# acmater/prograph

Measured on AMD Instinct MI355X. Metric: sequence-pairs/s, higher is better.
Workload: dtype u8; 1 GPU; cfg3: N=200000 L=64 Hamming, kNN k=16; N=200000, L=64, rows_per_gpu=200000, alphabet=5-bit tokens 1..20, parallelism=rowblock1, engine=mfma

## Files before the change

include/prograph_hip.h:

```cpp
#ifndef PROGRAPH_HIP_H
#define PROGRAPH_HIP_H

#include <stdint.h>

#ifdef __cplusplus
extern "C" {
#endif

#define PG_ABI_VERSION 3

#define PG_E_BADARG   (-1)
#define PG_E_TOOLONG  (-2)
#define PG_E_TOOMANY  (-3)
#define PG_E_NODEV    (-4)
#define PG_E_COMM     (-5)

#define PG_MAX_L      128
#define PG_MAX_L_5BIT 255
#define PG_MAX_N_KNN  16777216
#define PG_MAX_K      63
#define PG_LEV_MAX_BAND 8

#define PG_BITS_5 5
#define PG_BITS_8 8

#define PG_CMP_LE 0
#define PG_CMP_LT 1
#define PG_CMP_EQ 2
#define PG_CMP_GE 3
#define PG_CMP_GT 4
#define PG_CMP_KEEP_ZERO 0x10

int         pg_version(void);
const char *pg_last_error(void);
int         pg_device_info(int *cu_count, int *wave_size, char *arch, int arch_len);

int64_t     pg_npad(int64_t n);
int         pg_ngroups(int l);
int         pg_nchunks(int l, int bits);
int64_t     pg_planes_bytes(int64_t n, int l, int bits);
int64_t     pg_workspace_bytes(int64_t nrows);

int pg_pack_planes(const void *src, int elem_bytes, int64_t n, int l, int64_t ld,
                   const int64_t *rows, int bits, void *planes, int64_t npad, uint32_t *flags,
                   void *stream);

int pg_pack_bytes(const uint8_t *src, int64_t n, int width, int64_t ld, const int64_t *rows, const uint8_t *lut256,
                  int bits, void *planes, int64_t npad, uint8_t *tokens_out, uint32_t *flags, void *stream);

int pg_hamming_dense(const void *x_planes, int64_t n, int64_t x_npad,
                     const void *y_planes, int64_t m, int64_t y_npad,
                     int l, int bits, void *out, int out_elem_bytes, int64_t ldo,
                     int accumulate, void *stream);

int pg_eps_slots(const void *row_planes, int64_t row_npad, int64_t row0, int64_t nrows,
                 const void *col_planes, int64_t col_npad, int64_t ncols,
                 int l, int bits, int cmp, double eps, int cap,
                 int32_t *slot_idx, uint8_t *slot_w, uint32_t *counts, void *workspace, void *stream);

int pg_eps_slots_sym(const void *planes, int64_t npad, int64_t n, int l, int bits, int cmp, double eps, int cap,
                     int32_t *slot_idx, uint8_t *slot_w, uint32_t *counts_up, uint32_t *counts_lo, void *workspace,
                     void *stream);
int pg_eps_compact_sym(const void *planes, int64_t npad, int64_t n, int l, int bits, int cmp, double eps, int cap,
                       const int32_t *slot_idx, const uint8_t *slot_w, const uint32_t *counts_up,
                       const uint32_t *counts_lo, const int64_t *indptr, int32_t *indices, uint8_t *weights,
                       int leave_overflow, void *stream);

int64_t pg_scan_scratch_bytes(int64_t n);
int pg_exclusive_scan(const uint32_t *counts, int64_t n, int64_t *indptr, void *scratch,
                      void *stream);

int pg_eps_compact(const void *row_planes, int64_t row_npad, int64_t row0, int64_t nrows,
                   const void *col_planes, int64_t col_npad, int64_t ncols,
                   int l, int bits, int cmp, double eps, int cap,
                   const int32_t *slot_idx, const uint8_t *slot_w, const uint32_t *counts,
                   const int64_t *indptr, int32_t *indices, uint8_t *weights, int leave_overflow, void *stream);

int pg_eps_fill_rows(const void *row_planes, int64_t row_npad, int64_t row0, const int64_t *row_list, int64_t n_list,
                     const void *col_planes, int64_t col_npad, int64_t ncols, int l, int bits, int cmp, double eps,
                     const int64_t *indptr, int32_t *indices, uint8_t *weights, uint32_t *scratch_counts, void *workspace,
                     void *stream);

int pg_knn_hamming(const void *row_planes, int64_t row_npad, int64_t row0, int64_t nrows,
                   const void *col_planes, int64_t col_npad, int64_t ncols,
                   int l, int bits, int k, int32_t *idx_out, uint8_t *dist_out,
                   void *workspace, void *stream);

int64_t pg_knn_sym_plan(int64_t n, int64_t slots, int piece, int piece_min, int32_t *out, int64_t max_passes);

int pg_knn_hamming_round(const void *row_planes, int64_t row_npad, int64_t row0, int64_t nrows,
                         const void *col_planes, int64_t col_npad, int64_t ncols, int l, int bits,
                         int k, int first_round, const uint32_t *floor_keys, uint32_t *last_keys,
                         int32_t *idx_out, uint8_t *dist_out, void *workspace, void *stream);

int64_t pg_query_workspace_bytes(int64_t nq, int64_t ndb, int k);
int pg_query_knn_hamming(const void *q_planes, int64_t nq, int64_t q_npad, const void *db_planes, int64_t ndb,
                         int64_t db_npad, int l, int bits, int k, const uint32_t *floor_keys, uint32_t *last_keys,
                         int32_t *idx_out, uint8_t *dist_out, void *workspace, int64_t workspace_bytes, void *stream);

int64_t pg_query_eps_segments(int64_t nq, int64_t ndb);
int pg_query_eps_count(const void *q_planes, int64_t nq, int64_t q_npad, const void *db_planes, int64_t ndb,
                       int64_t db_npad, int l, int bits, int cmp, double eps, int64_t nseg, uint32_t *seg_counts,
                       void *stream);
int pg_query_eps_fill(const void *q_planes, int64_t nq, int64_t q_npad, const void *db_planes, int64_t ndb,
                      int64_t db_npad, int l, int bits, int cmp, double eps, int64_t nseg, const int64_t *seg_indptr,
                      int32_t *indices, uint8_t *weights, void *stream);

int pg_index_flags(const void *planes, int64_t n, int64_t npad, int l, int bits,
                   int64_t ref, const uint32_t *want_dist, int pos_mode,
                   const uint32_t *pos_mask, const uint32_t *not_mask,
                   uint8_t *dist_out, uint64_t *hist, uint8_t *flags, void *stream);

int pg_lev_profile(const uint8_t *tokens, int64_t n, int l, int64_t ld, void *profiles,
                   int64_t npad, int32_t *lens, uint32_t *flags, void *stream);
int pg_lev_candidates(const void *profiles, int64_t npad, int64_t n, int64_t row0, int64_t nrows,
                      int band, int cap, int32_t *slot_idx, uint8_t *slot_w, uint32_t *counts,
                      void *stream);
int pg_lev_candidates_sym(const void *profiles, int64_t npad, int64_t n, int band, int cap,
                          int32_t *slot_idx, uint8_t *slot_w, int32_t *slot_aux, uint32_t *counts_up,
                          uint32_t *counts_lo, void *stream);
int pg_lev_knn(const uint8_t *tokens, int64_t n, int l, int64_t ld, const void *planes128,
               int64_t npad, const int32_t *lens, int64_t row0, int64_t nrows, int band, int k,
               int cap, const int32_t *slot_idx, uint8_t *slot_w, const int32_t *slot_aux,
               const uint32_t *counts, const uint32_t *counts_lo, int32_t *idx_out, uint8_t *dist_out,
               void *stream);

int pg_levenshtein_dense(const void *x_planes128, int64_t n, int64_t x_npad, const int32_t *x_lens,
                         const void *y_planes128, int64_t m, int64_t y_npad, const int32_t *y_lens, int l,
                         void *out, int out_elem_bytes, int64_t ldo, void *stream);
int pg_lev_eps_pairs(const uint8_t *tokens, int64_t n, int l, int64_t ld, const void *planes128,
                     int64_t npad, const int32_t *lens, int band, int cap, const int32_t *slot_idx,
                     uint8_t *slot_w, const int32_t *slot_aux, const uint32_t *counts_up,
                     const uint32_t *counts_lo, void *stream);
int pg_lev_eps_count(int64_t n, int cap, int cmp, int thr, const uint8_t *slot_w,
                     const uint32_t *counts_up, const uint32_t *counts_lo, uint32_t *counts_out,
                     void *stream);
int pg_lev_eps_fill(int64_t n, int cap, int cmp, int thr, const int32_t *slot_idx, const uint8_t *slot_w,
                    const uint32_t *counts_up, const uint32_t *counts_lo, const int64_t *indptr,
                    int32_t *indices, uint8_t *weights, void *stream);

#define PG_LEV_LONG_MAX_L 2048
int pg_lev_long_pack(const uint8_t *tokens, int64_t n, int l, int64_t ld, void *planes, int64_t npad, int32_t *lens,
                     uint32_t *flags, void *stream);
int pg_levenshtein_long_dense(const void *x_planes, int64_t n, int64_t x_npad, const int32_t *x_lens, int xl,
                              const void *y_planes, int64_t m, int64_t y_npad, const int32_t *y_lens, int yl, void *out,
                              int out_elem_bytes, int64_t ldo, void *stream);

int pg_sub_pack(const uint8_t *tokens, int64_t n, int l, int64_t ld, int a, void *packed, int64_t npad,
                uint32_t *flags, void *stream);
int pg_substitution_dense(const void *x_packed, int64_t n, int64_t x_npad, const void *y_packed, int64_t m,
                          int64_t y_npad, int l, const uint8_t *cost_u8, void *out, int64_t ldo,
                          int out_elem_bytes, int accumulate, void *stream);

int pg_alignment_dense(const void *x_packed, int64_t n, int64_t x_npad, int xl, const void *y_packed, int64_t m,
                       int64_t y_npad, int yl, const uint8_t *cost_u8, int gap, void *out, int64_t ldo,
                       int out_elem_bytes, void *stream);

int pg_alignment_affine_dense(const void *x_packed, int64_t n, int64_t x_npad, int xl, const void *y_packed, int64_t m,
                              int64_t y_npad, int yl, const uint8_t *cost_u8, int gap, int gap_open, void *out,
                              int64_t ldo, int out_elem_bytes, void *stream);

int pg_alignment_local_dense(const void *x_packed, int64_t n, int64_t x_npad, int xl, const void *y_packed, int64_t m,
                             int64_t y_npad, int yl, const int8_t *score_i8, int gap, int gap_open, void *out,
                             int64_t ldo, int out_elem_bytes, void *stream);

#define PG_ALN_LONG_MAX_L 2048
int pg_alignment_long_workspace(int xl, int64_t *one_workgroup_bytes, int64_t *full_bytes);
int pg_alignment_long_dense(const void *x_packed, int64_t n, int64_t x_npad, int xl, const void *y_packed, int64_t m,
                            int64_t y_npad, int yl, const uint8_t *cost_u8, int gap, int gap_open, void *out,
                            int64_t ldo, int out_elem_bytes, void *workspace, int64_t workspace_bytes, void *stream);
int pg_alignment_local_long_dense(const void *x_packed, int64_t n, int64_t x_npad, int xl, const void *y_packed, int64_t m,
                                  int64_t y_npad, int yl, const int8_t *score_i8, int gap, int gap_open, void *out,
                                  int64_t ldo, int out_elem_bytes, void *workspace, int64_t workspace_bytes,
                                  void *stream);

int pg_alignment_semiglobal_dense(const void *x_packed, int64_t n, int64_t x_npad, int xl, const void *y_packed, int64_t m,
                                  int64_t y_npad, int yl, const int8_t *score_i8, int gap, int gap_open, void *out,
                                  int64_t ldo, int out_elem_bytes, void *stream);
int pg_alignment_semiglobal_long_dense(const void *x_packed, int64_t n, int64_t x_npad, int xl, const void *y_packed, int64_t m,
                                       int64_t y_npad, int yl, const int8_t *score_i8, int gap, int gap_open, void *out,
                                       int64_t ldo, int out_elem_bytes, void *workspace, int64_t workspace_bytes,
                                       void *stream);

int pg_alignment_fit_dense(const void *x_packed, int64_t n, int64_t x_npad, int xl, const void *y_packed, int64_t m,
                           int64_t y_npad, int yl, const int8_t *score_i8, int gap, int gap_open, int bias, void *out,
                           int64_t ldo, int out_elem_bytes, void *stream);
int pg_alignment_fit_long_dense(const void *x_packed, int64_t n, int64_t x_npad, int xl, const void *y_packed, int64_t m,
                                int64_t y_npad, int yl, const int8_t *score_i8, int gap, int gap_open, int bias, void *out,
                                int64_t ldo, int out_elem_bytes, void *workspace, int64_t workspace_bytes, void *stream);

int pg_alignment_profile_dense(int mode, const void *x_packed, int64_t n, int64_t x_npad, int xl, const void *profiles,
                               const int32_t *lengths, int64_t m, int lpad, int yl, int bias, int top, int gap, int gap_open,
                               int out_bias, void *out, int64_t ldo, int out_elem_bytes, void *stream);
int pg_alignment_profile_long_dense(int mode, const void *x_packed, int64_t n, int64_t x_npad, int xl, const void *profiles,
                                    const int32_t *lengths, int64_t m, int lpad, int yl, int bias, int top, int gap,
                                    int gap_open, int out_bias, void *out, int64_t ldo, int out_elem_bytes, void *workspace,
                                    int64_t workspace_bytes, void *stream);

#define PG_ALN_TRACE_GLOBAL 0
#define PG_ALN_TRACE_LOCAL 1
#define PG_ALN_TRACE_SEMIGLOBAL 2
int pg_alignment_trace_workspace(int xl, int yl, int64_t *bytes_per_wave);
int pg_alignment_trace(int mode, const void *x_packed, int64_t n, int64_t x_npad, int xl, const void *y_packed, int64_t m,
                       int64_t y_npad, int yl, const int32_t *xi, const int32_t *yi, int64_t npairs, const void *table, int gap,
                       int gap_open, int32_t *head, uint8_t *ops, int64_t ldo, void *workspace, int64_t workspace_bytes,
                       void *stream);
int pg_alignment_trace_long_workspace(int xl, int yl, int64_t *bytes_per_wave);
int pg_alignment_trace_long(int mode, const void *x_packed, int64_t n, int64_t x_npad, int xl, const void *y_packed, int64_t m,
                            int64_t y_npad, int yl, const int32_t *xi, const int32_t *yi, int64_t npairs, const void *table,
                            int gap, int gap_open, int32_t *head, uint8_t *ops, int64_t ldo, void *workspace,
                            int64_t workspace_bytes, void *stream);
int pg_alignment_fit_trace(const void *x_packed, int64_t n, int64_t x_npad, int xl, const void *y_packed, int64_t m,
                           int64_t y_npad, int yl, const int32_t *xi, const int32_t *yi, int64_t npairs, const void *table,
                           int gap, int gap_open, int32_t *head, uint8_t *ops, int64_t ldo, void *workspace,
                           int64_t workspace_bytes, void *stream);
int pg_alignment_fit_trace_long(const void *x_packed, int64_t n, int64_t x_npad, int xl, const void *y_packed, int64_t m,
                                int64_t y_npad, int yl, const int32_t *xi, const int32_t *yi, int64_t npairs,
                                const void *table, int gap, int gap_open, int32_t *head, uint8_t *ops, int64_t ldo,
                                void *workspace, int64_t workspace_bytes, void *stream);

int pg_alignment_stats(int mode, const void *x_packed, int64_t n, int64_t x_npad, int xl, const void *y_packed, int64_t m,
                       int64_t y_npad, int yl, const int32_t *xi, const int32_t *yi, int64_t npairs, const void *table, int gap,
                       int gap_open, int32_t *head, void *stream);

int pg_alignment_list_scores(int mode, const void *x_packed, int64_t n, int64_t x_npad, int xl, const void *y_packed, int64_t m,
                             int64_t y_npad, int yl, const int64_t *indptr, const int32_t *indices, const void *table, int gap,
                             int gap_open, int32_t *scores, void *stream);

int pg_alignment_list_long_scores(int mode, const void *x_packed, int64_t n, int64_t x_npad, int xl, const void *y_packed,
                                  int64_t m, int64_t y_npad, int yl, const int64_t *indptr, const int32_t *indices,
                                  const void *table, int gap, int gap_open, int32_t *scores, void *workspace,
                                  int64_t workspace_bytes, void *stream);

int pg_spectrum_dims(int k, int symbols, int dims);
int pg_spectrum_profile(const uint8_t *tokens, int64_t n, int l, int64_t ld, const int64_t *rows, int k, int symbols, int dims,
                        void *out_f16, int64_t ldo, int32_t *flags, void *stream);

int pg_csr_row_stats(const int64_t *indptr, const int32_t *indices, const uint8_t *weights_u8,
                     const float *weights_f32, int64_t nrows, int64_t row0, const double *f, double *deg,
                     double *sum_f, double *sum_wf, double *self_w, double *col_sum, void *stream);

#define PG_W_UNSIGNED 0
#define PG_W_SIGNED 1
#define PG_W_FLOAT 2
#define PG_SYM_UNION 0
#define PG_SYM_MUTUAL 1
#define PG_COMBINE_MIN 0
#define PG_COMBINE_MAX 1
int64_t pg_csr_sort_workspace(int64_t nnz);
int pg_csr_sort_rows_count(const int64_t *indptr, const int32_t *indices, int64_t nrows, int64_t nnz, int64_t ncols,
                           uint32_t *counts, void *workspace, int64_t workspace_bytes, void *stream);
int pg_csr_sort_rows_fill(const int64_t *indptr, const void *weights, int elem_bytes, int64_t nrows, int64_t nnz,
                          const uint32_t *counts, const int64_t *out_indptr, int32_t *out_indices, void *out_weights,
                          const void *workspace, int64_t workspace_bytes, void *stream);
int pg_csr_histogram(const int32_t *indices, int64_t nnz, int64_t ncols, uint32_t *counts, void *stream);
int64_t pg_csr_transpose_workspace(int64_t nnz, int64_t ncols);
int pg_csr_transpose(const int64_t *indptr, const int32_t *indices, const void *weights, int elem_bytes, int64_t nrows,
                     int64_t nnz, int64_t ncols, int64_t row0, const int64_t *t_indptr, int32_t *t_indices, void *t_weights,
                     void *workspace, int64_t workspace_bytes, void *stream);
int64_t pg_csr_symmetrize_workspace(int64_t nnz_a, int64_t nnz_t);
int pg_csr_symmetrize_count(const int64_t *a_indptr, const int32_t *a_indices, const void *a_weights, int64_t nnz_a,
                            const int64_t *t_indptr, const int32_t *t_indices, const void *t_weights, int64_t nnz_t,
                            int elem_bytes, int kind, int mode, int combine, int64_t nrows, uint32_t *counts, void *workspace,
                            int64_t workspace_bytes, void *stream);
int pg_csr_symmetrize_fill(const int64_t *a_indptr, int64_t nnz_a, const int64_t *t_indptr, int64_t nnz_t, int elem_bytes,
                           int64_t nrows, const int64_t *out_indptr, int32_t *out_indices, void *out_weights,
                           const void *workspace, int64_t workspace_bytes, void *stream);

int pg_compact_flags(const uint8_t *flags, int64_t n, int64_t *out_idx, int64_t *out_count,
                     void *scratch, void *stream);

int pg_f16_nchunks(int d);
int pg_pack_f16(const void *src_f16, int64_t n, int d, int64_t ld, const int64_t *rows, void *packed, int64_t npad,
                void *stream);
int pg_minkowski_dense(const void *x_packed, int64_t n, int64_t x_npad, const void *y_packed, int64_t m,
                       int64_t y_npad, int d, int similarity, void *out_f16, int64_t ldo, void *stream);
int pg_f16_knn(const void *dist_f16, int64_t m, int64_t n, int64_t ld, int k, int first, int descending,
               int32_t *idx_out, void *w_out_f16, void *stream);
int pg_f16_knn_round(const void *dist_f16, int64_t m, int64_t n, int64_t ld, int k, int descending,
                     const int32_t *floor_idx, const void *floor_w_f16, int64_t floor_ld, int32_t *idx_out,
                     void *w_out_f16, int64_t ldo, void *stream);
int pg_f16_eps_count(const void *dist_f16, int64_t m, int64_t n, int64_t ld, int cmp, float eps_f16, int similarity,
                     uint32_t *counts, void *stream);
int pg_f16_eps_fill(const void *dist_f16, int64_t m, int64_t n, int64_t ld, int cmp, float eps_f16, int similarity,
                    const int64_t *indptr, int32_t *indices, void *weights_f16, void *stream);

int pg_i32_knn(const int32_t *vals, int64_t m, int64_t n, int64_t ld, int k, int first, int descending, int32_t *idx_out,
               int32_t *w_out, void *stream);
int pg_i32_knn_round(const int32_t *vals, int64_t m, int64_t n, int64_t ld, int k, int descending,
                     const int32_t *floor_idx, const int32_t *floor_w, int64_t floor_ld, int32_t *idx_out, int32_t *w_out,
                     int64_t ldo, void *stream);
int pg_i32_eps_count(const int32_t *vals, int64_t m, int64_t n, int64_t ld, int cmp, int64_t thr, uint32_t *counts,
                     void *stream);
int pg_i32_eps_fill(const int32_t *vals, int64_t m, int64_t n, int64_t ld, int cmp, int64_t thr, const int64_t *indptr,
                    int32_t *indices, int32_t *weights, void *stream);

int pg_minkowski_knn(const void *x_packed, int64_t n, int64_t x_npad, const void *y_packed, int64_t m, int64_t y_npad,
                     int d, int similarity, int k, int first, int32_t *idx_out, void *w_out_f16, void *stream);
int pg_minkowski_knn_round(const void *x_packed, int64_t n, int64_t x_npad, const void *y_packed, int64_t m,
                           int64_t y_npad, int d, int similarity, int k, const int32_t *floor_idx,
                           const void *floor_w_f16, int64_t floor_ld, int32_t *idx_out, void *w_out_f16, int64_t ldo,
                           void *stream);
int pg_minkowski_eps_slots(const void *x_packed, int64_t n, int64_t x_npad, const void *y_packed, int64_t m,
                           int64_t y_npad, int d, int similarity, int cmp, float eps_f16, int cap, int32_t *slot_idx,
                           void *slot_w_f16, uint32_t *counts, void *stream);
int pg_minkowski_eps_compact(int64_t m, int cap, const int32_t *slot_idx, const void *slot_w_f16, const uint32_t *counts,
                             const int64_t *indptr, int32_t *indices, void *weights_f16, void *stream);
int pg_minkowski_eps_fill_rows(const void *x_packed, int64_t n, int64_t x_npad, const void *y_packed, int64_t m,
                               int64_t y_npad, int d, int similarity, int cmp, float eps_f16, const int64_t *row_list,
                               int64_t n_list, const int64_t *indptr, int32_t *indices, void *weights_f16, void *stream);

int pg_cosine_prep(const void *packed, int64_t n, int64_t npad, int d, float *norms, float *rnorms, uint32_t *flags,
                   void *stream);
int pg_cosine_dense(const void *x_packed, const float *x_norms, const float *x_rnorms, int64_t n, int64_t x_npad,
                    const void *y_packed, const float *y_norms, const float *y_rnorms, int64_t m, int64_t y_npad, int d,
                    int similarity, float *out, int64_t ldo, void *stream);
int pg_cosine_knn(const void *x_packed, const float *x_norms, const float *x_rnorms, int64_t n, int64_t x_npad,
                  const void *y_packed, const float *y_norms, const float *y_rnorms, int64_t m, int64_t y_npad, int d,
                  int similarity, int k, int first, int32_t *idx_out, float *w_out, void *stream);
int pg_cosine_knn_round(const void *x_packed, const float *x_norms, const float *x_rnorms, int64_t n, int64_t x_npad,
                        const void *y_packed, const float *y_norms, const float *y_rnorms, int64_t m, int64_t y_npad, int d,
                        int similarity, int k, const int32_t *floor_idx, const float *floor_w, int64_t floor_ld,
                        int32_t *idx_out, float *w_out, int64_t ldo, void *stream);
int pg_cosine_eps_slots(const void *x_packed, const float *x_norms, const float *x_rnorms, int64_t n, int64_t x_npad,
                        const void *y_packed, const float *y_norms, const float *y_rnorms, int64_t m, int64_t y_npad, int d,
                        int similarity, int cmp, float eps, int cap, int32_t *slot_idx, float *slot_w, uint32_t *counts,
                        void *stream);
int pg_cosine_eps_compact(int64_t m, int cap, const int32_t *slot_idx, const float *slot_w, const uint32_t *counts,
                          const int64_t *indptr, int32_t *indices, float *weights, void *stream);
int pg_cosine_eps_fill_rows(const void *x_packed, const float *x_norms, const float *x_rnorms, int64_t n, int64_t x_npad,
                            const void *y_packed, const float *y_norms, const float *y_rnorms, int64_t m, int64_t y_npad,
                            int d, int similarity, int cmp, float eps, const int64_t *row_list, int64_t n_list,
                            const int64_t *indptr, int32_t *indices, float *weights, void *stream);

int pg_euclidean_dense(const void *x_packed, const float *x_norms, const float *x_rnorms, int64_t n, int64_t x_npad,
                       const void *y_packed, const float *y_norms, const float *y_rnorms, int64_t m, int64_t y_npad, int d,
                       int similarity, float *out, int64_t ldo, void *stream);
int pg_euclidean_knn(const void *x_packed, const float *x_norms, const float *x_rnorms, int64_t n, int64_t x_npad,
                     const void *y_packed, const float *y_norms, const float *y_rnorms, int64_t m, int64_t y_npad, int d,
                     int similarity, int k, int first, int32_t *idx_out, float *w_out, void *stream);
int pg_euclidean_knn_round(const void *x_packed, const float *x_norms, const float *x_rnorms, int64_t n, int64_t x_npad,
                           const void *y_packed, const float *y_norms, const float *y_rnorms, int64_t m, int64_t y_npad,
                           int d, int similarity, int k, const int32_t *floor_idx, const float *floor_w, int64_t floor_ld,
                           int32_t *idx_out, float *w_out, int64_t ldo, void *stream);
int pg_euclidean_eps_slots(const void *x_packed, const float *x_norms, const float *x_rnorms, int64_t n, int64_t x_npad,
                           const void *y_packed, const float *y_norms, const float *y_rnorms, int64_t m, int64_t y_npad,
                           int d, int similarity, int cmp, float eps, int cap, int32_t *slot_idx, float *slot_w,
                           uint32_t *counts, void *stream);
int pg_euclidean_eps_fill_rows(const void *x_packed, const float *x_norms, const float *x_rnorms, int64_t n, int64_t x_npad,
                               const void *y_packed, const float *y_norms, const float *y_rnorms, int64_t m, int64_t y_npad,
                               int d, int similarity, int cmp, float eps, const int64_t *row_list, int64_t n_list,
                               const int64_t *indptr, int32_t *indices, float *weights, void *stream);

#define PG_COMM_ID_BYTES 128
int pg_comm_available(void);
int pg_comm_unique_id(void *id128);
int pg_comm_init(void **comm, int nranks, int rank, const void *id128);
int pg_comm_destroy(void *comm);
int pg_allgather_tokens(void *comm, const void *shard, int64_t rows_per_rank, int l, void *full, void *stream);

#ifdef __cplusplus
}
#endif
#endif
```

prograph_amd/_native.py:

```python
import ctypes
import os
import threading

import numpy as np
import torch

_HERE = os.path.dirname(os.path.abspath(__file__))
LIB_PATH = os.environ.get("PROGRAPH_HIP_LIB") or os.path.join(_HERE, "libprograph_hip.so")
ABI_VERSION = 3

BITS_5, BITS_8 = 5, 8
CMP_LE, CMP_LT, CMP_EQ, CMP_GE, CMP_GT = 0, 1, 2, 3, 4
CMP_KEEP_ZERO = 0x10
MAX_L, MAX_L_5BIT, MAX_K, MAX_K_ROUNDS, MAX_N_KNN, LEV_MAX_BAND = 128, 255, 63, 1023, 1 << 24, 8
SUB_MAX_L, SUB_MAX_A = 2048, 32
ALN_MAX_L, ALN_MAX_GAP = 128, 255
ALN_MAX_OPEN = 255
ALN_LOCAL_MIN, ALN_LOCAL_MAX = -128, 127
ALN_LONG_MAX_L = 2048
ALN_TRACE_GLOBAL, ALN_TRACE_LOCAL, ALN_TRACE_SEMIGLOBAL = 0, 1, 2
ALN_TRACE_FIT = 3
ALN_PROFILE_MODES = ("local", "semiglobal", "fit")
ALN_TRACE_LONG_WORKSPACE = 2 << 30
LEV_LONG_MAX_L = 2048
SPECTRUM_MAX_L, SPECTRUM_MAX_K, SPECTRUM_MAX_D = 2048, 6, 32768
ALN_LONG_CELL_MAX = 65535

SYMBOLS = [
    "pg_version", "pg_last_error", "pg_device_info", "pg_npad", "pg_ngroups", "pg_nchunks", "pg_planes_bytes", "pg_workspace_bytes",
    "pg_pack_planes", "pg_pack_bytes",
    "pg_hamming_dense", "pg_eps_slots", "pg_scan_scratch_bytes", "pg_exclusive_scan",
    "pg_eps_compact", "pg_eps_fill_rows", "pg_eps_slots_sym", "pg_eps_compact_sym", "pg_knn_hamming", "pg_knn_sym_plan", "pg_knn_hamming_round", "pg_index_flags", "pg_compact_flags",
    "pg_lev_profile", "pg_lev_candidates", "pg_lev_candidates_sym", "pg_lev_knn", "pg_csr_row_stats",
    "pg_levenshtein_dense", "pg_lev_eps_pairs", "pg_lev_eps_count", "pg_lev_eps_fill",
    "pg_lev_long_pack", "pg_levenshtein_long_dense",
    "pg_sub_pack", "pg_substitution_dense", "pg_alignment_dense", "pg_alignment_affine_dense",
    "pg_alignment_local_dense", "pg_alignment_long_workspace", "pg_alignment_long_dense", "pg_alignment_local_long_dense",
    "pg_alignment_semiglobal_dense", "pg_alignment_semiglobal_long_dense",
    "pg_alignment_fit_dense", "pg_alignment_fit_long_dense", "pg_alignment_fit_trace", "pg_alignment_fit_trace_long",
    "pg_alignment_profile_dense", "pg_alignment_profile_long_dense",
    "pg_alignment_trace_workspace", "pg_alignment_trace", "pg_alignment_trace_long_workspace", "pg_alignment_trace_long",
    "pg_alignment_stats", "pg_alignment_list_scores", "pg_alignment_list_long_scores",
    "pg_spectrum_dims", "pg_spectrum_profile",
    "pg_i32_knn", "pg_i32_knn_round", "pg_i32_eps_count", "pg_i32_eps_fill",
    "pg_comm_available", "pg_comm_unique_id", "pg_comm_init", "pg_comm_destroy", "pg_allgather_tokens",
    "pg_f16_nchunks", "pg_pack_f16", "pg_minkowski_dense", "pg_f16_knn", "pg_f16_knn_round", "pg_f16_eps_count",
    "pg_f16_eps_fill", "pg_minkowski_knn", "pg_minkowski_knn_round", "pg_minkowski_eps_slots", "pg_minkowski_eps_compact",
    "pg_minkowski_eps_fill_rows", "pg_cosine_prep", "pg_cosine_dense", "pg_cosine_knn", "pg_cosine_knn_round",
    "pg_cosine_eps_slots", "pg_cosine_eps_compact", "pg_cosine_eps_fill_rows",
    "pg_euclidean_dense", "pg_euclidean_knn", "pg_euclidean_knn_round", "pg_euclidean_eps_slots", "pg_euclidean_eps_fill_rows",
    "pg_query_workspace_bytes", "pg_query_knn_hamming",
    "pg_query_eps_segments", "pg_query_eps_count", "pg_query_eps_fill",
    "pg_csr_sort_workspace", "pg_csr_sort_rows_count", "pg_csr_sort_rows_fill", "pg_csr_histogram", "pg_csr_transpose_workspace",
    "pg_csr_transpose", "pg_csr_symmetrize_workspace", "pg_csr_symmetrize_count", "pg_csr_symmetrize_fill",
]


class NativeUnavailable(RuntimeError):
    pass


_lib = None
_lock = threading.Lock()

_i64, _i32, _vp, _dbl = ctypes.c_int64, ctypes.c_int, ctypes.c_void_p, ctypes.c_double
_COS_METRICS = ("cosine", "euclidean")


def _load():
    global _lib
    with _lock:
        if _lib is not None:
            return _lib
        if not os.path.exists(LIB_PATH):
            raise NativeUnavailable(
                f"{LIB_PATH} is missing: build it with `python -c 'import __graft_entry__ as g; g.build()'` "
                "or `make -C prograph_amd/csrc` (hipcc, --offload-arch=gfx950)")
        try:
            lib = ctypes.CDLL(LIB_PATH, mode=ctypes.RTLD_GLOBAL)
        except OSError as e:
            raise NativeUnavailable(f"cannot load {LIB_PATH}: {e}") from e
        missing = [s for s in SYMBOLS if not hasattr(lib, s)]
        if missing:
            raise NativeUnavailable(f"{LIB_PATH} does not export {missing}")
        lib.pg_version.restype = _i32
        if lib.pg_version() != ABI_VERSION:
            raise NativeUnavailable(f"ABI mismatch: library {lib.pg_version()}, binding {ABI_VERSION}")
        lib.pg_last_error.restype = ctypes.c_char_p
        lib.pg_npad.restype = _i64
        lib.pg_npad.argtypes = [_i64]
        lib.pg_ngroups.restype = _i32
        lib.pg_ngroups.argtypes = [_i32]
        lib.pg_nchunks.restype = _i32
        lib.pg_nchunks.argtypes = [_i32, _i32]
        lib.pg_planes_bytes.restype = _i64
        lib.pg_planes_bytes.argtypes = [_i64, _i32, _i32]
        lib.pg_scan_scratch_bytes.restype = _i64
        lib.pg_scan_scratch_bytes.argtypes = [_i64]
        lib.pg_workspace_bytes.restype = _i64
        lib.pg_workspace_bytes.argtypes = [_i64]
        lib.pg_device_info.argtypes = [ctypes.POINTER(_i32), ctypes.POINTER(_i32), ctypes.c_char_p, _i32]
        lib.pg_pack_planes.argtypes = [_vp, _i32, _i64, _i32, _i64, _vp, _i32, _vp, _i64, _vp, _vp]
        lib.pg_pack_bytes.argtypes = [_vp, _i64, _i32, _i64, _vp, _vp, _i32, _vp, _i64, _vp, _vp, _vp]
        lib.pg_hamming_dense.argtypes = [_vp, _i64, _i64, _vp, _i64, _i64, _i32, _i32, _vp, _i32, _i64, _i32, _vp]
        lib.pg_eps_slots.argtypes = [_vp, _i64, _i64, _i64, _vp, _i64, _i64, _i32, _i32, _i32, _dbl, _i32,
                                     _vp, _vp, _vp, _vp, _vp]
        lib.pg_exclusive_scan.argtypes = [_vp, _i64, _vp, _vp, _vp]
        lib.pg_eps_slots_sym.argtypes = [_vp, _i64, _i64, _i32, _i32, _i32, _dbl, _i32, _vp, _vp, _vp, _vp, _vp, _vp]
        lib.pg_eps_compact_sym.argtypes = [_vp, _i64, _i64, _i32, _i32, _i32, _dbl, _i32, _vp, _vp, _vp, _vp, _vp, _vp,
                                           _vp, _i32, _vp]
        lib.pg_eps_compact.argtypes = [_vp, _i64, _i64, _i64, _vp, _i64, _i64, _i32, _i32, _i32, _dbl, _i32,
                                       _vp, _vp, _vp, _vp, _vp, _vp, _i32, _vp]
        lib.pg_eps_fill_rows.argtypes = [_vp, _i64, _i64, _vp, _i64, _vp, _i64, _i64, _i32, _i32, _i32, _dbl,
                                         _vp, _vp, _vp, _vp, _vp, _vp]
        lib.pg_knn_hamming.argtypes = [_vp, _i64, _i64, _i64, _vp, _i64, _i64, _i32, _i32, _i32, _vp, _vp, _vp, _vp]
        lib.pg_knn_sym_plan.restype = _i64
        lib.pg_knn_sym_plan.argtypes = [_i64, _i64, _i32, _i32, _vp, _i64]
        lib.pg_knn_hamming_round.argtypes = [_vp, _i64, _i64, _i64, _vp, _i64, _i64, _i32, _i32, _i32, _i32, _vp, _vp, _vp,
                                             _vp, _vp, _vp]
        lib.pg_query_workspace_bytes.restype = _i64
        lib.pg_query_workspace_bytes.argtypes = [_i64, _i64, _i32]
        lib.pg_query_knn_hamming.argtypes = [_vp, _i64, _i64, _vp, _i64, _i64, _i32, _i32, _i32, _vp, _vp, _vp, _vp, _vp,
                                             _i64, _vp]
        lib.pg_query_eps_segments.restype = _i64
        lib.pg_query_eps_segments.argtypes = [_i64, _i64]
        lib.pg_query_eps_count.argtypes = [_vp, _i64, _i64, _vp, _i64, _i64, _i32, _i32, _i32, _dbl, _i64, _vp, _vp]
        lib.pg_query_eps_fill.argtypes = [_vp, _i64, _i64, _vp, _i64, _i64, _i32, _i32, _i32, _dbl, _i64, _vp, _vp, _vp, _vp]
        lib.pg_index_flags.argtypes = [_vp, _i64, _i64, _i32, _i32, _i64, _vp, _i32, _vp, _vp, _vp, _vp, _vp, _vp]
        lib.pg_compact_flags.argtypes = [_vp, _i64, _vp, _vp, _vp, _vp]
        lib.pg_csr_row_stats.argtypes = [_vp, _vp, _vp, _vp, _i64, _i64, _vp, _vp, _vp, _vp, _vp, _vp, _vp]
        lib.pg_csr_sort_workspace.restype = lib.pg_csr_transpose_workspace.restype = lib.pg_csr_symmetrize_workspace.restype = _i64
        lib.pg_csr_sort_workspace.argtypes = [_i64]
        lib.pg_csr_transpose_workspace.argtypes = lib.pg_csr_symmetrize_workspace.argtypes = [_i64, _i64]
        lib.pg_csr_sort_rows_count.argtypes = [_vp, _vp, _i64, _i64, _i64, _vp, _vp, _i64, _vp]
        lib.pg_csr_sort_rows_fill.argtypes = [_vp, _vp, _i32, _i64, _i64, _vp, _vp, _vp, _vp, _vp, _i64, _vp]
        lib.pg_csr_histogram.argtypes = [_vp, _i64, _i64, _vp, _vp]
        lib.pg_csr_transpose.argtypes = [_vp, _vp, _vp, _i32, _i64, _i64, _i64, _i64, _vp, _vp, _vp, _vp, _i64, _vp]
        lib.pg_csr_symmetrize_count.argtypes = [_vp, _vp, _vp, _i64, _vp, _vp, _vp, _i64, _i32, _i32, _i32, _i32, _i64, _vp, _vp,
                                                _i64, _vp]
        lib.pg_csr_symmetrize_fill.argtypes = [_vp, _i64, _vp, _i64, _i32, _i64, _vp, _vp, _vp, _vp, _i64, _vp]
        lib.pg_lev_profile.argtypes = [_vp, _i64, _i32, _i64, _vp, _i64, _vp, _vp, _vp]
        lib.pg_lev_candidates.argtypes = [_vp, _i64, _i64, _i64, _i64, _i32, _i32, _vp, _vp, _vp, _vp]
        lib.pg_lev_candidates_sym.argtypes = [_vp, _i64, _i64, _i32, _i32, _vp, _vp, _vp, _vp, _vp, _vp]
        lib.pg_lev_knn.argtypes = [_vp, _i64, _i32, _i64, _vp, _i64, _vp, _i64, _i64, _i32, _i32, _i32, _vp, _vp, _vp, _vp,
                                   _vp, _vp, _vp, _vp]
        lib.pg_levenshtein_dense.argtypes = [_vp, _i64, _i64, _vp, _vp, _i64, _i64, _vp, _i32, _vp, _i32, _i64, _vp]
        lib.pg_lev_eps_pairs.argtypes = [_vp, _i64, _i32, _i64, _vp, _i64, _vp, _i32, _i32, _vp, _vp, _vp, _vp, _vp, _vp]
        lib.pg_lev_eps_count.argtypes = [_i64, _i32, _i32, _i32, _vp, _vp, _vp, _vp, _vp]
        lib.pg_lev_eps_fill.argtypes = [_i64, _i32, _i32, _i32, _vp, _vp, _vp, _vp, _vp, _vp, _vp, _vp]
        lib.pg_lev_long_pack.argtypes = [_vp, _i64, _i32, _i64, _vp, _i64, _vp, _vp, _vp]
        lib.pg_levenshtein_long_dense.argtypes = [_vp, _i64, _i64, _vp, _i32, _vp, _i64, _i64, _vp, _i32, _vp, _i32, _i64, _vp]
        lib.pg_sub_pack.argtypes = [_vp, _i64, _i32, _i64, _i32, _vp, _i64, _vp, _vp]
        lib.pg_substitution_dense.argtypes = [_vp, _i64, _i64, _vp, _i64, _i64, _i32, _vp, _vp, _i64, _i32, _i32, _vp]
        lib.pg_alignment_dense.argtypes = [_vp, _i64, _i64, _i32, _vp, _i64, _i64, _i32, _vp, _i32, _vp, _i64, _i32, _vp]
        lib.pg_alignment_affine_dense.argtypes = [_vp, _i64, _i64, _i32, _vp, _i64, _i64, _i32, _vp, _i32, _i32, _vp, _i64, _i32,
                                                  _vp]
        lib.pg_alignment_local_dense.argtypes = lib.pg_alignment_affine_dense.argtypes
        lib.pg_alignment_long_workspace.argtypes = [_i32, ctypes.POINTER(_i64), ctypes.POINTER(_i64)]
        lib.pg_alignment_long_dense.argtypes = [_vp, _i64, _i64, _i32, _vp, _i64, _i64, _i32, _vp, _i32, _i32, _vp, _i64, _i32,
                                                _vp, _i64, _vp]
        lib.pg_alignment_local_long_dense.argtypes = lib.pg_alignment_long_dense.argtypes
        lib.pg_alignment_semiglobal_dense.argtypes = lib.pg_alignment_affine_dense.argtypes
        lib.pg_alignment_semiglobal_long_dense.argtypes = lib.pg_alignment_long_dense.argtypes
        lib.pg_alignment_fit_dense.argtypes = [_vp, _i64, _i64, _i32, _vp, _i64, _i64, _i32, _vp, _i32, _i32, _i32, _vp, _i64,
                                               _i32, _vp]
        lib.pg_alignment_fit_long_dense.argtypes = [_vp, _i64, _i64, _i32, _vp, _i64, _i64, _i32, _vp, _i32, _i32, _i32, _vp,
                                                    _i64, _i32, _vp, _i64, _vp]
        lib.pg_alignment_profile_dense.argtypes = [_i32, _vp, _i64, _i64, _i32, _vp, _vp, _i64, _i32, _i32, _i32, _i32, _i32, _i32,
                                                   _i32, _vp, _i64, _i32, _vp]
        lib.pg_alignment_profile_long_dense.argtypes = lib.pg_alignment_profile_dense.argtypes[:-1] + [_vp, _i64, _vp]
        lib.pg_alignment_trace_workspace.argtypes = [_i32, _i32, ctypes.POINTER(_i64)]
        lib.pg_alignment_trace.argtypes = [_i32, _vp, _i64, _i64, _i32, _vp, _i64, _i64, _i32, _vp, _vp, _i64, _vp, _i32, _i32,
                                           _vp, _vp, _i64, _vp, _i64, _vp]
        lib.pg_alignment_trace_long_workspace.argtypes = lib.pg_alignment_trace_workspace.argtypes
        lib.pg_alignment_trace_long.argtypes = lib.pg_alignment_trace.argtypes
        lib.pg_alignment_fit_trace.argtypes = lib.pg_alignment_trace.argtypes[1:]
        lib.pg_alignment_fit_trace_long.argtypes = lib.pg_alignment_trace.argtypes[1:]
        lib.pg_alignment_stats.argtypes = lib.pg_alignment_trace.argtypes[:16] + [_vp]
        lib.pg_alignment_list_scores.argtypes = [_i32, _vp, _i64, _i64, _i32, _vp, _i64, _i64, _i32, _vp, _vp, _vp, _i32, _i32, _vp, _vp]
        lib.pg_alignment_list_long_scores.argtypes = [_i32, _vp, _i64, _i64, _i32, _vp, _i64, _i64, _i32, _vp, _vp, _vp, _i32, _i32, _vp,
                                                      _vp, _i64, _vp]
        lib.pg_spectrum_dims.argtypes = [_i32, _i32, _i32]
        lib.pg_spectrum_profile.argtypes = [_vp, _i64, _i32, _i64, _vp, _i32, _i32, _i32, _vp, _i64, _vp, _vp]
        lib.pg_i32_knn.argtypes = [_vp, _i64, _i64, _i64, _i32, _i32, _i32, _vp, _vp, _vp]
        lib.pg_i32_knn_round.argtypes = [_vp, _i64, _i64, _i64, _i32, _i32, _vp, _vp, _i64, _vp, _vp, _i64, _vp]
        lib.pg_i32_eps_count.argtypes = [_vp, _i64, _i64, _i64, _i32, _i64, _vp, _vp]
        lib.pg_i32_eps_fill.argtypes = [_vp, _i64, _i64, _i64, _i32, _i64, _vp, _vp, _vp, _vp]
        lib.pg_f16_nchunks.argtypes = [_i32]
        lib.pg_pack_f16.argtypes = [_vp, _i64, _i32, _i64, _vp, _vp, _i64, _vp]
        lib.pg_minkowski_dense.argtypes = [_vp, _i64, _i64, _vp, _i64, _i64, _i32, _i32, _vp, _i64, _vp]
        lib.pg_f16_knn.argtypes = [_vp, _i64, _i64, _i64, _i32, _i32, _i32, _vp, _vp, _vp]
        lib.pg_f16_knn_round.argtypes = [_vp, _i64, _i64, _i64, _i32, _i32, _vp, _vp, _i64, _vp, _vp, _i64, _vp]
        lib.pg_f16_eps_count.argtypes = [_vp, _i64, _i64, _i64, _i32, ctypes.c_float, _i32, _vp, _vp]
        lib.pg_f16_eps_fill.argtypes = [_vp, _i64, _i64, _i64, _i32, ctypes.c_float, _i32, _vp, _vp, _vp, _vp]
        lib.pg_minkowski_knn.argtypes = [_vp, _i64, _i64, _vp, _i64, _i64, _i32, _i32, _i32, _i32, _vp, _vp, _vp]
        lib.pg_minkowski_knn_round.argtypes = [_vp, _i64, _i64, _vp, _i64, _i64, _i32, _i32, _i32, _vp, _vp, _i64, _vp, _vp,
                                               _i64, _vp]
        lib.pg_minkowski_eps_slots.argtypes = [_vp, _i64, _i64, _vp, _i64, _i64, _i32, _i32, _i32, ctypes.c_float, _i32,
                                               _vp, _vp, _vp, _vp]
        lib.pg_minkowski_eps_compact.argtypes = [_i64, _i32, _vp, _vp, _vp, _vp, _vp, _vp, _vp]
        lib.pg_minkowski_eps_fill_rows.argtypes = [_vp, _i64, _i64, _vp, _i64, _i64, _i32, _i32, _i32, ctypes.c_float, _vp,
                                                   _i64, _vp, _vp, _vp, _vp]
        _ops = [_vp, _vp, _vp, _i64, _i64, _vp, _vp, _vp, _i64, _i64, _i32, _i32]
        lib.pg_cosine_prep.argtypes = [_vp, _i64, _i64, _i32, _vp, _vp, _vp, _vp]
        lib.pg_cosine_eps_compact.argtypes = [_i64, _i32, _vp, _vp, _vp, _vp, _vp, _vp, _vp]
        for metric in _COS_METRICS:
            getattr(lib, f"pg_{metric}_dense").argtypes = _ops + [_vp, _i64, _vp]
            getattr(lib, f"pg_{metric}_knn").argtypes = _ops + [_i32, _i32, _vp, _vp, _vp]
            getattr(lib, f"pg_{metric}_knn_round").argtypes = _ops + [_i32, _vp, _vp, _i64, _vp, _vp, _i64, _vp]
            getattr(lib, f"pg_{metric}_eps_slots").argtypes = _ops + [_i32, ctypes.c_float, _i32, _vp, _vp, _vp, _vp]
            getattr(lib, f"pg_{metric}_eps_fill_rows").argtypes = _ops + [_i32, ctypes.c_float, _vp, _i64, _vp, _vp, _vp, _vp]
        lib.pg_comm_unique_id.argtypes = [_vp]
        lib.pg_comm_init.argtypes = [ctypes.POINTER(_vp), _i32, _i32, _vp]
        lib.pg_comm_destroy.argtypes = [_vp]
        lib.pg_allgather_tokens.argtypes = [_vp, _vp, _i64, _i32, _vp, _vp]
        for name in SYMBOLS:
            fn = getattr(lib, name)
            if fn.restype is ctypes.c_int and name not in ("pg_version",):
                fn.restype = _i32
        _lib = lib
        return lib


def lib():
    return _load()


def device():
    if not torch.cuda.is_available():
        raise NativeUnavailable("no HIP device visible to torch; the Hamming/graph path has no CPU fallback")
    return torch.device("cuda", torch.cuda.current_device())


def _check(rc, what):
    if rc != 0:
        msg = lib().pg_last_error().decode("utf-8", "replace")
        raise RuntimeError(f"{what} failed (rc={rc}): {msg}")


def _stream():
    return ctypes.c_void_p(torch.cuda.current_stream().cuda_stream)


def _ptr(t):
    return ctypes.c_void_p(0) if t is None else ctypes.c_void_p(t.data_ptr())


def workspace(nrows, dev):
    return torch.empty(int(lib().pg_workspace_bytes(int(nrows))), dtype=torch.uint8, device=dev)


def npad(n):
    return ((max(int(n), 1) + 255) // 256) * 256


def ngroups(l):
    return (max(int(l), 1) + 31) // 32


def nchunks(l, bits):
    return (ngroups(l) * int(bits) + 3) // 4


def planes_bytes(n, l, bits):
    return (nchunks(l, bits) * 16 + 64) * npad(n)


class Planes:
    __slots__ = ("buf", "n", "l", "npad", "g", "q", "bits", "flags")

    def __init__(self, buf, n, l, bits, flags=None):
        self.buf, self.n, self.l, self.bits, self.flags = buf, int(n), int(l), int(bits), flags
        self.npad, self.g, self.q = npad(n), ngroups(l), nchunks(l, bits)

    def ensure_valid(self):
        if self.flags is not None and int(self.flags.item()):
            raise ValueError(f"tokens outside 0..{(1 << self.bits) - 1} cannot be packed with {self.bits} bit planes")
        self.flags = None

    @property
    def nbytes(self):
        return self.buf.numel()


def pack(tokens, rows=None, bits=None, width=None, check=True):
    L = lib()
    dev = device()
    if not isinstance(tokens, torch.Tensor):
        tokens = torch.from_numpy(np.ascontiguousarray(np.asarray(tokens)))
    if tokens.dim() != 2:
        raise ValueError("token matrix must be 2-D")
    if tokens.dtype not in (torch.uint8, torch.int8, torch.int16, torch.int32, torch.int64):
        raise TypeError(f"integer tokens expected, got {tokens.dtype}")
    if tokens.dtype == torch.int8:
        tokens = tokens.to(torch.int16)
    tokens = tokens.to(dev).contiguous()
    n_src, l = tokens.shape
    lw = l if width is None else int(width)
    if lw < l:
        raise ValueError("width smaller than the token matrix")
    if lw > MAX_L_5BIT:
        raise ValueError(f"L={lw} exceeds the native limit of {MAX_L_5BIT}")
    ridx = None
    n = n_src
    if rows is not None:
        ridx = torch.as_tensor(np.asarray(rows), dtype=torch.int64).reshape(-1)
        if ridx.numel() and (int(ridx.min()) < -n_src or int(ridx.max()) >= n_src):
            raise IndexError("row index out of range")
        ridx = torch.where(ridx < 0, ridx + n_src, ridx).to(dev)
        n = int(ridx.numel())
    if n == 0 or l == 0:
        raise ValueError("empty token matrix")
    if bits is None:
        lo, hi = int(tokens.min()), int(tokens.max())
        if lo < 0 or hi > 255:
            raise ValueError("tokens outside 0..255 cannot use the byte-token Hamming path")
        bits = BITS_5 if hi <= 31 else BITS_8
    if lw > (MAX_L_5BIT if bits == BITS_5 else MAX_L):
        raise ValueError(f"L={lw} exceeds the native limit for {bits} bit planes")
    np_ = npad(n)
    if lw != l:
        wide = torch.zeros((n_src, lw), dtype=tokens.dtype, device=dev)
        wide[:, :l] = tokens
        tokens = wide
    buf = torch.empty(planes_bytes(n, lw, bits), dtype=torch.uint8, device=dev)
    flags = torch.empty(1, dtype=torch.int32, device=dev)
    _check(L.pg_pack_planes(_ptr(tokens), tokens.element_size(), n, lw, tokens.stride(0), _ptr(ridx), int(bits),
                            _ptr(buf), np_, _ptr(flags), _stream()), "pg_pack_planes")
    planes = Planes(buf, n, lw, bits, flags)
    if check:
        planes.ensure_valid()
    return planes


def pack_bytes(raw, lut, bits=BITS_5, want_tokens=True, check=True):
    L = lib()
    dev = device()
    if not isinstance(raw, torch.Tensor):
        raw = torch.from_numpy(np.ascontiguousarray(np.asarray(raw, dtype=np.uint8)))
    if raw.dim() != 2 or raw.dtype != torch.uint8:
        raise TypeError("pack_bytes expects a 2-D uint8 byte matrix")
    raw = raw.to(dev).contiguous()
    n, width = raw.shape
    if n == 0 or width == 0:
        raise ValueError("empty byte matrix")
    if width > (MAX_L_5BIT if bits == BITS_5 else MAX_L):
        raise ValueError(f"L={width} exceeds the native limit for {bits} bit planes")
    lut_t = torch.as_tensor(np.asarray(lut, dtype=np.uint8).reshape(256)).to(dev)
    np_ = npad(n)
    buf = torch.empty(planes_bytes(n, width, bits), dtype=torch.uint8, device=dev)
    flags = torch.empty(1, dtype=torch.int32, device=dev)
    tokens = torch.empty((n, width), dtype=torch.uint8, device=dev) if want_tokens else None
    _check(L.pg_pack_bytes(_ptr(raw), n, width, raw.stride(0), None, _ptr(lut_t), int(bits), _ptr(buf), np_, _ptr(tokens),
                           _ptr(flags), _stream()), "pg_pack_bytes")
    planes = Planes(buf, n, width, bits, flags)
    if check:
        planes.ensure_valid()
    return planes, tokens


_TORCH_OUT = {1: torch.uint8, 2: torch.float16, 4: torch.int32, 8: torch.int64}


def hamming_dense(xp, yp, out_bytes=8, out=None):
    if xp.g != yp.g or xp.bits != yp.bits:
        raise ValueError("operands must be packed with the same width and bit planes")
    accumulate = out is not None
    if out is None:
        out = torch.empty((yp.n, xp.n), dtype=_TORCH_OUT[out_bytes], device=xp.buf.device)
    out_bytes = out.element_size()
    _check(lib().pg_hamming_dense(_ptr(xp.buf), xp.n, xp.npad, _ptr(yp.buf), yp.n, yp.npad, xp.g * 32, xp.bits,
                                  _ptr(out), out_bytes, out.stride(0), 1 if accumulate else 0, _stream()),
           "pg_hamming_dense")
    return out


def _bits2(rp, cp):
    if rp.bits != cp.bits or rp.g != cp.g:
        raise ValueError("row and column operands must be packed with the same width and bit planes")
    return rp.bits


def _csr_alloc(counts, wdtype, extra=None):
    L = lib()
    m, dev = counts.numel(), counts.device
    indptr = torch.empty(m + 1, dtype=torch.int64, device=dev)
    scratch = torch.empty(int(L.pg_scan_scratch_bytes(m)), dtype=torch.uint8, device=dev)
    _check(L.pg_exclusive_scan(_ptr(counts), m, _ptr(indptr), _ptr(scratch), _stream()), "pg_exclusive_scan")
    if extra is None:
        nnz, also = int(indptr[-1].item()), ()
    else:
        nnz, *also = (int(v) for v in torch.stack([indptr[-1], extra]).cpu())
    indices = torch.empty(max(nnz, 1), dtype=torch.int32, device=dev)[:nnz]
    weights = torch.empty(max(nnz, 1), dtype=wdtype, device=dev)[:nnz]
    return (indptr, indices, weights, *also)


def cat_csr(parts):
    if len(parts) == 1:
        return parts[0]
    base, ptrs = 0, [torch.zeros(1, dtype=torch.int64, device=parts[0][0].device)]
    for indptr, _, _ in parts:
        ptrs.append(indptr[1:] + base)
        base += int(indptr[-1].item())
    return torch.cat(ptrs), torch.cat([p_[1] for p_ in parts]), torch.cat([p_[2] for p_ in parts])


def eps_graph(rp, cp, cmp, eps, row0=0, nrows=None, cap=256):
    L = lib()
    nrows = rp.n - row0 if nrows is None else int(nrows)
    dev = rp.buf.device
    bits = _bits2(rp, cp)
    cap = int(cap)
    symenv = os.environ.get("PG_EPS_SYM", "auto")
    sym = (rp is cp and row0 == 0 and nrows == rp.n and rp.n < (1 << 27) and cap >= 2 and symenv != "0"
           and (symenv == "1" or rp.n >= 32768))
    counts = torch.empty(nrows, dtype=torch.int32, device=dev)
    counts_lo = torch.empty(nrows, dtype=torch.int32, device=dev) if sym else None
    slot_idx = torch.empty(nrows * cap, dtype=torch.int32, device=dev)
    slot_w = torch.empty(nrows * cap, dtype=torch.uint8, device=dev)
# ... 1266 lines not shown
```

prograph_amd/csrc/pg_api.hip:

```cpp
#include "pg_common.h"
#include "pg_mm.h"
#include "pg_plan.h"
#include "../../include/prograph_hip.h"

#include <dlfcn.h>
#include <math.h>
#include <rccl/rccl.h>
#include <stdio.h>
#include <stdlib.h>
#include <string.h>
#include <atomic>
#include <mutex>

static thread_local char g_err[256] = "";

void pg_set_error(const char *msg) { snprintf(g_err, sizeof(g_err), "%s", msg); }

extern char **environ;
static PgKnobs read_knobs() { return pg_knobs_read(environ); }

#define PG_MAX_DEVICES 64
static int cu_count() {
  static std::atomic<int> cus[PG_MAX_DEVICES];
  int dev = 0;
  if (hipGetDevice(&dev) != hipSuccess) return 0;
  const bool cached = dev >= 0 && dev < PG_MAX_DEVICES;
  if (cached && cus[dev].load(std::memory_order_relaxed) > 0) return cus[dev].load(std::memory_order_relaxed);
  hipDeviceProp_t prop;
  if (hipGetDeviceProperties(&prop, dev) != hipSuccess) return 0;
  if (cached) cus[dev].store(prop.multiProcessorCount, std::memory_order_relaxed);
  return prop.multiProcessorCount;
}

extern "C" {

int pg_version(void) { return PG_ABI_VERSION; }
const char *pg_last_error(void) { return g_err; }

int pg_device_info(int *cus, int *wave, char *arch, int arch_len) {
  int dev = 0;
  hipDeviceProp_t prop;
  hipError_t e = hipGetDevice(&dev);
  if (e != hipSuccess) return pg_launched((int)e, "hipGetDevice");
  e = hipGetDeviceProperties(&prop, dev);
  if (e != hipSuccess) return pg_launched((int)e, "hipGetDeviceProperties");
  if (cus) *cus = prop.multiProcessorCount;
  if (wave) *wave = prop.warpSize;
  if (arch && arch_len > 0) snprintf(arch, (size_t)arch_len, "%s", prop.gcnArchName);
  return 0;
}

int64_t pg_npad(int64_t n) { return n <= 0 ? 256 : ((n + 255) / 256) * 256; }
int pg_ngroups(int l) { return plan_ngroups(l); }
int pg_nchunks(int l, int bits) { return plan_nchunks(l, bits); }
int64_t pg_planes_bytes(int64_t n, int l, int bits) { return ((int64_t)pg_nchunks(l, bits) * 16 + PG_AUX_BYTES) * pg_npad(n); }
int64_t pg_workspace_bytes(int64_t nrows) { return workspace_bytes(nrows, cu_count(), read_knobs()); }

}

__global__ __launch_bounds__(1024) void pg_knn_sym_plan_kernel(long long nb, long long nst, long long slots, int piece, int pmin,
                                                                int4 *plan, u32 *pieceStart, uint4 *zero, long long zero4) {
  __shared__ u32 sums[1024];
  const int t = threadIdx.x;
  if (blockIdx.x > 0) {
    for (long long i = (long long)(blockIdx.x - 1) * 1024 + t; i < zero4; i += (long long)(gridDim.x - 1) * 1024) zero[i] = make_uint4(0u, 0u, 0u, 0u);
    return;
  }
  const long long per = (nb + 1023) / 1024, b0 = t * per, b1 = b0 + per < nb ? b0 + per : nb;
  u32 mine = 0;
  for (long long b = b0; b < b1; ++b) mine += (u32)sym_block_pieces(b, nst, slots, piece, pmin);
  sums[t] = mine;
  __syncthreads();
  for (int o = 1; o < 1024; o <<= 1) {
    const u32 x = t >= o ? sums[t - o] : 0u;
    __syncthreads();
    sums[t] += x;
    __syncthreads();
  }
  u32 at = sums[t] - mine;
  for (long long b = b0; b < b1; ++b) {
    const int np = sym_block_pieces(b, nst, slots, piece, pmin);
    pieceStart[b] = at;
    for (int q = 0; q < np; ++q, ++at) {
      int f, e;
      sym_piece_range(b, nst, np, q, &f, &e);
      plan[at] = make_int4((int)b, f, e, q);
    }
  }
  if (t == 1023) pieceStart[nb] = sums[1023];
}
extern "C" {
int64_t pg_knn_sym_plan(int64_t n, int64_t slots, int piece, int piece_min, int32_t *out, int64_t max_passes) {
  if (n <= 0 || slots <= 0) return pg_fail(PG_E_BADARG, "pg_knn_sym_plan: bad argument");
  return sym_plan_host(n, slots, piece, piece_min > 0 ? piece_min : (int)read_knobs().symPieceMin.v, out, max_passes);
}
}

#define PG_PACK_SEQS 64
#define PG_PACK_LD 68

__host__ __device__ __forceinline__ unsigned long long pg_transpose8(unsigned long long x) {
  unsigned long long t;
  t = (x ^ (x >> 7)) & 0x00AA00AA00AA00AAull;  x = x ^ t ^ (t << 7);
  t = (x ^ (x >> 14)) & 0x0000CCCC0000CCCCull; x = x ^ t ^ (t << 14);
  t = (x ^ (x >> 28)) & 0x00000000F0F0F0F0ull; x = x ^ t ^ (t << 28);
  return x;
}

template <typename T, int B>
__global__ __launch_bounds__(256) void pg_pack_kernel(const T *__restrict__ src, long long n, int l, long long ld,
                                                      const long long *__restrict__ rows, u32 *__restrict__ planes,
                                                      long long npad, int ng, int nq, u32 *flags,
                                                      const unsigned char *__restrict__ lut = nullptr,
                                                      unsigned char *__restrict__ tokOut = nullptr) {
  constexpr int E = (int)sizeof(T), PER = 16 / E;
  __shared__ __attribute__((aligned(16))) u32 words[PG_PACK_SEQS * PG_PACK_LD];
  const long long s0 = (long long)blockIdx.x * PG_PACK_SEQS;
  const int tid = threadIdx.x;
  const bool vec = !lut && ((unsigned long long)src & 15ull) == 0 && ((ld * E) & 15ll) == 0;
  for (int item = tid; item < PG_PACK_SEQS * ng; item += 256) {
    const int sl = item / ng, g = item - sl * ng;
    const long long s = s0 + sl;
    unsigned long long x[4] = {0, 0, 0, 0}, high = 0;
    if (s < n) {
      const T *row = src + (rows ? rows[s] : s) * ld;
      if (vec && g * 32 + 32 <= l) {
        const uint4 *r16 = reinterpret_cast<const uint4 *>(row + g * 32);
#pragma unroll
        for (int c = 0; c < 32 / PER; ++c) {
          const uint4 v = r16[c];
          T e[PER];
          __builtin_memcpy(e, &v, 16);
#pragma unroll
          for (int i = 0; i < PER; ++i) {
            const int j = c * PER + i;
            const unsigned long long t = (unsigned long long)(long long)e[i];
            high |= t;
            x[j >> 3] |= (t & 0xFFull) << (8 * (j & 7));
          }
        }
      } else {
#pragma unroll
        for (int j = 0; j < 32; ++j) {
          const int pos = g * 32 + j;
          if (pos < l) {
            long long v = (long long)row[pos];
            if (lut) {
              v = lut[(unsigned char)v];
              if (tokOut) tokOut[s * (long long)l + pos] = (unsigned char)v;
            }
            high |= (unsigned long long)v;
            x[j >> 3] |= ((unsigned long long)v & 0xFFull) << (8 * (j & 7));
          }
        }
      }
    }
    if (high >> B) atomicOr(flags, 1u);
#pragma unroll
    for (int i = 0; i < 4; ++i) x[i] = pg_transpose8(x[i]);
#pragma unroll
    for (int p = 0; p < B; ++p) {
      const u32 w = (u32)((x[0] >> (8 * p)) & 0xFFull) | (u32)((x[1] >> (8 * p)) & 0xFFull) << 8 |
                    (u32)((x[2] >> (8 * p)) & 0xFFull) << 16 | (u32)((x[3] >> (8 * p)) & 0xFFull) << 24;
      words[sl * PG_PACK_LD + p * ng + g] = w;
    }
  }
  __syncthreads();
  const int nw = ng * B;
  for (int item = tid; item < PG_PACK_SEQS * nq; item += 256) {
    const int q = item / PG_PACK_SEQS, sl = item % PG_PACK_SEQS;
    uint4 v = *reinterpret_cast<const uint4 *>(&words[sl * PG_PACK_LD + 4 * q]);
    if (4 * q + 1 >= nw) v.y = 0;
    if (4 * q + 2 >= nw) v.z = 0;
    if (4 * q + 3 >= nw) v.w = 0;
    reinterpret_cast<uint4 *>(planes)[(long long)q * npad + s0 + sl] = v;
  }
  const int sl = tid & 63;
  const long long s = s0 + sl;
  if (tid < 64) {
    u32 sigw[2] = {0, 0};
    for (int g = 0; g < ng; ++g) sigw[g & 1] ^= words[sl * PG_PACK_LD + g];
    const unsigned long long sig = pg_sig54(sigw[0], sigw[1]);
    const u32 lo = (u32)sig, hi = (u32)(sig >> 32) | (s < n ? 0xFFC00000u : 0u);
    uint4 *e = reinterpret_cast<uint4 *>(planes + (long long)nq * npad * 4) + (s >> 5) * 64 + (s & 31);
    e[0] = make_uint4(pg_nib8(lo) << 1, pg_nib8(lo >> 8) << 1, pg_nib8(lo >> 16) << 1, pg_nib8(lo >> 24) << 1);
    e[32] = make_uint4(pg_nib8(hi) << 1, pg_nib8(hi >> 8) << 1, pg_nib8(hi >> 16) << 1, pg_nib8(hi >> 24) << 1);
  } else if (tid < 128) {
    u32 fold[8] = {0, 0, 0, 0, 0, 0, 0, 0};
#pragma unroll
    for (int p = 0; p < B; ++p)
      for (int g = 0; g < ng; ++g) fold[p] ^= words[sl * PG_PACK_LD + p * ng + g];
    uint4 *f = reinterpret_cast<uint4 *>(planes + (long long)nq * npad * 4) + npad * 2;
    f[s] = make_uint4(fold[0], fold[1], fold[2], fold[3]);
    f[npad + s] = make_uint4(fold[4], fold[5], fold[6], fold[7]);
  }
}

#define PG_SCAN_TILE 2048

template <typename T>
__device__ __forceinline__ long long scan_val(const T *in, long long i, long long n) {
  return i < n ? (long long)(in[i] != 0 ? (sizeof(T) == 1 ? 1 : in[i]) : 0) : 0;
}

__device__ __forceinline__ long long wave_incl_scan(long long v, int lane) {
#pragma unroll
  for (int o = 1; o < 64; o <<= 1) {
    long long t = __shfl_up(v, o);
    if (lane >= o) v += t;
  }
  return v;
}

__device__ __forceinline__ long long block_excl_scan(long long v, long long &total) {
  __shared__ long long wsum[4];
  const int lane = threadIdx.x & 63, wv = threadIdx.x >> 6;
  const long long inc = wave_incl_scan(v, lane);
  if (lane == 63) wsum[wv] = inc;
  __syncthreads();
  long long base = 0;
  for (int w = 0; w < wv; ++w) base += wsum[w];
  total = wsum[0] + wsum[1] + wsum[2] + wsum[3];
  __syncthreads();
  return base + inc - v;
}

template <typename T>
__global__ __launch_bounds__(256) void pg_scan_partials(const T *__restrict__ in, long long n, long long *partials) {
  const long long b0 = (long long)blockIdx.x * PG_SCAN_TILE;
  long long s = 0;
#pragma unroll
  for (int j = 0; j < 8; ++j) s += scan_val(in, b0 + threadIdx.x * 8 + j, n);
  long long total;
  block_excl_scan(s, total);
  if (threadIdx.x == 0) partials[blockIdx.x] = total;
}

__global__ __launch_bounds__(256) void pg_scan_single(long long *partials, long long nb) {
  long long carry = 0;
  for (long long c0 = 0; c0 < nb; c0 += 256) {
    const long long i = c0 + threadIdx.x;
    const long long v = i < nb ? partials[i] : 0;
    long long total;
    const long long ex = block_excl_scan(v, total);
    if (i < nb) partials[i] = carry + ex;
    carry += total;
  }
  if (threadIdx.x == 0) partials[nb] = carry;
}

template <typename T, int MODE>
__global__ __launch_bounds__(256) void pg_scan_apply(const T *__restrict__ in, long long n, const long long *partials,
                                                     long long nb, long long *out, long long *count) {
  const long long b0 = (long long)blockIdx.x * PG_SCAN_TILE;
  long long v[8], s = 0;
#pragma unroll
  for (int j = 0; j < 8; ++j) { v[j] = scan_val(in, b0 + threadIdx.x * 8 + j, n); s += v[j]; }
  long long total;
  long long ex = block_excl_scan(s, total) + partials[blockIdx.x];
#pragma unroll
  for (int j = 0; j < 8; ++j) {
    const long long i = b0 + threadIdx.x * 8 + j;
    if (i < n) {
      if (MODE == 0) out[i] = ex;
      else if (v[j]) out[ex] = i;
    }
    ex += v[j];
  }
  if (blockIdx.x == 0 && threadIdx.x == 0) {
    if (MODE == 0) out[n] = partials[nb];
    if (count) *count = partials[nb];
  }
}

template <int B>
__global__ __launch_bounds__(256) void pg_index_kernel(const u32 *__restrict__ planes, long long n, long long npad, int ng,
                                                       long long ref, const u32 *__restrict__ want, int posMode,
                                                       const u32 *__restrict__ posMask, const u32 *__restrict__ notMask,
                                                       unsigned char *distOut, u64 *hist, unsigned char *flags) {
  __shared__ u32 lh[256];
  lh[threadIdx.x] = 0;
  __syncthreads();
  const long long s = (long long)blockIdx.x * 256 + threadIdx.x;
  if (s < n) {
    u32 d = 0, anyP = 0, anyNot = 0;
    bool allP = true;
    for (int g = 0; g < ng; ++g) {
      u32 t = 0;
#pragma unroll
      for (int p = 0; p < B; ++p) {
        const int w = p * ng + g;
        const long long base = (long long)(w >> 2) * npad;
        t |= planes[(base + s) * 4 + (w & 3)] ^ planes[(base + ref) * 4 + (w & 3)];
      }
      d += __builtin_popcount(t);
      if (posMode) {
        const u32 pm = posMask[g], nm = notMask[g];
        anyP |= t & pm;
        allP = allP && ((t & pm) == pm);
        anyNot |= t & nm;
      }
    }
    if (distOut) distOut[s] = (unsigned char)d;
    if (hist) atomicAdd(&lh[d & 255u], 1u);
    if (flags) {
      bool ok = want ? ((want[(d >> 5) & 7u] >> (d & 31u)) & 1u) != 0 : true;
      if (posMode == 1) ok = ok && (anyP != 0) && (anyNot == 0);
      if (posMode == 2) ok = ok && allP && (anyNot == 0);
      flags[s] = ok ? 1 : 0;
    }
  }
  __syncthreads();
  if (hist && lh[threadIdx.x]) atomicAdd((unsigned long long *)&hist[threadIdx.x], (unsigned long long)lh[threadIdx.x]);
}

__device__ __forceinline__ double wave_sum(double v) {
#pragma unroll
  for (int o = 32; o > 0; o >>= 1) v += __shfl_down(v, o);
  return v;
}

__global__ __launch_bounds__(256) void pg_csr_row_stats_kernel(const long long *__restrict__ indptr,
                                                               const int *__restrict__ indices,
                                                               const unsigned char *__restrict__ w8,
                                                               const float *__restrict__ wf, long long nrows,
                                                               long long row0, const double *__restrict__ f, double *deg,
                                                               double *sf, double *swf, double *selfw, double *colsum) {
  const int lane = threadIdx.x & 63;
  const long long row = (long long)blockIdx.x * 4 + (threadIdx.x >> 6);
  if (row >= nrows) return;
  const long long a = indptr[row], b = indptr[row + 1];
  double d = 0, s1 = 0, s2 = 0, sw = 0;
  for (long long e = a + lane; e < b; e += 64) {
    const double w = w8 ? (double)w8[e] : (wf ? (double)wf[e] : 1.0);
    const int col = indices[e];
    if (col < 0) continue;
    const double fj = f ? f[col] : 0.0;
    d += w; s1 += fj; s2 += w * fj;
    if (col == row0 + row) sw += w;
    if (colsum) atomicAdd(&colsum[col], w);
  }
  d = wave_sum(d); s1 = wave_sum(s1); s2 = wave_sum(s2); sw = wave_sum(sw);
  if (lane == 0) {
    if (deg) deg[row] = d;
    if (sf) sf[row] = s1;
    if (swf) swf[row] = s2;
    if (selfw) selfw[row] = sw;
  }
}

static int check_l(int l, int bits = 8, bool exact = false) {
  if (l <= 0) return pg_fail(PG_E_BADARG, "sequence length must be positive");
  const int maxg = bits == 5 ? PG_MAX_L_5BIT / 32 + 1 : PG_MAX_L / 32;
  if ((l + 31) / 32 > maxg || (exact && l > (bits == 5 ? PG_MAX_L_5BIT : PG_MAX_L)))
    return pg_fail(PG_E_TOOLONG, "sequence length exceeds the native limit (128 tokens, 255 with 5 bit planes)");
  return 0;
}
static int check_bits(int b) {
  if (b != PG_BITS_5 && b != PG_BITS_8) return pg_fail(PG_E_BADARG, "bits must be 5 or 8");
  return 0;
}

static void eps_interval(int cmp, double eps, u32 *lo, u32 *span, long long dmin = 1) {
  const long long INF = 1000000;
  long long l = dmin, h = INF;
  switch (cmp) {
    case PG_CMP_LE: h = (long long)floor(eps); break;
    case PG_CMP_LT: h = (long long)ceil(eps) - 1; break;
    case PG_CMP_EQ:
      if (floor(eps) == eps) { l = (long long)eps; h = (long long)eps; } else { l = 1; h = 0; }
      break;
    case PG_CMP_GE: l = (long long)ceil(eps); break;
    case PG_CMP_GT: l = (long long)floor(eps) + 1; break;
  }
  if (l < dmin) l = dmin;
  if (h > INF) h = INF;
  if (h < l) { *lo = 0xFFFFFF00u; *span = 0; return; }
  *lo = (u32)l;
  *span = (u32)(h - l);
}

__global__ __launch_bounds__(1024) void pg_decide_kernel(const u32 *counts, int nsample, int wavesPerRow, u32 need, long long ncols,
                                                          int force, u32 *gate, u32 *line, int lineWords) {
  __shared__ u32 sClustered[16];
  __shared__ unsigned long long sEps[16], sNear[16];
  const int tid = threadIdx.x, s = tid >> 4, sub = tid & 15;
  if (tid < lineWords) line[tid] = 0u;
  u32 nearS = 0, epsS = 0;
  if (s < nsample)
    for (int w = sub; w < wavesPerRow; w += 16) {
      nearS += counts[2 * (s * wavesPerRow + w)];
      epsS += counts[2 * (s * wavesPerRow + w) + 1];
    }
  for (int o = 8; o > 0; o >>= 1) {
    nearS += (u32)__shfl_xor((int)nearS, o);
    epsS += (u32)__shfl_xor((int)epsS, o);
  }
  u32 clustered = (sub == 0 && s < nsample && nearS * PG_PROBE_STRIDE >= need) ? 1u : 0u;
  unsigned long long eps = (sub == 0 && s < nsample) ? (unsigned long long)epsS * PG_PROBE_STRIDE : 0ull;
  unsigned long long nearAll = (sub == 0 && s < nsample) ? (unsigned long long)nearS * PG_PROBE_STRIDE : 0ull;
  for (int o = 32; o > 0; o >>= 1) {
    clustered += (u32)__shfl_xor((int)clustered, o);
    eps += (unsigned long long)__shfl_xor((long long)eps, o);
    nearAll += (unsigned long long)__shfl_xor((long long)nearAll, o);
  }
  if ((tid & 63) == 0) { sClustered[tid >> 6] = clustered; sEps[tid >> 6] = eps; sNear[tid >> 6] = nearAll; }
  __syncthreads();
  if (tid == 0) {
    clustered = 0; eps = 0; nearAll = 0;
    for (int i = 0; i < 16; ++i) { clustered += sClustered[i]; eps += sEps[i]; nearAll += sNear[i]; }
    const bool oneCluster = 2ull * nearAll > (unsigned long long)nsample * (unsigned long long)ncols;
    gate[0] = force >= 0 ? (u32)(force & 1) + ((force & 4) ? 2u : 0u) : (2u * clustered >= (u32)nsample ? (oneCluster ? 2u : 0u) : 1u);
    gate[1] = force >= 0 ? (u32)((force >> 1) & 1) : (eps * 25ull > (unsigned long long)nsample * (unsigned long long)ncols ? 1u : 0u);
  }
}
__global__ __launch_bounds__(PG_WG_THREADS) void pg_knn_merge_kernel(const u32 *partial, long long nrows, int pieces, int k, int *idx,
                                                                     unsigned char *dist, u32 cap, u32 *evictCount, u32 *evictRows,
                                                                     long long rowAbs0, const u32 *gate, u32 gateMask) {
  __shared__ u32 keys[PG_WG_WAVES][4][16 * PG_MM_KL];
  if (gate && !((gateMask >> __builtin_nontemporal_load(gate)) & 1u)) return;
  const int lane = threadIdx.x & 63, wv = threadIdx.x >> 6, g = lane >> 4, b = lane & 15;
  const long long row0 = ((long long)blockIdx.x * PG_WG_WAVES + wv) * 4;
  if (row0 >= nrows) return;
  const int k1 = k + 1, n = pieces * k1;
  for (int r = 0; r < 4; ++r)
    if (row0 + r < nrows)
      for (int e = lane; e < n; e += 64) keys[wv][r][e] = partial[(row0 + r) * n + e];
  __builtin_amdgcn_fence(__ATOMIC_RELEASE, "wavefront");
  __builtin_amdgcn_wave_barrier();
  __builtin_amdgcn_fence(__ATOMIC_ACQUIRE, "wavefront");
  const long long row = row0 + g;
  const bool mine = row < nrows && b < pieces;
  int pos = 0;
  u32 head = mine ? keys[wv][g][b * k1] : 0xFFFFFFFFu;
  for (int r = 0; r <= k; ++r) {
    u32 m = head;
    for (int o = 8; o > 0; o >>= 1) {
      const u32 x = (u32)__shfl_xor((int)m, o, 16);
      m = x < m ? x : m;
    }
    if (b == 0 && row < nrows) {
      if (r >= 1) {
        idx[row * k + r - 1] = m == 0xFFFFFFFFu ? -1 : (int)(m & 0x00FFFFFFu);
        dist[row * k + r - 1] = (unsigned char)(m >> 24);
      }
      if (r == k && (m >> 24) >= cap) evictRows[atomicAdd(evictCount, 1u)] = (u32)(rowAbs0 + row);
    }
    if (mine && head == m && m != 0xFFFFFFFFu) {
      ++pos;
      head = pos < k1 ? keys[wv][g][b * k1 + pos] : 0xFFFFFFFFu;
    }
  }
}

#define PG_SYM_ROR(x, N) ((u32)__builtin_amdgcn_update_dpp(0, (int)(x), 0x120 + (N), 0xF, 0xF, false))
#define PG_SYM_CE(a, b) { const u32 x_ = a, y_ = b; a = x_ < y_ ? x_ : y_; b = x_ < y_ ? y_ : x_; }
__global__ __launch_bounds__(PG_WG_THREADS) __attribute__((amdgpu_waves_per_eu(7, 8))) void pg_knn_sym_merge_kernel(const u32 *partial, const u32 *pieceStart, const u32 *lowCount,
                                                                         const u32 *lowKeys, u32 capL, int rowBits, long long nrows, int k, int *idx,
                                                                         unsigned char *dist, u32 cap, u32 *evictCount, u32 *evictRows,
                                                                         const u32 *gate, u32 gateMask, u32 *gate2, u32 *ticket, u32 limit) {
  constexpr int kRec = PG_MM_KL, kOwn = PG_SYM_MAX_PIECES * kRec, kLane = PG_SYM_MAX_CAPL / 16;
  static_assert(kRec == 20 && kLane == 16, "records of whole uint4; sixteen delivered keys a lane");
  __shared__ __attribute__((aligned(16))) u32 keys[PG_WG_WAVES][4][kOwn];
  static_assert(4 * PG_WG_WAVES * PG_SYM_MAX_CAPL <= PG_WG_WAVES * 4 * kOwn, "the bins fit the records' block");
  u32 (*bins)[PG_SYM_MAX_CAPL] = reinterpret_cast<u32 (*)[PG_SYM_MAX_CAPL]>(&keys[0][0][0]);
  __shared__ u32 binCount[2][4 * PG_WG_WAVES];
  const u32 gv = gate ? __builtin_nontemporal_load(gate) : 0u;
  const int lane = threadIdx.x & 63, wv = threadIdx.x >> 6, g = lane >> 4, b = lane & 15;
  const bool open = !gate || ((gateMask >> gv) & 1u);
  if (threadIdx.x < 4 * PG_WG_WAVES) binCount[0][threadIdx.x] = 0u;
  int trip = 0;
  for (long long first = (long long)blockIdx.x * (4 * PG_WG_WAVES); open && first < nrows; first += (long long)gridDim.x * (4 * PG_WG_WAVES), trip ^= 1) {
    const int k1 = k + 1, off = kRec - k1;
    const long long blk = first >> 6;
    const long long row = first + 4 * wv + g;
    const bool mine = row < nrows;
    const long long rowIn = mine ? row : first;
    const u32 s0 = pieceStart[blk], s1 = pieceStart[blk + 1];
    const u32 logged = lowCount[first];
    u32 np = s1 - s0;
    np = np > PG_SYM_MAX_PIECES ? PG_SYM_MAX_PIECES : np;
    u32 *own = &keys[wv][g][0];
    const bool has = mine && b < (int)np;
    const uint4 *rec = reinterpret_cast<const uint4 *>(partial) + (((long long)s0 + (b < (int)np ? b : 0)) * 64 + (rowIn & 63)) * (kRec / 4);
    const uint4 r0 = rec[0], r1 = rec[1], r2 = rec[2], r3 = rec[3], r4 = rec[4];
    const u32 capG = sym_group_cap((u32)nrows, (u32)first, capL);
    const u32 nlog = logged < capG ? logged : capG;
    const u32 *log = lowKeys + first * (long long)capL;
    __syncthreads();
    for (u32 e0 = threadIdx.x; e0 < nlog; e0 += 4 * PG_WG_THREADS) {
      u32 en[4];
#pragma unroll
      for (int j = 0; j < 4; ++j) en[j] = e0 + j * PG_WG_THREADS < nlog ? log[e0 + j * PG_WG_THREADS] : 0u;
#pragma unroll
      for (int j = 0; j < 4; ++j) {
        if (e0 + j * PG_WG_THREADS < nlog) {
          const u32 place = sym_entry_place(en[j]);
          const u32 at = atomicAdd(&binCount[trip][place], 1u);
          if (at < capL) bins[place][at] = sym_entry_key(en[j], rowBits);
        }
      }
    }
    if (threadIdx.x < 4 * PG_WG_WAVES) binCount[trip ^ 1][threadIdx.x] = 0u;
    __syncthreads();
    const u32 cnt = mine ? binCount[trip][4 * wv + g] : 0u;
    const int nl = (int)(cnt < capL ? cnt : capL);
    const u32 *low = &bins[4 * wv + g][b];
    u32 d0, d1, d2, d3, d4, d5, d6, d7, d8, d9, d10, d11, d12, d13, d14, d15;
#define PG_SYM_BIN(j, d) d = 16 * j + b < nl ? low[16 * j] : 0xFFFFFFFFu;
    PG_SYM_BIN(0, d0) PG_SYM_BIN(1, d1) PG_SYM_BIN(2, d2) PG_SYM_BIN(3, d3) PG_SYM_BIN(4, d4) PG_SYM_BIN(5, d5) PG_SYM_BIN(6, d6) PG_SYM_BIN(7, d7)
    PG_SYM_BIN(8, d8) PG_SYM_BIN(9, d9) PG_SYM_BIN(10, d10) PG_SYM_BIN(11, d11) PG_SYM_BIN(12, d12) PG_SYM_BIN(13, d13) PG_SYM_BIN(14, d14) PG_SYM_BIN(15, d15)
#undef PG_SYM_BIN
    __syncthreads();
    {
      uint4 *st = reinterpret_cast<uint4 *>(own + b * kRec);
      st[0] = r0; st[1] = r1; st[2] = r2; st[3] = r3; st[4] = r4;
    }
    if (__builtin_amdgcn_ballot_w64(nl > 16) != 0) {
      PG_SYM_CE(d0, d1) PG_SYM_CE(d2, d3) PG_SYM_CE(d4, d5) PG_SYM_CE(d6, d7) PG_SYM_CE(d8, d9) PG_SYM_CE(d10, d11) PG_SYM_CE(d12, d13) PG_SYM_CE(d14, d15)
      PG_SYM_CE(d0, d2) PG_SYM_CE(d1, d3) PG_SYM_CE(d4, d6) PG_SYM_CE(d5, d7) PG_SYM_CE(d8, d10) PG_SYM_CE(d9, d11) PG_SYM_CE(d12, d14) PG_SYM_CE(d13, d15)
      PG_SYM_CE(d1, d2) PG_SYM_CE(d5, d6) PG_SYM_CE(d9, d10) PG_SYM_CE(d13, d14) PG_SYM_CE(d0, d4) PG_SYM_CE(d1, d5) PG_SYM_CE(d2, d6) PG_SYM_CE(d3, d7)
      PG_SYM_CE(d8, d12) PG_SYM_CE(d9, d13) PG_SYM_CE(d10, d14) PG_SYM_CE(d11, d15) PG_SYM_CE(d2, d4) PG_SYM_CE(d3, d5) PG_SYM_CE(d10, d12) PG_SYM_CE(d11, d13)
      PG_SYM_CE(d1, d2) PG_SYM_CE(d3, d4) PG_SYM_CE(d5, d6) PG_SYM_CE(d9, d10) PG_SYM_CE(d11, d12) PG_SYM_CE(d13, d14) PG_SYM_CE(d0, d8) PG_SYM_CE(d1, d9)
      PG_SYM_CE(d2, d10) PG_SYM_CE(d3, d11) PG_SYM_CE(d4, d12) PG_SYM_CE(d5, d13) PG_SYM_CE(d6, d14) PG_SYM_CE(d7, d15) PG_SYM_CE(d4, d8) PG_SYM_CE(d5, d9)
      PG_SYM_CE(d6, d10) PG_SYM_CE(d7, d11) PG_SYM_CE(d2, d4) PG_SYM_CE(d3, d5) PG_SYM_CE(d6, d8) PG_SYM_CE(d7, d9) PG_SYM_CE(d10, d12) PG_SYM_CE(d11, d13)
      PG_SYM_CE(d1, d2) PG_SYM_CE(d3, d4) PG_SYM_CE(d5, d6) PG_SYM_CE(d7, d8) PG_SYM_CE(d9, d10) PG_SYM_CE(d11, d12) PG_SYM_CE(d13, d14)
    }
    int pos = 0;
    u32 head = has ? own[b * kRec + off] : 0xFFFFFFFFu, res = 0xFFFFFFFFu;
    for (int r = 0; r <= k; ++r) {
      u32 m = head < d0 ? head : d0, x;
      x = PG_SYM_ROR(m, 8); m = x < m ? x : m;
      x = PG_SYM_ROR(m, 4); m = x < m ? x : m;
      x = PG_SYM_ROR(m, 2); m = x < m ? x : m;
      x = PG_SYM_ROR(m, 1); m = x < m ? x : m;
      const bool any = m != 0xFFFFFFFFu;
      if (any && head == m) {
        ++pos;
        head = pos < k1 ? own[b * kRec + off + pos] : 0xFFFFFFFFu;
      }
      const bool dwin = any && d0 == m;
      d0 = dwin ? d1 : d0; d1 = dwin ? d2 : d1; d2 = dwin ? d3 : d2; d3 = dwin ? d4 : d3;
      d4 = dwin ? d5 : d4; d5 = dwin ? d6 : d5; d6 = dwin ? d7 : d6; d7 = dwin ? d8 : d7;
      d8 = dwin ? d9 : d8; d9 = dwin ? d10 : d9; d10 = dwin ? d11 : d10; d11 = dwin ? d12 : d11;
      d12 = dwin ? d13 : d12; d13 = dwin ? d14 : d13; d14 = dwin ? d15 : d14; d15 = dwin ? 0xFFFFFFFFu : d15;
      if (b == r - 1) res = m;
      if (b == 0 && mine) {
        if (r > 16) {
          idx[row * k + r - 1] = m == 0xFFFFFFFFu ? -1 : (int)(m & 0x00FFFFFFu);
          dist[row * k + r - 1] = (unsigned char)(m >> 24);
        }
        if (r == k && ((m >> 24) >= cap || cnt > capL || logged > capG)) evictRows[atomicAdd(evictCount, 1u)] = (u32)row;
      }
    }
    if (mine && b < k) {
      idx[row * k + b] = res == 0xFFFFFFFFu ? -1 : (int)(res & 0x00FFFFFFu);
      dist[row * k + b] = (unsigned char)(res >> 24);
    }
  }
  __syncthreads();
  if (threadIdx.x == 0) {
    if (__hip_atomic_fetch_add(ticket, 1u, __ATOMIC_RELAXED, __HIP_MEMORY_SCOPE_AGENT) == gridDim.x - 1u) {
      u32 zero = 0u;
      asm volatile("" : "+v"(zero));
      const u32 evictedRows = __hip_atomic_fetch_add(evictCount, zero, __ATOMIC_RELAXED, __HIP_MEMORY_SCOPE_AGENT);
      *ticket = 0u;
      if (gv != 0u) *gate2 = gv;
      else if (evictedRows > limit) { *evictCount = 0u; *gate2 = 0u; }
      else *gate2 = 3u;
    }
  }
}

typedef int (*probe_fn)(int, const ProbeParams &, hipStream_t);
typedef int (*knn_rows_fn)(int, const KnnRowsParams &, int, hipStream_t);
static const knn_rows_fn kKnnRows[8] = {pg_launch_knn_rows_g1, pg_launch_knn_rows_g2, pg_launch_knn_rows_g3, pg_launch_knn_rows_g4,
                                        pg_launch_knn_rows_g5, pg_launch_knn_rows_g6, pg_launch_knn_rows_g7, pg_launch_knn_rows_g8};
static const probe_fn kProbe[8] = {pg_launch_probe_g1, pg_launch_probe_g2, pg_launch_probe_g3, pg_launch_probe_g4,
                                   pg_launch_probe_g5, pg_launch_probe_g6, pg_launch_probe_g7, pg_launch_probe_g8};
static int run_probe(const NsqParams &e, int l, int bits, u32 near, u32 lo, u32 span, u32 need, void *workspace, hipStream_t s,
                     const PgKnobs &kn, const u32 **gate) {
  if (!workspace) return pg_fail(PG_E_BADARG, "workspace required (pg_workspace_bytes)");
  u32 *gates = (u32 *)((char *)workspace + PG_WS_GATES), *counts = (u32 *)((char *)workspace + PG_WS_COUNTS);
  ProbeParams pp;
  pp.rowPlanes = e.rowPlanes; pp.colPlanes = e.colPlanes; pp.rowNpad = e.rowNpad; pp.colNpad = e.colNpad;
  pp.row0 = e.row0; pp.nrows = e.nrows; pp.ncols = e.ncols;
  pp.nsample = e.nrows < PG_PROBE_ROWS ? (int)e.nrows : PG_PROBE_ROWS;
  pp.wavesPerRow = PG_PROBE_WAVES;
  if (kn.probeS.v > 0) pp.nsample = (int)kn.probeS.v;
  if (kn.probeW.v > 0) pp.wavesPerRow = (int)kn.probeW.v;
  pp.near = near; pp.lo = lo; pp.span = span; pp.counts = counts;
  if (int rc = pg_launched(kProbe[pg_ngroups(l) - 1](bits, pp, s), "pg_probe_kernel")) return rc;
  const int force = (int)kn.gateForce.v;
  static_assert(PG_WS_GATES / 4 <= 1024, "pg_decide_kernel zeroes one word per thread");
  pg_decide_kernel<<<dim3(1), dim3(1024), 0, s>>>(counts, pp.nsample, pp.wavesPerRow, need, e.ncols, force, gates, (u32 *)workspace,
                                                  PG_WS_GATES / 4);
  if (int rc = pg_launched("pg_decide_kernel")) return rc;
  *gate = gates;
  return 0;
}

typedef int (*nsq_fn)(int, int, const NsqParams &, int, hipStream_t);
typedef int (*dense_fn)(int, const DenseParams &, hipStream_t);
typedef int (*compact_fn)(int, const CompactParams &, hipStream_t);
typedef int (*occ_fn)(int, int);
static const occ_fn kNsqOcc[8] = {pg_occ_nsq_g1, pg_occ_nsq_g2, pg_occ_nsq_g3, pg_occ_nsq_g4,
                                  pg_occ_nsq_g5, pg_occ_nsq_g6, pg_occ_nsq_g7, pg_occ_nsq_g8};
static int nsq_occupancy(int groups, int mode, int bits) {
  static std::atomic<int> cache[8][3][2];
  std::atomic<int> &c = cache[groups - 1][mode][bits == 8];
  int v = c.load(std::memory_order_relaxed);
  if (v == 0) {
    const int n = kNsqOcc[groups - 1](mode, bits);
    v = n < 1 ? 4 : (n > 8 ? 8 : n);
    c.store(v, std::memory_order_relaxed);
  }
  return v;
}
static const nsq_fn kNsq[8] = {pg_launch_nsq_g1, pg_launch_nsq_g2, pg_launch_nsq_g3, pg_launch_nsq_g4,
                               pg_launch_nsq_g5, pg_launch_nsq_g6, pg_launch_nsq_g7, pg_launch_nsq_g8};
static const dense_fn kDense[8] = {pg_launch_dense_g1, pg_launch_dense_g2, pg_launch_dense_g3, pg_launch_dense_g4,
                                   pg_launch_dense_g5, pg_launch_dense_g6, pg_launch_dense_g7, pg_launch_dense_g8};
static const compact_fn kCompact[8] = {pg_launch_compact_g1, pg_launch_compact_g2, pg_launch_compact_g3,
                                       pg_launch_compact_g4, pg_launch_compact_g5, pg_launch_compact_g6,
                                       pg_launch_compact_g7, pg_launch_compact_g8};

static void set_rows_plan(NsqParams *p, int *grid, const PassPlan &pl, const PgKnobs &kn) {
  if (kn.debugPlan.set) fprintf(stderr, "[pg plan] rows=%lld occ=%d rows_per_wave=%lld waves=%lld\n", (long long)p->nrows, pl.occ, (long long)pl.rowsPerWave, pl.passes);
  p->rowsPerWave = pl.rowsPerWave; p->rowsPerPass = pl.rowsPerPass;
  *grid = pl.grid;
}
static int plan_rows_here(NsqParams *p, int *grid, int occ, double recBytes, const PgKnobs &kn, int maxRows = PG_RB) {
  const int cus = cu_count();
  if (cus <= 0) return pg_fail(PG_E_NODEV, "no HIP device");
  set_rows_plan(p, grid, plan_rows(p->nrows, p->ncols, cus, occ, recBytes, kn, maxRows), kn);
  return 0;
}

extern "C" {

int pg_pack_planes(const void *src, int elem_bytes, int64_t n, int l, int64_t ld, const int64_t *rows, int bits,
                   void *planes, int64_t npad, uint32_t *flags, void *stream) {
  if (!src || !planes || !flags || n < 0 || ld < l) return pg_fail(PG_E_BADARG, "pg_pack_planes: bad argument");
  if (int rc = check_bits(bits)) return rc;
  if (int rc = check_l(l, bits, true)) return rc;
  if (npad < n || npad % 256) return pg_fail(PG_E_BADARG, "pg_pack_planes: npad must be pg_npad(n)");
  const int ng = pg_ngroups(l), nq = pg_nchunks(l, bits);
  hipStream_t s = (hipStream_t)stream;
  hipError_t e = hipMemsetAsync(flags, 0, sizeof(uint32_t), s);
  if (e != hipSuccess) return pg_launched((int)e, "hipMemsetAsync");
  const dim3 grid((unsigned)(npad / PG_PACK_SEQS)), block(256);
  const long long *r = (const long long *)rows;
  u32 *pl = (u32 *)planes;
#define PG_PACK(T)                                                                                          \
  do {                                                                                                      \
    if (bits == 5) pg_pack_kernel<T, 5><<<grid, block, 0, s>>>((const T *)src, n, l, ld, r, pl, npad, ng, nq, flags); \
    else pg_pack_kernel<T, 8><<<grid, block, 0, s>>>((const T *)src, n, l, ld, r, pl, npad, ng, nq, flags); \
  } while (0)
  switch (elem_bytes) {
    case 1: PG_PACK(unsigned char); break;
    case 2: PG_PACK(short); break;
    case 4: PG_PACK(int); break;
    case 8: PG_PACK(long long); break;
    default: return pg_fail(PG_E_BADARG, "pg_pack_planes: elem_bytes must be 1, 2, 4 or 8");
  }
#undef PG_PACK
  return pg_launched("pg_pack_kernel");
}

int pg_pack_bytes(const uint8_t *src, int64_t n, int width, int64_t ld, const int64_t *rows, const uint8_t *lut256, int bits,
                  void *planes, int64_t npad, uint8_t *tokens_out, uint32_t *flags, void *stream) {
  if (!src || !lut256 || !planes || !flags || n < 0 || ld < width) return pg_fail(PG_E_BADARG, "pg_pack_bytes: bad argument");
  if (int rc = check_bits(bits)) return rc;
  if (int rc = check_l(width, bits, true)) return rc;
  if (npad < n || npad % 256) return pg_fail(PG_E_BADARG, "pg_pack_bytes: npad must be pg_npad(n)");
  const int ng = pg_ngroups(width), nq = pg_nchunks(width, bits);
  hipStream_t s = (hipStream_t)stream;
  hipError_t e = hipMemsetAsync(flags, 0, sizeof(uint32_t), s);
  if (e != hipSuccess) return pg_launched((int)e, "hipMemsetAsync");
  const dim3 grid((unsigned)(npad / PG_PACK_SEQS)), block(256);
  if (bits == 5)
    pg_pack_kernel<unsigned char, 5><<<grid, block, 0, s>>>(src, n, width, ld, (const long long *)rows, (u32 *)planes, npad, ng, nq,
                                                            flags, lut256, tokens_out);
  else
    pg_pack_kernel<unsigned char, 8><<<grid, block, 0, s>>>(src, n, width, ld, (const long long *)rows, (u32 *)planes, npad, ng, nq,
                                                            flags, lut256, tokens_out);
  return pg_launched("pg_pack_kernel(bytes)");
}

int pg_hamming_dense(const void *x_planes, int64_t n, int64_t x_npad, const void *y_planes, int64_t m, int64_t y_npad,
                     int l, int bits, void *out, int out_elem_bytes, int64_t ldo, int accumulate, void *stream) {
  if (!x_planes || !y_planes || !out || n <= 0 || m <= 0 || ldo < n)
    return pg_fail(PG_E_BADARG, "pg_hamming_dense: bad argument");
  if (int rc = check_bits(bits)) return rc;
  if (int rc = check_l(l, bits)) return rc;
  if (out_elem_bytes != 1 && out_elem_bytes != 2 && out_elem_bytes != 4 && out_elem_bytes != 8)
    return pg_fail(PG_E_BADARG, "pg_hamming_dense: out_elem_bytes must be 1, 2, 4 or 8");
  if (x_npad < n || x_npad % 256 || y_npad < m) return pg_fail(PG_E_BADARG, "pg_hamming_dense: bad npad");
  if ((m + PG_RBD - 1) / PG_RBD > 65535) return pg_fail(PG_E_BADARG, "pg_hamming_dense: m too large for one launch");
  DenseParams p;
  p.xPlanes = (const uint4 *)x_planes; p.xNpad = x_npad; p.n = n;
  p.yPlanes = (const uint4 *)y_planes; p.yNpad = y_npad; p.m = m;
  p.out = out; p.ldo = ldo; p.outBytes = out_elem_bytes; p.accumulate = accumulate ? 1 : 0;
  return pg_launched(kDense[pg_ngroups(l) - 1](bits, p, (hipStream_t)stream), "pg_dense_kernel");
}

static int fill_nsq(NsqParams *p, const void *row_planes, int64_t row_npad, int64_t row0, int64_t nrows,
                    const void *col_planes, int64_t col_npad, int64_t ncols, int l, int bits, const PgKnobs &kn) {
  if (!row_planes || !col_planes || row0 < 0 || nrows <= 0 || ncols <= 0) return pg_fail(PG_E_BADARG, "bad argument");
  if (int rc = check_bits(bits)) return rc;
  if (int rc = check_l(l, bits)) return rc;
  if (col_npad < ncols || col_npad % 256 || row_npad < row0 + nrows) return pg_fail(PG_E_BADARG, "bad npad");
  if (ncols > 0x7fffffffLL) return pg_fail(PG_E_TOOMANY, "ncols exceeds int32 indices");
  memset(p, 0, sizeof(*p));
  p->filter = (int)kn.lbFilter.v;
  p->rowPlanes = (const uint4 *)row_planes; p->rowNpad = row_npad; p->row0 = row0; p->nrows = nrows;
  p->colPlanes = (const uint4 *)col_planes; p->colNpad = col_npad; p->ncols = ncols;
  p->colSig = p->colPlanes + (long long)pg_nchunks(l, bits) * col_npad;
  p->colFold = p->colSig + 2 * col_npad;
  p->rowFold = p->rowPlanes + ((long long)pg_nchunks(l, bits) + 2) * row_npad;
  return 0;
}

#ifdef PG_MM_STATS
static unsigned long long *g_stats = nullptr;
extern "C" int pg_debug_stats(unsigned long long *out12, int reset) {
  const size_t nst = PG_NSTAT + 2 * 65536;
  if (!g_stats) { if (hipMalloc(&g_stats, nst * 8) != hipSuccess) return -1; hipMemset(g_stats, 0, nst * 8); }
  if (out12) { hipDeviceSynchronize(); hipMemcpy(out12, g_stats, (reset & 2 ? nst : PG_NSTAT) * 8, hipMemcpyDeviceToHost); }
  if (reset & 1) hipMemset(g_stats, 0, nst * 8);
  return 0;
}
#endif
typedef int (*mm_sym_fn)(const NsqParams &, int, hipStream_t);
static const mm_sym_fn kMmSym[8] = {pg_launch_mm_knn_sym_g1, pg_launch_mm_knn_sym_g2, pg_launch_mm_knn_sym_g3, pg_launch_mm_knn_sym_g4,
                                    pg_launch_mm_knn_sym_g5, pg_launch_mm_knn_sym_g6, pg_launch_mm_knn_sym_g7, pg_launch_mm_knn_sym_g8};
static const nsq_fn kMm[8] = {pg_launch_mm_g1, pg_launch_mm_g2, pg_launch_mm_g3, pg_launch_mm_g4,
                              pg_launch_mm_g5, pg_launch_mm_g6, pg_launch_mm_g7, pg_launch_mm_g8};
static int mm_occupancy(int groups, int mode, int bits) {
  static std::atomic<int> cache[8][5][2];
  std::atomic<int> &c = cache[groups - 1][mode][bits == 8];
  int v = c.load(std::memory_order_relaxed);
  if (v == 0) {
    const int n = kMm[groups - 1](mode, bits, NsqParams(), -1, nullptr);
    v = n < 1 ? 4 : (n > 4 ? 4 : n);
    c.store(v, std::memory_order_relaxed);
  }
  return v;
}
static void set_mm_plan(NsqParams *p, int *grid, int64_t nrows, const PassPlan &pl, const PgKnobs &kn) {
  p->rowsPerWave = pl.rowsPerWave; p->rowsPerPass = pl.rowsPerPass;
  p->mmTailFrom = pl.tailFrom; p->mmTailRows = pl.tailRows;
  if (kn.debugPlan.set) fprintf(stderr, "[pg plan mm] rows=%lld: %lld passes of %lld rows + %lld of %lld\n", (long long)nrows, pl.tailFrom, (long long)pl.rowsPerWave, pl.passes - pl.tailFrom, (long long)pl.tailRows);
  p->mmDenseL1 = (int)kn.mmL1.v;
  p->mmDenseL2 = (int)kn.mmL2.v;
  p->mmDirectRun = (int)kn.mmRun.v;
#ifdef PG_MM_STATS
  if (!g_stats) pg_debug_stats(nullptr, 1);
  p->stats = g_stats;
#endif
  p->mmPasses = pl.passes; p->mmGridWaves = pl.gridWaves;
  if (grid) *grid = pl.grid;
}
static int pass_counter(NsqParams *p, void *workspace, hipStream_t s, bool probed = false) {
  if (!workspace) return pg_fail(PG_E_BADARG, "workspace required (pg_workspace_bytes)");
  unsigned *c = (unsigned *)workspace;
  if (!probed) {
    const hipError_t e = hipMemsetAsync(c, 0, PG_WS_GATES, s);
    if (e != hipSuccess) return pg_launched((int)e, "workspace: hipMemsetAsync");
  }
  p->mmPassCounter = c;
  return 0;
}

int pg_eps_slots(const void *row_planes, int64_t row_npad, int64_t row0, int64_t nrows, const void *col_planes,
                 int64_t col_npad, int64_t ncols, int l, int bits, int cmp, double eps, int cap, int32_t *slot_idx,
                 uint8_t *slot_w, uint32_t *counts, void *workspace, void *stream) {
  NsqParams p;
  const PgKnobs kn = read_knobs();
  if (int rc = fill_nsq(&p, row_planes, row_npad, row0, nrows, col_planes, col_npad, ncols, l, bits, kn)) return rc;
  if (!slot_idx || !slot_w || !counts || cap < 0 || cmp < PG_CMP_LE || cmp > PG_CMP_GT)
    return pg_fail(PG_E_BADARG, "pg_eps_slots: bad argument");
  eps_interval(cmp, eps, &p.lo, &p.span);
  p.hi1 = (p.lo > 0xFFFFFF00u - 1u) ? 0u : p.lo + p.span + 1u;
  p.cap = (u32)cap; p.slotIdx = slot_idx; p.slotW = slot_w; p.counts = counts;
  int grid = 0;
  p.epsOrdered = kn.epsOrdered.v != 0;
  if (use_mm_engine(nrows, kn, l, false)) {
    set_mm_plan(&p, &grid, nrows, plan_mm(nrows, cu_count(), kn), kn);
    if (int rc = pass_counter(&p, workspace, (hipStream_t)stream)) return rc;
    return pg_launched(kMm[pg_ngroups(l) - 1](PG_MODE_EPS, bits, p, grid, (hipStream_t)stream), "pg_mm_kernel(eps)");
  }
  if (int rc = plan_rows_here(&p, &grid, nsq_occupancy(pg_ngroups(l), PG_MODE_EPS, bits), 16.0 * pg_nchunks(l, bits), kn)) return rc;
  return pg_launched(kNsq[pg_ngroups(l) - 1](PG_MODE_EPS, bits, p, grid, (hipStream_t)stream), "pg_nsq_kernel(eps)");
}

int pg_eps_slots_sym(const void *planes, int64_t npad, int64_t n, int l, int bits, int cmp, double eps, int cap,
                     int32_t *slot_idx, uint8_t *slot_w, uint32_t *counts_up, uint32_t *counts_lo, void *workspace,
                     void *stream) {
  NsqParams p;
  const PgKnobs kn = read_knobs();
  if (int rc = fill_nsq(&p, planes, npad, 0, n, planes, npad, n, l, bits, kn)) return rc;
  if (!slot_idx || !slot_w || !counts_up || !counts_lo || cap < 0 || cmp < PG_CMP_LE || cmp > PG_CMP_GT)
    return pg_fail(PG_E_BADARG, "pg_eps_slots_sym: bad argument");
  if (n >= (1ll << 27)) return pg_fail(PG_E_TOOMANY, "pg_eps_slots_sym: n must be below 2^27");
  eps_interval(cmp, eps, &p.lo, &p.span);
  p.hi1 = (p.lo > 0xFFFFFF00u - 1u) ? 0u : p.lo + p.span + 1u;
  p.cap = (u32)cap; p.slotIdx = slot_idx; p.slotW = slot_w; p.counts = counts_up; p.countsLo = counts_lo;
  hipError_t e = hipMemsetAsync(counts_lo, 0, (size_t)n * sizeof(uint32_t), (hipStream_t)stream);
  if (e != hipSuccess) return pg_launched((int)e, "hipMemsetAsync");
  int grid = 0;
  if (probe_enabled(kn) && n >= PG_PROBE_MIN_N) {
    const u32 *gate = nullptr;
    if (int rc = run_probe(p, l, bits, 0u, p.lo, p.span, 1u, workspace, (hipStream_t)stream, kn, &gate)) return rc;
    NsqParams r = p;
    r.countsLo = nullptr;
    r.gate = gate + 1; r.gateMask = 1u << 1;
    int rgrid = 0;
    if (int rc = plan_rows_here(&r, &rgrid, nsq_occupancy(pg_ngroups(l), PG_MODE_EPS, bits), 16.0 * pg_nchunks(l, bits), kn)) return rc;
    if (int rc = pg_launched(kNsq[pg_ngroups(l) - 1](PG_MODE_EPS, bits, r, rgrid, (hipStream_t)stream), "pg_nsq_kernel(eps, gated)")) return rc;
    p.gate = gate + 1; p.gateMask = 1u << 0;
  }
  p.epsOrdered = kn.epsOrdered.v != 0;
  if (use_mm_engine(n, kn, l, false)) {
    long long rs = (n + 6399) / 6400;
    rs = (rs + 1) / 2 * 2;
    rs = rs < 8 ? 8 : (rs > PG_MM_RB ? PG_MM_RB : rs);
    const bool fine = pg_nchunks(l, bits) <= 3 && kn.mmPlan.v != 2;
    set_mm_plan(&p, &grid, n, plan_mm(n, cu_count(), kn, PG_MM_RB, 4, false, fine ? (int)rs : 0), kn);
    if (int rc = pass_counter(&p, workspace, (hipStream_t)stream, p.gate != nullptr)) return rc;
    return pg_launched(kMm[pg_ngroups(l) - 1](PG_MODE_EPS_SYM, bits, p, grid, (hipStream_t)stream), "pg_mm_kernel(eps sym)");
  }
  if (!kn.rowsPerWave.set && !kn.wavesPerCu.set) {
    const long long r = n >= 80000 ? 16 : 8;
    p.rowsPerWave = (int)r; p.rowsPerPass = (int)r;
    grid = (int)(((n + r - 1) / r + PG_WG_WAVES - 1) / PG_WG_WAVES);
  } else if (int rc = plan_rows_here(&p, &grid, nsq_occupancy(pg_ngroups(l), PG_MODE_EPS_SYM, bits), 16.0 * pg_nchunks(l, bits), kn, 16)) {
    return rc;
  }
  return pg_launched(kNsq[pg_ngroups(l) - 1](PG_MODE_EPS_SYM, bits, p, grid, (hipStream_t)stream), "pg_nsq_kernel(eps sym)");
}

int pg_eps_compact_sym(const void *planes, int64_t npad, int64_t n, int l, int bits, int cmp, double eps, int cap,
                       const int32_t *slot_idx, const uint8_t *slot_w, const uint32_t *counts_up,
                       const uint32_t *counts_lo, const int64_t *indptr, int32_t *indices, uint8_t *weights,
                       int leave_overflow, void *stream) {
  CompactParams c;
  c.skipOverflow = leave_overflow ? 1 : 0;
  if (int rc = fill_nsq(&c.e, planes, npad, 0, n, planes, npad, n, l, bits, read_knobs())) return rc;
  if (!slot_idx || !slot_w || !counts_up || !counts_lo || !indptr || cap < 0 || cmp < PG_CMP_LE || cmp > PG_CMP_GT)
    return pg_fail(PG_E_BADARG, "pg_eps_compact_sym: bad argument");
  eps_interval(cmp, eps, &c.e.lo, &c.e.span);
  c.e.hi1 = c.e.lo + c.e.span + 1u;
  c.e.cap = (u32)cap;
  c.e.slotIdx = const_cast<int *>(slot_idx);
  c.e.slotW = const_cast<unsigned char *>(slot_w);
  c.e.counts = const_cast<u32 *>(counts_up);
  c.e.countsLo = const_cast<u32 *>(counts_lo);
  c.indptr = (const long long *)indptr; c.indices = indices; c.weights = weights;
  return pg_launched(kCompact[pg_ngroups(l) - 1](bits, c, (hipStream_t)stream), "pg_compact_kernel(sym)");
}

int64_t pg_scan_scratch_bytes(int64_t n) {
  const int64_t nb = (n + PG_SCAN_TILE - 1) / PG_SCAN_TILE;
  return (nb + 2) * (int64_t)sizeof(long long);
}

int pg_exclusive_scan(const uint32_t *counts, int64_t n, int64_t *indptr, void *scratch, void *stream) {
  if (!counts || !indptr || !scratch || n <= 0) return pg_fail(PG_E_BADARG, "pg_exclusive_scan: bad argument");
  hipStream_t s = (hipStream_t)stream;
  const long long nb = (n + PG_SCAN_TILE - 1) / PG_SCAN_TILE;
  long long *part = (long long *)scratch;
  pg_scan_partials<u32><<<dim3((unsigned)nb), dim3(256), 0, s>>>(counts, n, part);
  pg_scan_single<<<dim3(1), dim3(256), 0, s>>>(part, nb);
  pg_scan_apply<u32, 0><<<dim3((unsigned)nb), dim3(256), 0, s>>>(counts, n, part, nb, (long long *)indptr, nullptr);
  return pg_launched("pg_scan");
}

int pg_eps_compact(const void *row_planes, int64_t row_npad, int64_t row0, int64_t nrows, const void *col_planes,
                   int64_t col_npad, int64_t ncols, int l, int bits, int cmp, double eps, int cap,
                   const int32_t *slot_idx, const uint8_t *slot_w, const uint32_t *counts, const int64_t *indptr,
                   int32_t *indices, uint8_t *weights, int leave_overflow, void *stream) {
  CompactParams c;
  c.skipOverflow = leave_overflow ? 1 : 0;
  if (int rc = fill_nsq(&c.e, row_planes, row_npad, row0, nrows, col_planes, col_npad, ncols, l, bits, read_knobs())) return rc;
  if (!slot_idx || !slot_w || !counts || !indptr || cap < 0 || cmp < PG_CMP_LE || cmp > PG_CMP_GT)
    return pg_fail(PG_E_BADARG, "pg_eps_compact: bad argument");
  eps_interval(cmp, eps, &c.e.lo, &c.e.span);
  c.e.hi1 = c.e.lo + c.e.span + 1u;
  c.e.cap = (u32)cap;
  c.e.slotIdx = const_cast<int *>(slot_idx);
  c.e.slotW = const_cast<unsigned char *>(slot_w);
  c.e.counts = const_cast<u32 *>(counts);
  c.indptr = (const long long *)indptr; c.indices = indices; c.weights = weights;
  return pg_launched(kCompact[pg_ngroups(l) - 1](bits, c, (hipStream_t)stream), "pg_compact_kernel");
}

int pg_eps_fill_rows(const void *row_planes, int64_t row_npad, int64_t row0, const int64_t *row_list, int64_t n_list,
                     const void *col_planes, int64_t col_npad, int64_t ncols, int l, int bits, int cmp, double eps,
                     const int64_t *indptr, int32_t *indices, uint8_t *weights, uint32_t *scratch_counts, void *workspace,
                     void *stream) {
  NsqParams p;
  if (!row_list || n_list <= 0) return pg_fail(PG_E_BADARG, "pg_eps_fill_rows: bad argument");
  const PgKnobs kn = read_knobs();
  if (int rc = fill_nsq(&p, row_planes, row_npad, row0, n_list, col_planes, col_npad, ncols, l, bits, kn)) return rc;
  if (!indptr || !indices || !weights || !scratch_counts || cmp < PG_CMP_LE || cmp > PG_CMP_GT)
    return pg_fail(PG_E_BADARG, "pg_eps_fill_rows: bad argument");
  eps_interval(cmp, eps, &p.lo, &p.span);
  p.hi1 = (p.lo > 0xFFFFFF00u - 1u) ? 0u : p.lo + p.span + 1u;
  p.cap = 0xFFFFFFFFu;
  p.rowList = (const long long *)row_list; p.fillIndptr = (const long long *)indptr;
  p.slotIdx = indices; p.slotW = weights; p.counts = scratch_counts;
  int grid = 0;
  set_mm_plan(&p, &grid, n_list, plan_mm(n_list, cu_count(), kn), kn);
  if (int rc = pass_counter(&p, workspace, (hipStream_t)stream)) return rc;
  return pg_launched(kMm[pg_ngroups(l) - 1](PG_MODE_EPS, bits, p, grid, (hipStream_t)stream), "pg_mm_kernel(eps fill)");
}

struct KnnRun {
  const KnnPlan &pl;
  const PgKnobs &kn;
  NsqParams p;
  int l, bits, ng, k;
  int64_t row0, nrows;
  int32_t *idx;
  uint8_t *dist;
  void *workspace;
  hipStream_t stream;
  u32 *gates() const { return (u32 *)((char *)workspace + PG_WS_GATES); }
};
static KnnHw knn_hw(const KnnShape &s, const PgKnobs &kn) {
  const int ng = pg_ngroups(s.l);
  const bool shortList = knn_short_list(s, kn);
  KnnHw hw;
  hw.cus = cu_count();
  hw.occValu = nsq_occupancy(ng, PG_MODE_KNN, s.bits);
  hw.occMm32 = mm_occupancy(ng, shortList ? PG_MODE_KNN_SHORT : PG_MODE_KNN, s.bits);
  hw.occMm64 = shortList ? mm_occupancy(ng, PG_MODE_KNN_SHORT2, s.bits) : 0;
  static std::atomic<int> occCache[8];
  int occS = occCache[ng - 1].load(std::memory_order_relaxed);
  if (occS == 0) {
    const int n = kMmSym[ng - 1](NsqParams(), -1, nullptr);
    occS = n < 1 ? 4 : (n > 4 ? 4 : n);
    occCache[ng - 1].store(occS, std::memory_order_relaxed);
  }
  hw.occSym = occS;
  return hw;
}
static int launch_valu(const KnnRun &r, bool gated) {
  NsqParams q = r.p;
  if (gated) { q.knnGuess = r.pl.guessValu; q.gate = r.gates(); q.gateMask = 1u << 1; }
  if (r.pl.valu.grid <= 0) return pg_fail(PG_E_NODEV, "no HIP device");
  int grid = 0;
  set_rows_plan(&q, &grid, r.pl.valu, r.kn);
  return pg_launched(kNsq[r.ng - 1](PG_MODE_KNN, r.bits, q, grid, r.stream), "pg_nsq_kernel(knn)");
}
static int launch_sym(const KnnRun &r) {
  const KnnPlan &pl = r.pl;
  char *base = (char *)r.workspace + pl.symBase;
  NsqParams s = r.p;
  s.nrows = r.nrows;
  s.gateMask = pl.symGateMask;
  SymArgs sa;
  sa.plan = (const int4 *)(base + pl.symWs.plan); sa.partial = (u32 *)(base + pl.symWs.partial);
  sa.lowCount = (u32 *)(base + pl.symWs.lowCount); sa.lowKeys = (u32 *)(base + pl.symWs.lowKeys);
  sa.capL = pl.symCapL;
  sa.deliver = pl.symDeliver;
  sa.rowBits = pl.symRowBits;
  pg_sym_set(&s, sa);
  s.mmEvict = nullptr; s.mmEvictRows = nullptr; s.mmPieces = 0; s.mmPieceFrom = 0; s.mmPartial = nullptr;
  s.rowsPerWave = 2 * PG_MM_RB; s.rowsPerPass = 2 * PG_MM_RB; s.mmTailFrom = pl.symPasses; s.mmTailRows = 2 * PG_MM_RB;
  s.mmPasses = pl.symPasses;
  s.mmGridWaves = pl.symGridWaves;
  s.mmPassCounter = r.p.mmPassCounter + 16;
  u32 *pieceStart = (u32 *)(base + pl.symWs.pieceStart), *gate2 = r.gates() + 2;
  if (r.kn.debugPlan.set) fprintf(stderr, "[pg plan sym] rows=%lld: %lld passes for %lld slots\n", (long long)r.nrows, pl.symPasses, pl.symSlots);
  pg_knn_sym_plan_kernel<<<dim3(pl.symPlanGrid), dim3(1024), 0, r.stream>>>(pl.symNb, pl.symNst, pl.symSlots, pl.symPiece, pl.symPieceMin, (int4 *)(base + pl.symWs.plan),
                                                                            pieceStart, (uint4 *)sa.lowCount, pl.symZero4);
  if (int rc = pg_launched("pg_knn_sym_plan_kernel")) return rc;
  if (int rc = pg_launched(kMmSym[r.ng - 1](s, (int)(s.mmGridWaves / PG_WG_WAVES), r.stream), "pg_mm_knn_sym_kernel")) return rc;
  pg_knn_sym_merge_kernel<<<dim3(pl.symMergeGrid), dim3(PG_WG_THREADS), 0, r.stream>>>(
      sa.partial, pieceStart, sa.lowCount, sa.lowKeys, sa.capL, sa.rowBits, r.nrows, r.k, r.idx, r.dist, r.p.knnGuess, r.p.mmEvict,
      r.p.mmEvictRows, s.gate, s.gateMask, gate2, r.p.mmPassCounter + 17, (u32)(pl.symLimit < 0 ? 0 : pl.symLimit));
  return pg_launched("pg_knn_sym_merge_kernel");
}
static int launch_main(KnnRun &r) {
  const KnnPlan &pl = r.pl;
  NsqParams &p = r.p;
  if (!pl.split) return pg_launched(kMm[r.ng - 1](pl.mode, r.bits, p, pl.launch.grid, r.stream), "pg_mm_kernel(knn)");
  const long long rem = r.nrows - pl.mainRows;
  p.nrows = r.nrows;
  p.mmPieces = pl.pieces; p.mmPieceFrom = pl.main.passes; p.mmPartial = (u32 *)((char *)r.workspace + PG_WS_PARTIAL);
  p.mmPasses = pl.launch.passes;
  p.mmTailFrom = pl.launch.tailFrom; p.mmTailRows = pl.launch.tailRows;
  p.mmGridWaves = pl.launch.gridWaves;
  if (int rc = pg_launched(kMm[r.ng - 1](pl.mode, r.bits, p, pl.launch.grid, r.stream), "pg_mm_kernel(knn + column pieces)")) return rc;
  pg_knn_merge_kernel<<<dim3(pl.pieceMergeGrid), dim3(PG_WG_THREADS), 0, r.stream>>>(
      p.mmPartial, rem, pl.pieces, r.k, r.idx + pl.mainRows * r.k, r.dist + pl.mainRows * r.k, p.knnGuess, p.mmEvict, p.mmEvictRows,
      (long long)r.row0 + pl.mainRows, p.gate, p.gateMask);
  return pg_launched("pg_knn_merge_kernel");
}
static int launch_alt32(const KnnRun &r) {
  NsqParams q = r.p;
  q.nrows = r.nrows;
  q.mmPieces = 0; q.mmPieceFrom = 0; q.mmPartial = nullptr;
  q.mmEvict = nullptr; q.mmEvictRows = nullptr;
  set_mm_plan(&q, nullptr, r.nrows, r.pl.alt, r.kn);
  q.mmPassCounter = r.p.mmPassCounter + 8;
  q.gateMask = 1u << 2;
  return pg_launched(kMm[r.ng - 1](PG_MODE_KNN_SHORT, r.bits, q, r.pl.alt.grid, r.stream), "pg_mm_kernel(knn, 32-row passes, gated)");
}
static int launch_evicted(const KnnRun &r) {
  const NsqParams &p = r.p;
  KnnRowsParams kr;
  kr.rowPlanes = p.rowPlanes; kr.colPlanes = p.colPlanes; kr.rowNpad = p.rowNpad; kr.colNpad = p.colNpad; kr.ncols = p.ncols;
  kr.count = p.mmEvict; kr.rows = p.mmEvictRows; kr.baseRow = r.row0; kr.k = r.k;
  kr.knnIdx = r.idx; kr.knnDist = r.dist; kr.gate = p.gate; kr.gateMask = r.pl.evictGateMask;
  return pg_launched(kKnnRows[r.ng - 1](r.bits, kr, r.pl.evictGrid, r.stream), "pg_knn_rows_kernel");
}

static int knn_launch(const void *row_planes, int64_t row_npad, int64_t row0, int64_t nrows, const void *col_planes,
                      int64_t col_npad, int64_t ncols, int l, int bits, int k, int first, const uint32_t *floor_keys,
                      uint32_t *last_keys, int32_t *idx_out, uint8_t *dist_out, void *workspace, void *stream) {
  const PgKnobs kn = read_knobs();
  NsqParams p;
  if (int rc = fill_nsq(&p, row_planes, row_npad, row0, nrows, col_planes, col_npad, ncols, l, bits, kn)) return rc;
  if (!idx_out || !dist_out) return pg_fail(PG_E_BADARG, "pg_knn_hamming: bad argument");
  if (k < 1 || first < 0 || first > 1 || first + k > 64) return pg_fail(PG_E_BADARG, "pg_knn_hamming: k out of range");
  if (ncols > PG_MAX_N_KNN) return pg_fail(PG_E_TOOMANY, "pg_knn_hamming: ncols exceeds 2^24");
  KnnShape shape;
  shape.nrows = nrows; shape.ncols = ncols; shape.row0 = row0;
  shape.samePlanes = row_planes == col_planes && row_npad == col_npad;
  shape.l = l; shape.bits = bits; shape.k = k; shape.first = first;
  shape.floorKeys = floor_keys != nullptr; shape.lastKeys = last_keys != nullptr; shape.workspace = workspace != nullptr;
  const KnnPlan pl = knn_plan(shape, knn_hw(shape, kn), kn);

  p.k = k; p.knnFirst = first; p.floorKeys = floor_keys; p.lastKeys = last_keys;
  p.knnGuess = pl.guess;
  p.knnIdx = idx_out; p.knnDist = dist_out;
  KnnRun r = {pl, kn, p, l, bits, pg_ngroups(l), k, row0, nrows, idx_out, dist_out, workspace, (hipStream_t)stream};
  if (!pl.mm) return launch_valu(r, false);
  if (pl.probe) {
    const u32 *gate = nullptr;
    if (int rc = run_probe(r.p, l, bits, pl.guess, 1u, 0u, (u32)(first + k), workspace, r.stream, kn, &gate)) return rc;
    if (int rc = launch_valu(r, true)) return rc;
    r.p.gate = gate;
  }
  r.p.gateMask = pl.mainGateMask;
  set_mm_plan(&r.p, nullptr, pl.mainRows, pl.main, kn);
  r.p.nrows = pl.mainRows;
  if (int rc = pass_counter(&r.p, workspace, r.stream, pl.probe)) return rc;
  if (pl.evict) {
    r.p.mmEvict = (u32 *)workspace + 1;
    r.p.mmEvictRows = (u32 *)((char *)workspace + pl.evictOffset);
  }
  if (pl.sym) {
    if (int rc = launch_sym(r)) return rc;
    r.p.gate = r.gates() + 2;
  }
  if (pl.split) {
    if (int rc = launch_main(r)) return rc;
  }
  if (pl.alt32) {
    if (int rc = launch_alt32(r)) return rc;
  }
  if (!pl.split) {
    if (int rc = launch_main(r)) return rc;
  }
  return pl.evict ? launch_evicted(r) : 0;
}

int pg_knn_hamming(const void *row_planes, int64_t row_npad, int64_t row0, int64_t nrows, const void *col_planes,
                   int64_t col_npad, int64_t ncols, int l, int bits, int k, int32_t *idx_out, uint8_t *dist_out,
                   void *workspace, void *stream) {
  if (k < 1 || k > PG_MAX_K) return pg_fail(PG_E_BADARG, "pg_knn_hamming: k must be in 1..63");
  return knn_launch(row_planes, row_npad, row0, nrows, col_planes, col_npad, ncols, l, bits, k, 1, nullptr, nullptr,
                    idx_out, dist_out, workspace, stream);
}

int pg_knn_hamming_round(const void *row_planes, int64_t row_npad, int64_t row0, int64_t nrows, const void *col_planes,
                         int64_t col_npad, int64_t ncols, int l, int bits, int k, int first_round,
                         const uint32_t *floor_keys, uint32_t *last_keys, int32_t *idx_out, uint8_t *dist_out,
                         void *workspace, void *stream) {
  if (!last_keys || (!first_round && !floor_keys)) return pg_fail(PG_E_BADARG, "pg_knn_hamming_round: key arrays required");
  return knn_launch(row_planes, row_npad, row0, nrows, col_planes, col_npad, ncols, l, bits, k, first_round ? 1 : 0,
                    first_round ? nullptr : floor_keys, last_keys, idx_out, dist_out, workspace, stream);
}

}

#define PG_QUERY_TARGET_WG 2048
static int query_pieces(int64_t nq, int64_t ndb, int k) {
  const long long ngrp = (nq + PG_QUERY_RW - 1) / PG_QUERY_RW;
  const long long ntiles = (ndb + PG_QUERY_TILE - 1) / PG_QUERY_TILE;
  long long p = (PG_QUERY_TARGET_WG + ngrp - 1) / ngrp;
  const long long byTiles = (ntiles + 3) / 4, byLds = PG_QUERY_MERGE_KEYS / (k > 0 ? k : 1);
  if (p > byTiles) p = byTiles;
  if (p > byLds) p = byLds;
  return (int)(p < 1 ? 1 : p);
}

__global__ __launch_bounds__(PG_WG_THREADS) void pg_query_merge_kernel(const u32 *partial, int pieces, int k, int *idx,
                                                                       unsigned char *dist, u32 *lastKeys) {
  __shared__ u32 keys[PG_QUERY_MERGE_KEYS];
  __shared__ u32 lists[PG_WG_WAVES][64];
  const int lane = threadIdx.x & 63, wv = threadIdx.x >> 6;
  const long long q = blockIdx.x;
  const int n = pieces * k;
  const u32 *src = partial + q * (long long)n;
  for (int e = threadIdx.x; e < n; e += PG_WG_THREADS) keys[e] = src[e];
  __syncthreads();
  u32 l = 0xFFFFFFFFu, t = 0xFFFFFFFFu;
  for (int e0 = wv * 64; e0 < n; e0 += PG_WG_WAVES * 64) {
    const u32 key = e0 + lane < n ? keys[e0 + lane] : 0xFFFFFFFFu;
    u64 m = __builtin_amdgcn_ballot_w64(key < t);
    while (m) {
      const int j = __builtin_ctzll(m);
      m &= m - 1;
      const u32 x = (u32)__builtin_amdgcn_readlane((int)key, j);
      if (x < t) {
        const u32 prev = wave_shr1(l, 0u);
        l = (l <= x) ? l : (prev > x ? prev : x);
        t = (u32)__builtin_amdgcn_readlane((int)l, k - 1);
      }
    }
  }
  lists[wv][lane] = l;
  __syncthreads();
  if (wv != 0) return;
  for (int w = 1; w < PG_WG_WAVES; ++w) {
    const u32 other = lists[w][lane];
    u64 m = __builtin_amdgcn_ballot_w64(other < t && lane < k);
    while (m) {
      const int j = __builtin_ctzll(m);
      m &= m - 1;
      const u32 x = (u32)__builtin_amdgcn_readlane((int)other, j);
      if (x < t) {
        const u32 prev = wave_shr1(l, 0u);
        l = (l <= x) ? l : (prev > x ? prev : x);
        t = (u32)__builtin_amdgcn_readlane((int)l, k - 1);
      }
    }
  }
  if (lane < k) {
    idx[q * k + lane] = l == 0xFFFFFFFFu ? -1 : (int)(l & 0x00FFFFFFu);
    dist[q * k + lane] = (unsigned char)(l >> 24);
    if (lastKeys && lane == k - 1) lastKeys[q] = l;
  }
}

typedef int (*query_fn)(int, const QueryParams &, long long, hipStream_t);
static const query_fn kQuery[8] = {pg_launch_query_g1, pg_launch_query_g2, pg_launch_query_g3, pg_launch_query_g4,
                                   pg_launch_query_g5, pg_launch_query_g6, pg_launch_query_g7, pg_launch_query_g8};

extern "C" {

int64_t pg_query_workspace_bytes(int64_t nq, int64_t ndb, int k) {
  if (nq <= 0 || ndb <= 0 || k < 1 || k > 64) return 0;
  const int pieces = query_pieces(nq, ndb, k);
  return pieces > 1 ? (int64_t)nq * pieces * k * 4 : 0;
}

int pg_query_knn_hamming(const void *q_planes, int64_t nq, int64_t q_npad, const void *db_planes, int64_t ndb,
                         int64_t db_npad, int l, int bits, int k, const uint32_t *floor_keys, uint32_t *last_keys,
                         int32_t *idx_out, uint8_t *dist_out, void *workspace, int64_t workspace_bytes, void *stream) {
  if (!q_planes || !db_planes || !idx_out || !dist_out || nq <= 0 || ndb <= 0 || workspace_bytes < 0)
    return pg_fail(PG_E_BADARG, "pg_query_knn_hamming: bad argument");
  if (k < 1 || k > 64) return pg_fail(PG_E_BADARG, "pg_query_knn_hamming: k must be in 1..64");
  if (int rc = check_bits(bits)) return rc;
  if (int rc = check_l(l, bits)) return rc;
  if (q_npad < nq || db_npad < ndb || db_npad % 256) return pg_fail(PG_E_BADARG, "pg_query_knn_hamming: bad npad");
  if (ndb >= PG_MAX_N_KNN) return pg_fail(PG_E_TOOMANY, "pg_query_knn_hamming: ndb must be below 2^24");
  long long pieces = query_pieces(nq, ndb, k);
  const long long fit = workspace ? workspace_bytes / ((long long)nq * k * 4) : 0;
  if (pieces > fit) pieces = fit < 1 ? 1 : fit;
  if (pieces > PG_QUERY_MERGE_KEYS / k) pieces = PG_QUERY_MERGE_KEYS / k;
  QueryParams p;
  p.qPlanes = (const uint4 *)q_planes; p.dbPlanes = (const uint4 *)db_planes;
  p.qNpad = q_npad; p.dbNpad = db_npad; p.nq = nq; p.ndb = ndb;
  p.k = k; p.pieces = (int)pieces;
  const long long ntiles = (ndb + PG_QUERY_TILE - 1) / PG_QUERY_TILE;
  p.tilesPerPiece = (ntiles + pieces - 1) / pieces;
  p.pieces = (int)((ntiles + p.tilesPerPiece - 1) / p.tilesPerPiece);
  p.floorKeys = floor_keys; p.partial = (u32 *)workspace;
  p.knnIdx = idx_out; p.knnDist = dist_out; p.lastKeys = last_keys;
  const long long ngrp = (nq + PG_QUERY_RW - 1) / PG_QUERY_RW;
  if (ngrp * p.pieces > 0x7FFFFFFFll) return pg_fail(PG_E_TOOMANY, "pg_query_knn_hamming: too many queries for one launch");
  hipStream_t s = (hipStream_t)stream;
  if (int rc = pg_launched(kQuery[pg_ngroups(l) - 1](bits, p, ngrp * p.pieces, s), "pg_query_knn_kernel")) return rc;
  if (p.pieces == 1) return 0;
  if (nq > 0x7FFFFFFFll) return pg_fail(PG_E_TOOMANY, "pg_query_knn_hamming: too many queries for one launch");
  pg_query_merge_kernel<<<dim3((unsigned)nq), dim3(PG_WG_THREADS), 0, s>>>((const u32 *)workspace, p.pieces, k, idx_out,
                                                                             dist_out, last_keys);
  return pg_launched("pg_query_merge_kernel");
}

}

static long long query_eps_pieces(int64_t nq, int64_t ndb) {
  const long long ngrp = (nq + PG_QUERY_RW - 1) / PG_QUERY_RW;
  const long long ntiles = (ndb + PG_QUERY_TILE - 1) / PG_QUERY_TILE;
  long long p = (PG_QUERY_TARGET_WG + ngrp - 1) / ngrp;
  const long long byTiles = (ntiles + PG_WG_WAVES - 1) / PG_WG_WAVES;
  if (p > byTiles) p = byTiles;
  return p < 1 ? 1 : p;
}

typedef int (*query_eps_fn)(int, int, const QueryEpsParams &, long long, hipStream_t);
static const query_eps_fn kQueryEps[8] = {pg_launch_query_eps_g1, pg_launch_query_eps_g2, pg_launch_query_eps_g3,
                                          pg_launch_query_eps_g4, pg_launch_query_eps_g5, pg_launch_query_eps_g6,
                                          pg_launch_query_eps_g7, pg_launch_query_eps_g8};

static int query_eps_launch(const char *who, int fill, const void *q_planes, int64_t nq, int64_t q_npad,
                            const void *db_planes, int64_t ndb, int64_t db_npad, int l, int bits, int cmp, double eps,
                            int64_t nseg, QueryEpsParams &p, void *stream) {
  if (!q_planes || !db_planes || nq <= 0 || ndb <= 0 || cmp < PG_CMP_LE || cmp > PG_CMP_GT || !(eps == eps))
    return pg_fail(PG_E_BADARG, who);
  if (int rc = check_bits(bits)) return rc;
  if (int rc = check_l(l, bits)) return rc;
  if (q_npad < nq || db_npad < ndb || db_npad % 256) return pg_fail(PG_E_BADARG, "pg_query_eps: bad npad");
  if (ndb > 0x7FFFFFFFll) return pg_fail(PG_E_TOOMANY, "pg_query_eps: ndb must fit int32 column indices");
  const long long ntiles = (ndb + PG_QUERY_TILE - 1) / PG_QUERY_TILE;
  if (nseg < PG_WG_WAVES || nseg % PG_WG_WAVES || nseg / PG_WG_WAVES > ntiles)
    return pg_fail(PG_E_BADARG, "pg_query_eps: nseg must be 4 x pieces, with at most one piece per column tile");
  const long long ngrp = (nq + PG_QUERY_RW - 1) / PG_QUERY_RW;
  const long long pieces = nseg / PG_WG_WAVES;
  if (ngrp * pieces > 0x7FFFFFFFll) return pg_fail(PG_E_TOOMANY, "pg_query_eps: too many queries for one launch");
  p.qPlanes = (const uint4 *)q_planes; p.dbPlanes = (const uint4 *)db_planes;
  p.qNpad = q_npad; p.dbNpad = db_npad; p.nq = nq; p.ndb = ndb;
  eps_interval(cmp, eps, &p.lo, &p.span, 0);
  p.pieces = (int)pieces;
  p.tilesPerPiece = (ntiles + pieces - 1) / pieces;
  return pg_launched(kQueryEps[pg_ngroups(l) - 1](bits, fill, p, ngrp * pieces, (hipStream_t)stream),
                  fill ? "pg_query_eps_kernel(fill)" : "pg_query_eps_kernel(count)");
}

extern "C" {

int64_t pg_query_eps_segments(int64_t nq, int64_t ndb) {
  if (nq <= 0 || ndb <= 0) return 0;
  return query_eps_pieces(nq, ndb) * PG_WG_WAVES;
}

int pg_query_eps_count(const void *q_planes, int64_t nq, int64_t q_npad, const void *db_planes, int64_t ndb, int64_t db_npad,
                       int l, int bits, int cmp, double eps, int64_t nseg, uint32_t *seg_counts, void *stream) {
  if (!seg_counts) return pg_fail(PG_E_BADARG, "pg_query_eps_count: bad argument");
  QueryEpsParams p = {};
  p.segCounts = seg_counts;
  return query_eps_launch("pg_query_eps_count: bad argument", 0, q_planes, nq, q_npad, db_planes, ndb, db_npad, l, bits, cmp,
                          eps, nseg, p, stream);
}

int pg_query_eps_fill(const void *q_planes, int64_t nq, int64_t q_npad, const void *db_planes, int64_t ndb, int64_t db_npad,
                      int l, int bits, int cmp, double eps, int64_t nseg, const int64_t *seg_indptr, int32_t *indices,
                      uint8_t *weights, void *stream) {
  if (!seg_indptr || !indices || !weights) return pg_fail(PG_E_BADARG, "pg_query_eps_fill: bad argument");
  QueryEpsParams p = {};
  p.segIndptr = (const long long *)seg_indptr; p.indices = indices; p.weights = weights;
  return query_eps_launch("pg_query_eps_fill: bad argument", 1, q_planes, nq, q_npad, db_planes, ndb, db_npad, l, bits, cmp,
                          eps, nseg, p, stream);
}

int pg_index_flags(const void *planes, int64_t n, int64_t npad, int l, int bits, int64_t ref,
                   const uint32_t *want_dist, int pos_mode, const uint32_t *pos_mask, const uint32_t *not_mask,
                   uint8_t *dist_out, uint64_t *hist, uint8_t *flags, void *stream) {
  if (!planes || n <= 0 || npad < n || ref < 0 || ref >= n) return pg_fail(PG_E_BADARG, "pg_index_flags: bad argument");
  if (int rc = check_bits(bits)) return rc;
  if (int rc = check_l(l, bits)) return rc;
  if (pos_mode < 0 || pos_mode > 2 || (pos_mode && (!pos_mask || !not_mask)))
    return pg_fail(PG_E_BADARG, "pg_index_flags: bad position mode / masks");
  const dim3 grid((unsigned)((n + 255) / 256)), block(256);
  hipStream_t s = (hipStream_t)stream;
  if (bits == 5)
    pg_index_kernel<5><<<grid, block, 0, s>>>((const u32 *)planes, n, npad, pg_ngroups(l), ref, want_dist, pos_mode,
                                              pos_mask, not_mask, dist_out, (u64 *)hist, flags);
  else
    pg_index_kernel<8><<<grid, block, 0, s>>>((const u32 *)planes, n, npad, pg_ngroups(l), ref, want_dist, pos_mode,
                                              pos_mask, not_mask, dist_out, (u64 *)hist, flags);
  return pg_launched("pg_index_kernel");
}

int pg_lev_profile(const uint8_t *tokens, int64_t n, int l, int64_t ld, void *profiles, int64_t npad, int32_t *lens,
                   uint32_t *flags, void *stream) {
  if (!tokens || !profiles || !lens || !flags || n <= 0 || ld < l) return pg_fail(PG_E_BADARG, "pg_lev_profile: bad argument");
  if (int rc = check_l(l)) return rc;
  if (npad < n || npad % 256) return pg_fail(PG_E_BADARG, "pg_lev_profile: npad must be pg_npad(n)");
  hipStream_t s = (hipStream_t)stream;
  hipError_t e = hipMemsetAsync(flags, 0, sizeof(uint32_t), s);
  if (e != hipSuccess) return pg_launched((int)e, "hipMemsetAsync");
  return pg_launched(pg_launch_lev_profile(tokens, n, l, ld, (u32 *)profiles, npad, lens, flags, s), "pg_lev_profile_kernel");
}

int pg_lev_candidates(const void *profiles, int64_t npad, int64_t n, int64_t row0, int64_t nrows, int band, int cap,
                      int32_t *slot_idx, uint8_t *slot_w, uint32_t *counts, void *stream) {
  if (!profiles || !slot_idx || !slot_w || !counts || n <= 0 || nrows <= 0 || row0 < 0 || row0 + nrows > n || cap < 0)
    return pg_fail(PG_E_BADARG, "pg_lev_candidates: bad argument");
  if (band < 0 || band > PG_LEV_MAX_BAND) return pg_fail(PG_E_BADARG, "pg_lev_candidates: band must be in 0..8");
  if (npad < n || npad % 256) return pg_fail(PG_E_BADARG, "pg_lev_candidates: bad npad");
  if (n > 0x7fffffffLL) return pg_fail(PG_E_TOOMANY, "n exceeds int32 indices");
  NsqParams p;
  const PgKnobs kn = read_knobs();
  memset(&p, 0, sizeof(p));
  p.rowPlanes = (const uint4 *)profiles; p.rowNpad = npad; p.row0 = row0; p.nrows = nrows;
  p.colPlanes = (const uint4 *)profiles; p.colNpad = npad; p.ncols = n;
  p.lo = 0; p.span = 2u * (u32)band; p.hi1 = p.span + 1u;
  p.filter = (int)kn.lbFilter.v;
  p.cap = (u32)cap; p.slotIdx = slot_idx; p.slotW = slot_w; p.counts = counts;
  int grid = 0;
  static int bag_occ = 0;
  if (!bag_occ) { bag_occ = pg_occ_nsq_bag(); if (bag_occ < 1) bag_occ = 4; }
  if (int rc = plan_rows_here(&p, &grid, bag_occ, 48.0, kn)) return rc;
  return pg_launched(pg_launch_nsq_bag(p, grid, (hipStream_t)stream), "pg_nsq_kernel(bag)");
}

int pg_lev_candidates_sym(const void *profiles, int64_t npad, int64_t n, int band, int cap, int32_t *slot_idx,
                          uint8_t *slot_w, int32_t *slot_aux, uint32_t *counts_up, uint32_t *counts_lo, void *stream) {
  if (!profiles || !slot_idx || !slot_w || !counts_up || !counts_lo || n <= 0 || cap < 0)
    return pg_fail(PG_E_BADARG, "pg_lev_candidates_sym: bad argument");
  if (band < 0 || band > PG_LEV_MAX_BAND) return pg_fail(PG_E_BADARG, "pg_lev_candidates_sym: band must be in 0..8");
  if (npad < n || npad % 256) return pg_fail(PG_E_BADARG, "pg_lev_candidates_sym: bad npad");
  if (n >= (1ll << 27)) return pg_fail(PG_E_TOOMANY, "pg_lev_candidates_sym: n must be below 2^27");
  NsqParams p;
  const PgKnobs kn = read_knobs();
  memset(&p, 0, sizeof(p));
  p.rowPlanes = (const uint4 *)profiles; p.rowNpad = npad; p.row0 = 0; p.nrows = n;
  p.colPlanes = (const uint4 *)profiles; p.colNpad = npad; p.ncols = n;
  p.lo = 0; p.span = 2u * (u32)band; p.hi1 = p.span + 1u;
  p.filter = (int)kn.lbFilter.v;
  p.cap = (u32)cap; p.slotIdx = slot_idx; p.slotW = slot_w; p.slotAux = slot_aux; p.counts = counts_up; p.countsLo = counts_lo;
  hipError_t e = hipMemsetAsync(counts_lo, 0, (size_t)n * sizeof(uint32_t), (hipStream_t)stream);
  if (e != hipSuccess) return pg_launched((int)e, "hipMemsetAsync");
  long long r = n >= 80000 ? 16 : 8;
  if (kn.rowsPerWave.v > 0) r = kn.rowsPerWave.v;
  p.rowsPerWave = (int)r; p.rowsPerPass = (int)(r > PG_RB ? PG_RB : r);
  const int grid = (int)(((n + r - 1) / r + PG_WG_WAVES - 1) / PG_WG_WAVES);
  return pg_launched(pg_launch_nsq_bag_sym(p, grid, (hipStream_t)stream), "pg_nsq_kernel(bag sym)");
}

int pg_lev_knn(const uint8_t *tokens, int64_t n, int l, int64_t ld, const void *planes128, int64_t npad,
               const int32_t *lens, int64_t row0, int64_t nrows,
               int band, int k, int cap, const int32_t *slot_idx, uint8_t *slot_w, const int32_t *slot_aux,
               const uint32_t *counts, const uint32_t *counts_lo, int32_t *idx_out, uint8_t *dist_out, void *stream) {
  if (!tokens || !planes128 || npad < n || npad % 256 || !lens || !slot_idx || !counts || !idx_out || !dist_out || n <= 0 || nrows <= 0 || row0 < 0 ||
      row0 + nrows > n || ld < l || cap < 0)
    return pg_fail(PG_E_BADARG, "pg_lev_knn: bad argument");
  if (int rc = check_l(l)) return rc;
  if (band < 0 || band > PG_LEV_MAX_BAND) return pg_fail(PG_E_BADARG, "pg_lev_knn: band must be in 0..8");
// ... 160 lines not shown
```

prograph_amd/csrc/pg_plan.h:

```cpp
#pragma once
#include "../../include/prograph_hip.h"

#include <math.h>
#include <stdint.h>
#include <stdlib.h>
#include <string.h>
#include <mutex>

#ifdef __HIPCC__
#define PG_HD __host__ __device__
#else
#define PG_HD
#endif

#ifndef PG_MODE_KNN_SHORT
enum { PG_MODE_EPS = 0, PG_MODE_KNN = 1, PG_MODE_EPS_SYM = 2 };
#define PG_MODE_KNN_SHORT 3
#define PG_MODE_KNN_SHORT2 4
#define PG_WG_WAVES 4
#define PG_RB 32
#define PG_RB_KNN 28
#define PG_MM_KL 20
#define PG_MM_RB 32
#define PG_MM_ST 128
#define PG_MM_DENSE_L1 56
#define PG_MM_DENSE_L2 48
#define PG_MM_DIRECT_RUN 8
#define PG_SYM_MAX_PIECES 16
#define PG_SYM_MAX_CAPL 256
#endif
static_assert(PG_MODE_KNN == 1 && PG_MODE_KNN_SHORT == 3 && PG_MODE_KNN_SHORT2 == 4 && PG_WG_WAVES == 4 && PG_RB == 32 &&
                  PG_RB_KNN == 28 && PG_MM_KL == 20 && PG_MM_RB == 32 && PG_MM_ST == 128 && PG_MM_DENSE_L1 == 56 &&
                  PG_MM_DENSE_L2 == 48 && PG_MM_DIRECT_RUN == 8 && PG_SYM_MAX_PIECES == 16 && PG_SYM_MAX_CAPL == 256,
              "pg_plan.h: the host-only copies of the engine's constants follow pg_common.h and pg_mm.h");

PG_HD static inline int sym_dist_bits(uint32_t cap) {
  int b = 0;
  for (uint32_t v = cap > 0 ? cap - 1u : 0u; v; v >>= 1) ++b;
  return b;
}
PG_HD static inline int sym_row_bits(uint32_t cap) { return 28 - sym_dist_bits(cap) < 24 ? 28 - sym_dist_bits(cap) : 24; }
PG_HD static inline bool sym_rows_fit(int64_t n, uint32_t cap) {
  const int rb = sym_row_bits(cap);
  return rb >= 1 && n <= ((int64_t)1 << rb);
}
PG_HD static inline uint32_t sym_entry(uint32_t place, uint32_t d, uint32_t row, int rowBits) { return place << 28 | d << rowBits | row; }
PG_HD static inline uint32_t sym_entry_place(uint32_t e) { return e >> 28; }
PG_HD static inline uint32_t sym_entry_key(uint32_t e, int rowBits) {
  return ((e & 0x0FFFFFFFu) >> rowBits) << 24 | (e & ((1u << rowBits) - 1u));
}
PG_HD static inline uint32_t sym_group_cap(uint32_t n, uint32_t first, uint32_t capL) {
  const uint32_t rows = n > first ? n - first : 0u;
  return (rows < 16u ? rows : 16u) * capL;
}

#define PG_PROBE_ROWS 64
#define PG_PROBE_WAVES 128
#define PG_PROBE_MIN_N 65536

static inline int plan_ngroups(int l) { return l <= 0 ? 1 : (l + 31) / 32; }
static inline int plan_nchunks(int l, int bits) { return (plan_ngroups(l) * bits + 3) / 4; }

struct PgKnob {
  bool set;
  long long v;
};
struct PgKnobs {
  PgKnob lbFilter, wavesPerCu, rowsPerWave, debugPlan, engine, engineMinRows, probe, probeS, probeW, gateForce, epsOrdered;
  PgKnob knnGuess, mmShort, mmR, mmSplit, mmEvict, mmPieces, mmPiecesAhead, mmPlan, mmTail, mmPersistent, mmL1, mmL2, mmRun;
  PgKnob knnSym, symCapL, symPiece, symPieceMin, symOcc, symDeliver, symEvictLimit, symMergeWgs;
};
enum { PG_ENGINE_AUTO = 0, PG_ENGINE_MFMA = 1, PG_ENGINE_VALU = 2 };
enum PgKnobRule { PG_KNOB_ANY, PG_KNOB_CLAMP, PG_KNOB_RANGE, PG_KNOB_WIDE, PG_KNOB_NAME };
struct PgKnobSpec {
  const char *name;
  PgKnob PgKnobs::*field;
  long long dflt, lo, hi;
  PgKnobRule rule;
  const char *what;
};
#define PG_KNOB_MAX 0x7fffffffll
static const PgKnobSpec kPgKnobs[] = {
    {"PG_LB_FILTER", &PgKnobs::lbFilter, 1, 0, 0, PG_KNOB_ANY, "stage-1 lower-bound filter: 1 adaptive, 0 off, 2 forced on"},
    {"PG_WAVES_PER_CU", &PgKnobs::wavesPerCu, 32, 4, 128, PG_KNOB_CLAMP, "VALU engine: size the row split for this many waves per CU (multiples of 4) instead of the cost rule"},
    {"PG_ROWS_PER_WAVE", &PgKnobs::rowsPerWave, 0, 1, PG_KNOB_MAX, PG_KNOB_RANGE, "uniform passes of that many rows (tuning sweeps); present: no column pieces, eps sym by plan_rows"},
    {"PG_DEBUG_PLAN", &PgKnobs::debugPlan, 0, 0, 0, PG_KNOB_ANY, "present: the [pg plan ...] lines on stderr"},
    {"PG_ENGINE", &PgKnobs::engine, PG_ENGINE_AUTO, 0, 0, PG_KNOB_NAME, "mfma / valu forces an engine; present: no probe"},
    {"PG_ENGINE_MIN_ROWS", &PgKnobs::engineMinRows, 0, 0, 0, PG_KNOB_WIDE, "rows from which the MFMA engine runs (default by kind of launch: use_mm_engine); present: no probe"},
    {"PG_PROBE", &PgKnobs::probe, 1, 0, 0, PG_KNOB_ANY, "0: no data probe, the size rules alone"},
    {"PG_PROBE_S", &PgKnobs::probeS, 0, 1, PG_PROBE_ROWS, PG_KNOB_RANGE, "sample rows of the probe (experiments)"},
    {"PG_PROBE_W", &PgKnobs::probeW, 0, 1, PG_PROBE_WAVES, PG_KNOB_RANGE, "waves per sample row of the probe (experiments)"},
    {"PG_GATE_FORCE", &PgKnobs::gateForce, -1, 0, 0, PG_KNOB_ANY, "the probe's decision is forced (tests): bit 0 gate[0], bit 1 gate[1]"},
    {"PG_EPS_ORDERED", &PgKnobs::epsOrdered, 0, 0, 0, PG_KNOB_ANY, "not 0: eps slots in column order (NsqParams::epsOrdered)"},
    {"PG_KNN_GUESS", &PgKnobs::knnGuess, 0, 0, 0, PG_KNOB_ANY, "the optimistic stage-1 cap (default by engine and length); present: no probe"},
    {"PG_MM_SHORT", &PgKnobs::mmShort, 1, 0, 0, PG_KNOB_ANY, "0: keep the 64-lane lists, no short-list instance (A/B runs)"},
    {"PG_MM_R", &PgKnobs::mmR, 0, 0, 0, PG_KNOB_ANY, "1 / 2 forces 32-row / 64-row passes; present: no gated 32-row alternative"},
    {"PG_MM_SPLIT", &PgKnobs::mmSplit, 1, 0, 0, PG_KNOB_ANY, "0: no column pieces, all rows in plain passes"},
    {"PG_MM_EVICT", &PgKnobs::mmEvict, 1, 0, 0, PG_KNOB_ANY, "0: rows that lose their cap finish inside the pass (no eviction, hence no pieces and no symmetric sweep)"},
    {"PG_MM_PIECES", &PgKnobs::mmPieces, 0, 2, 16, PG_KNOB_RANGE, "column pieces per row block (experiments; at most 8 beyond 64 row blocks)"},
    {"PG_MM_PIECES_AHEAD", &PgKnobs::mmPiecesAhead, 1, 0, 0, PG_KNOB_ANY, "0: the pieces always go through the pass counter"},
    {"PG_MM_PLAN", &PgKnobs::mmPlan, 0, 0, 0, PG_KNOB_ANY, "A/B of the pass rule: 2 = round 2's spreading rule everywhere, 1 = the waves-per-SIMD rule for eps too"},
    {"PG_MM_TAIL", &PgKnobs::mmTail, 0, 0, 0, PG_KNOB_ANY, "1: round 2's rule also shrinks the passes of the last round"},
    {"PG_MM_PERSISTENT", &PgKnobs::mmPersistent, 1, 0, 0, PG_KNOB_ANY, "0: one wave per pass instead of persistent waves"},
    {"PG_MM_L1", &PgKnobs::mmL1, PG_MM_DENSE_L1, 0, 0, PG_KNOB_ANY, "NsqParams::mmDenseL1"},
    {"PG_MM_L2", &PgKnobs::mmL2, PG_MM_DENSE_L2, 0, 0, PG_KNOB_ANY, "NsqParams::mmDenseL2"},
    {"PG_MM_RUN", &PgKnobs::mmRun, PG_MM_DIRECT_RUN, 1, PG_KNOB_MAX, PG_KNOB_CLAMP, "NsqParams::mmDirectRun"},
    {"PG_KNN_SYM", &PgKnobs::knnSym, -1, 0, 0, PG_KNOB_ANY, "symmetric kNN sweep: 0 off, 1 forced wherever the MFMA engine runs the short-list kNN"},
    {"PG_KNN_SYM_CAPL", &PgKnobs::symCapL, PG_SYM_MAX_CAPL, 8, PG_SYM_MAX_CAPL, PG_KNOB_CLAMP, "symmetric sweep: delivered keys per row"},
    {"PG_KNN_SYM_PIECE", &PgKnobs::symPiece, 0, 0, 0, PG_KNOB_ANY, "symmetric sweep: fixed piece length in super-tiles (default: guided)"},
    {"PG_KNN_SYM_PIECE_MIN", &PgKnobs::symPieceMin, 32, 4, PG_KNOB_MAX, PG_KNOB_CLAMP, "symmetric sweep: the guided rule's shortest piece"},
    {"PG_KNN_SYM_OCC", &PgKnobs::symOcc, 0, 1, 4, PG_KNOB_RANGE, "symmetric sweep: waves per SIMD the plan counts on"},
    {"PG_KNN_SYM_DELIVER", &PgKnobs::symDeliver, 1, 0, 0, PG_KNOB_ANY, "0: timing experiments, wrong results"},
    {"PG_KNN_SYM_EVICT_LIMIT", &PgKnobs::symEvictLimit, 0, 0, 0, PG_KNOB_WIDE, "evicted rows up to which the sweep's results stand (default: a sixteenth of the rows)"},
    {"PG_KNN_SYM_MERGE_WGS", &PgKnobs::symMergeWgs, 0, 1, PG_KNOB_MAX, PG_KNOB_RANGE, "workgroups of the sweep's merge at most (tests; default and bound: eight a CU)"},
};

static inline PgKnob pg_knob_parse(const PgKnobSpec &s, const char *text) {
  PgKnob k = {true, s.dflt};
  if (s.rule == PG_KNOB_NAME) {
    k.v = !strcmp(text, "mfma") ? PG_ENGINE_MFMA : (!strcmp(text, "valu") ? PG_ENGINE_VALU : PG_ENGINE_AUTO);
    return k;
  }
  const long long x = s.rule == PG_KNOB_WIDE ? atoll(text) : (long long)atoi(text);
  if (s.rule == PG_KNOB_CLAMP) k.v = x < s.lo ? s.lo : (x > s.hi ? s.hi : x);
  else if (s.rule == PG_KNOB_RANGE) k.v = x >= s.lo && x <= s.hi ? x : s.dflt;
  else k.v = x;
  return k;
}
static inline PgKnobs pg_knobs_read(const char *const *env) {
  PgKnobs kn;
  for (const PgKnobSpec &s : kPgKnobs) kn.*(s.field) = PgKnob{false, s.dflt};
  for (; env && *env; ++env) {
    const char *e = *env;
    if (e[0] != 'P' || e[1] != 'G' || e[2] != '_') continue;
    const char *eq = strchr(e, '=');
    if (!eq) continue;
    for (const PgKnobSpec &s : kPgKnobs)
      if (strlen(s.name) == (size_t)(eq - e) && !strncmp(s.name, e, (size_t)(eq - e))) {
        if (!(kn.*(s.field)).set) kn.*(s.field) = pg_knob_parse(s, eq + 1);
        break;
      }
  }
  return kn;
}

#define PG_WS_FLAGS 64
#define PG_WS_GATES 576
#define PG_WS_COUNTS 640
#define PG_WS_PARTIAL (PG_WS_COUNTS + 8 * 64 * 128)
#define PG_SPLIT_MAX_ROWS 8192
#define PG_SPLIT_MIN_ROWS 65536
#define PG_SYM_MIN_N 65536
#define PG_WS_PARTIAL_BYTES ((int64_t)PG_SPLIT_MAX_ROWS * 8 * PG_MM_KL * 4)
static_assert(PG_WS_COUNTS + 8 * PG_PROBE_ROWS * PG_PROBE_WAVES <= PG_WS_PARTIAL, "pg_workspace_bytes");
static inline int64_t ws_evict_offset(int64_t nrows) { return PG_WS_PARTIAL + (nrows > PG_SPLIT_MIN_ROWS ? PG_WS_PARTIAL_BYTES : 0); }
static inline int64_t ws_sym_offset(int64_t nrows) { return (ws_evict_offset(nrows) + 4 * (nrows > 0 ? nrows : 0) + 64 + 255) / 256 * 256; }

PG_HD static inline int sym_block_pieces(long long b, long long nst, long long slots, int piece, int pmin) {
  const long long len = nst - (b >> 1);
  const long long rem = len * (len + 1) - ((b & 1) ? len : 0);
  long long P = piece > 0 ? piece : (rem / (slots > 0 ? slots : 1)) & ~1ll;
  if (piece <= 0 && P < pmin) P = pmin;
  if (P < 3) P = 3;
  if (P > len) P = len > 3 ? len : 3;
  unsigned np = ((unsigned)len + (unsigned)P - 1u) / (unsigned)P;
  if (np > (unsigned)len / 3u) np = (unsigned)len / 3u;
  if (np > PG_SYM_MAX_PIECES) np = PG_SYM_MAX_PIECES;
  return np < 1 ? 1 : (int)np;
}
PG_HD static inline void sym_piece_range(long long b, long long nst, int np, int q, int *first, int *end) {
  const unsigned s0 = (unsigned)(b >> 1), len = (unsigned)nst - s0, unp = (unsigned)np, uq = (unsigned)q;
  *first = q == 0 ? (int)s0 : (int)(2u * ((s0 + len * uq / unp + 1u) / 2u));
  *end = q + 1 == np ? (int)nst : (int)(2u * ((s0 + len * (uq + 1u) / unp + 1u) / 2u));
}
static inline long long sym_plan_host(long long n, long long slots, int piece, int pmin, int32_t *out, long long cap) {
  const long long nb = (n + 63) / 64, nst = (n + PG_MM_ST - 1) / PG_MM_ST;
  struct Memo { long long n, slots, count; int piece, pmin; };
  static std::mutex memoLock;
  static Memo memo[4] = {};
  static int memoNext = 0;
  if (!out) {
    std::lock_guard<std::mutex> g(memoLock);
    for (const Memo &m : memo)
      if (m.n == n && m.slots == slots && m.piece == piece && m.pmin == pmin && m.count > 0) return m.count;
  }
  long long at = 0;
  for (long long b = 0; b < nb; ++b) {
    const int np = sym_block_pieces(b, nst, slots, piece, pmin);
    for (int q = 0; q < np; ++q, ++at) {
      if (!out || at >= cap) continue;
      int f, e;
      sym_piece_range(b, nst, np, q, &f, &e);
      out[4 * at] = (int)b; out[4 * at + 1] = f; out[4 * at + 2] = e; out[4 * at + 3] = q;
    }
  }
  if (!out) {
    std::lock_guard<std::mutex> g(memoLock);
    memo[memoNext] = Memo{n, slots, at, piece, pmin};
    memoNext = (memoNext + 1) % 4;
  }
  return at;
}
static inline long long sym_slots(int occ, int cus, const PgKnobs &kn) {
  if (kn.symOcc.v >= 1) occ = (int)kn.symOcc.v;
  return (long long)(cus > 0 ? cus : 256) * 4 * (occ < 1 ? 1 : (occ > 4 ? 4 : occ));
}
struct SymWs { int64_t plan, pieceStart, lowCount, partial, lowKeys, bytes; long long maxPasses; };
static inline SymWs sym_ws(int64_t n, int cus, const PgKnobs &kn) {
  SymWs w = {0, 0, 0, 0, 0, 0, 0};
  const int env = (int)kn.knnSym.v;
  if (n <= 0 || n > PG_MAX_N_KNN || env == 0 || (env != 1 && n < PG_SYM_MIN_N)) return w;
  auto up = [](int64_t x) { return (x + 255) / 256 * 256; };
  const long long nb = (n + 63) / 64;
  w.maxPasses = sym_plan_host(n, sym_slots(4, cus, kn), (int)kn.symPiece.v, (int)kn.symPieceMin.v, nullptr, 0);
  w.plan = 0;
  w.pieceStart = up(w.plan + 16 * w.maxPasses);
  w.lowCount = up(w.pieceStart + 4 * (nb + 1));
  w.partial = up(w.lowCount + 4 * n);
  w.lowKeys = up(w.partial + w.maxPasses * 64 * PG_MM_KL * 4);
  w.bytes = up(w.lowKeys + n * (int64_t)kn.symCapL.v * 4);
  return w;
}
static inline int64_t workspace_bytes(int64_t nrows, int cus, const PgKnobs &kn) { return ws_sym_offset(nrows) + sym_ws(nrows, cus, kn).bytes; }

struct PassPlan {
  int rowsPerWave, rowsPerPass;
  long long tailFrom;
  int tailRows;
  long long passes;
  long long gridWaves;
  int grid;
  int occ;
};

static inline int waves_per_cu(const PgKnobs &kn) { return (int)(kn.wavesPerCu.v / 4) * 4; }

static inline PassPlan plan_rows(int64_t nrows, int64_t ncols, int cus, int occ, double recBytes, const PgKnobs &kn, int maxRows = PG_RB) {
  long long rpw = 4;
  if (kn.wavesPerCu.set) {
    const long long maxWaves = (long long)cus * waves_per_cu(kn);
    rpw = (nrows + maxWaves - 1) / maxWaves;
    if (rpw < 1) rpw = 1;
    if (rpw >= 4) rpw = (rpw + 3) / 4 * 4;
  } else {
    static const long long kRound[9] = {0, 22, 31, 37, 43, 51, 60, 70, 80};
    if (occ < 1) occ = 1;
    if (occ > 8) occ = 8;
    const double matBytes = recBytes * (double)ncols;
    double bw = 13e12;
    if (matBytes > 0 && matBytes < 48e6) bw *= fmin(4.0, pow(48e6 / matBytes, 0.65));
    double best = -1;
    for (long long r = 4; r <= maxRows; r += 4) {
      const long long nw = (nrows + r - 1) / r;
      const long long wgs = (nw + PG_WG_WAVES - 1) / PG_WG_WAVES;
      const long long n = (wgs + cus - 1) / cus;
      const double valu = 1.21e-11 * (double)(((n / occ) * kRound[occ] + kRound[n % occ]) * (r + 1));
      const double stream = (double)nw * recBytes / bw;
      const double cost = valu > stream ? valu : stream;
      if (best < 0 || cost <= best * 1.0000001) { best = cost; rpw = r; }
    }
  }
  if (kn.rowsPerWave.v > 0) rpw = kn.rowsPerWave.v;
  const long long waves = (nrows + rpw - 1) / rpw;
  const long long passes = (rpw + maxRows - 1) / maxRows;
  PassPlan pl = {};
  pl.occ = occ;
  pl.rowsPerWave = (int)rpw;
  long long rpp = (rpw + passes - 1) / passes;
  if (rpp >= 4) rpp = (rpp + 3) / 4 * 4;
  if (rpp > maxRows) rpp = maxRows;
  pl.rowsPerPass = (int)rpp;
  pl.passes = waves;
  pl.grid = (int)((waves + PG_WG_WAVES - 1) / PG_WG_WAVES);
  pl.gridWaves = (long long)pl.grid * PG_WG_WAVES;
  return pl;
}

static inline bool use_mm_engine(int64_t nrows, const PgKnobs &kn, int l = 64, bool knn = true) {
  if (kn.engine.v == PG_ENGINE_MFMA) return true;
  if (kn.engine.v == PG_ENGINE_VALU) return false;
  const long long dflt = knn ? 20000 : (l <= 32 ? 36000 : 28000);
  const long long thr = kn.engineMinRows.set ? kn.engineMinRows.v : dflt;
  return nrows >= thr;
}

static inline PassPlan plan_mm(int64_t nrows, int cus, const PgKnobs &kn, int rb = PG_MM_RB, int occ = 4, bool knn = false, int uniformRows = 0) {
  long long rpw = rb, tailFrom = (nrows + rb - 1) / rb, tailRows = rb;
  const long long simds = (long long)(cus > 0 ? cus : 256) * 4;
  const long long slots = simds * (occ < 1 ? 1 : occ);
  const int planEnv = (int)kn.mmPlan.v;
  const bool oldPlan = planEnv == 2 || (!knn && planEnv != 1);
  if (kn.rowsPerWave.v > 0 || uniformRows > 0) {
    const int want = kn.rowsPerWave.v > 0 ? (int)kn.rowsPerWave.v : uniformRows;
    rpw = want < rb ? want : rb;
    tailFrom = (nrows + rpw - 1) / rpw; tailRows = rpw;
  } else if (!oldPlan) {
    if (tailFrom <= slots) {
      const long long w = (tailFrom + simds - 1) / simds;
      long long r = (nrows + w * simds - 1) / (w * simds);
      r = (r + 1) / 2 * 2;
      if (r < 4) r = 4;
      if (r > rb) r = rb;
      rpw = r; tailFrom = (nrows + r - 1) / r; tailRows = r;
    }
  } else {
    const long long full = nrows / (slots * rb) * slots;
    const long long rest = nrows - full * rb;
    if (rest > 0 && (full == 0 || kn.mmTail.v == 1)) {
      long long r = (long long)((double)rest / (0.97 * (double)slots)) + 1;
      r = (r + 1) / 2 * 2;
      if (r < 4) r = 4;
      if (r > rb) r = rb;
      if (full == 0 && r < 16) r = 16;
      tailFrom = full; tailRows = r;
    }
  }
  PassPlan pl = {};
  pl.occ = occ;
  pl.rowsPerWave = (int)rpw; pl.rowsPerPass = rb;
  pl.tailFrom = tailFrom; pl.tailRows = (int)tailRows;
  const long long headRows = tailFrom * rpw < nrows ? tailFrom * rpw : nrows;
  const long long waves = tailFrom + (nrows - headRows + tailRows - 1) / tailRows;
  long long gridWaves = waves < slots ? waves : slots;
  if (kn.mmPersistent.v == 0) gridWaves = waves;
  gridWaves = (gridWaves + PG_WG_WAVES - 1) / PG_WG_WAVES * PG_WG_WAVES;
  pl.passes = waves; pl.gridWaves = gridWaves;
  pl.grid = (int)(gridWaves / PG_WG_WAVES);
  return pl;
}

static inline double knn_plan_cost(long long nrows, long long ncols, int cus, int rb, int occ, bool canSplit, long long *mainRows) {
  static const double S1[4] = {0.43, 0.42, 0.37, 0.12}, H1[4] = {0.148, 0.200, 0.294, 0.477};
  static const double S2[4] = {0.64, 0.69, 0.64, 0.54}, H2[4] = {0.229, 0.292, 0.404, 0.557};
  const bool big = rb > PG_MM_RB;
  const double c = (double)ncols / 1e5, kPieces = 0.04 * c;
  auto T = [&](long long w) { return (big ? S2 : S1)[w - 1] + (big ? H2 : H1)[w - 1] * c; };
  const long long simds = (long long)(cus > 0 ? cus : 256) * 4;
  occ = occ < 1 ? 1 : (occ > 4 ? 4 : occ);
  const long long passes = (nrows + rb - 1) / rb, slots = simds * occ, maxRem = 128ll * rb;
  *mainRows = nrows;
  if (passes <= slots) {
    const long long w = (passes + simds - 1) / simds;
    if (canSplit && w >= 3 && nrows - (w - 1) * simds * rb <= maxRem) {
      *mainRows = (w - 1) * simds * rb;
      return T(w - 1) + kPieces;
    }
    return T(w);
  }
  const long long full = nrows / (slots * rb), rem = nrows - full * slots * rb;
  double t = (double)full * T(occ);
  if (rem > 0) {
    if (canSplit && rem <= maxRem) {
      *mainRows = full * slots * rb;
      t += kPieces;
    } else {
      t += T(((rem + rb - 1) / rb + simds - 1) / simds);
    }
  }
  return t;
}

static inline bool probe_enabled(const PgKnobs &kn) { return kn.probe.v != 0 && !kn.engine.set && !kn.engineMinRows.set; }

struct KnnShape {
  int64_t nrows, ncols, row0;
  bool samePlanes;
  int l, bits, k, first;
  bool floorKeys, lastKeys;
  bool workspace;
};
struct KnnHw {
  int cus;
  int occValu;
  int occMm32;
  int occMm64;
  int occSym;
};
struct KnnPlan {
  bool mm;
  uint32_t guess;
  uint32_t guessValu;
  bool probe;
  PassPlan valu;
  bool shortList, two;
  int mode, rb;
  long long mainRows;
  PassPlan main;
  PassPlan launch;
  uint32_t symGateMask, mainGateMask;
  bool evict;
  int64_t evictOffset;
  int evictGrid;
  uint32_t evictGateMask;
  bool split;
  long long nb;
  int pieces;
  bool piecesAhead;
  unsigned pieceMergeGrid;
  bool sym;
  long long symSlots, symPasses, symNb, symNst, symGridWaves, symLimit, symZero4;
  int symPiece, symPieceMin;
  uint32_t symCapL;
  int symRowBits;
  bool symDeliver;
  unsigned symPlanGrid, symMergeGrid;
  int64_t symBase;
  SymWs symWs;
  bool alt32;
  PassPlan alt;
};

static inline bool knn_short_list(const KnnShape &s, const PgKnobs &kn) {
  return s.first == 1 && s.k + 1 <= PG_MM_KL && !s.floorKeys && !s.lastKeys && kn.mmShort.v != 0;
}

static inline KnnPlan knn_plan(const KnnShape &s, const KnnHw &hw, const PgKnobs &kn) {
  KnnPlan pl = {};
  const int64_t nrows = s.nrows, ncols = s.ncols;
  const int filter = (int)kn.lbFilter.v, nq = plan_nchunks(s.l, s.bits);
  pl.mm = use_mm_engine(nrows, kn);
  const uint32_t guessMm = s.l > 32 ? 10u : 7u;
  pl.guessValu = 8u;
  pl.guess = kn.knnGuess.set ? (uint32_t)(int)kn.knnGuess.v : (pl.mm ? guessMm : pl.guessValu);
  if (filter == 0) pl.guess = 0;
  if (hw.cus > 0) pl.valu = plan_rows(nrows, ncols, hw.cus, hw.occValu, 16.0 * nq, kn, PG_RB_KNN);
  if (!pl.mm) return pl;
  pl.probe = probe_enabled(kn) && ncols >= PG_PROBE_MIN_N && nrows >= PG_PROBE_MIN_N / 2 && filter != 0 && !kn.knnGuess.set;
  pl.shortList = knn_short_list(s, kn);
  const int occ1 = hw.occMm32, occ2 = pl.shortList ? hw.occMm64 : 0;
  const bool evictOn = kn.mmEvict.v != 0;
  const bool canSplit = pl.shortList && s.workspace && evictOn && pl.guess > 0 && ncols >= 65536 && nrows > PG_SPLIT_MIN_ROWS &&
                        !kn.rowsPerWave.set && kn.mmSplit.v != 0;
  long long main1 = nrows, main2 = nrows;
  const double t1 = knn_plan_cost(nrows, ncols, hw.cus, PG_MM_RB, occ1, canSplit, &main1);
  const double t2 = pl.shortList ? knn_plan_cost(nrows, ncols, hw.cus, 2 * PG_MM_RB, occ2, canSplit, &main2) : 1e30;
  pl.two = pl.shortList && t2 < t1;
  if (kn.mmR.set) pl.two = pl.shortList && kn.mmR.v == 2;
  pl.rb = pl.two ? 2 * PG_MM_RB : PG_MM_RB;
  const int occm = pl.two ? occ2 : occ1;
  pl.mode = pl.two ? PG_MODE_KNN_SHORT2 : (pl.shortList ? PG_MODE_KNN_SHORT : PG_MODE_KNN);
  pl.mainRows = pl.two ? main2 : main1;
  pl.alt32 = pl.two && pl.probe && !kn.mmR.set;
  if (pl.probe) pl.mainGateMask = pl.alt32 ? (1u << 0) : ((1u << 0) | (1u << 2));
  pl.main = plan_mm(pl.mainRows, hw.cus, kn, pl.rb, occm, true);
  pl.launch = pl.main;
  pl.evict = s.first == 1 && !s.floorKeys && !s.lastKeys && pl.guess > 0 && evictOn;
  pl.evictOffset = ws_evict_offset(nrows);
  const long long rowsCap = (long long)(hw.cus > 0 ? hw.cus : 256) * 8;
  pl.evictGrid = (int)(nrows < rowsCap ? nrows : rowsCap);
  pl.symWs = sym_ws(nrows, hw.cus, kn);
  pl.symBase = ws_sym_offset(nrows);
  const bool sym = pl.shortList && pl.evict && s.bits == PG_BITS_5 && nq <= 3 && s.samePlanes && s.row0 == 0 && nrows == ncols &&
                   filter != 0 && pl.symWs.bytes > 0 && (kn.knnSym.v == 1 || pl.two) &&
                   sym_rows_fit(nrows, pl.guess);
  const long long symSlots = sym ? sym_slots(hw.occSym, hw.cus, kn) : 0;
  const long long symPasses = sym ? sym_plan_host(nrows, symSlots, (int)kn.symPiece.v, (int)kn.symPieceMin.v, nullptr, 0) : 0;
  pl.sym = sym && symPasses <= pl.symWs.maxPasses;
  if (pl.sym) {
    pl.symSlots = symSlots; pl.symPasses = symPasses;
    pl.symPiece = (int)kn.symPiece.v; pl.symPieceMin = (int)kn.symPieceMin.v;
    pl.symNb = (nrows + 63) / 64; pl.symNst = (nrows + PG_MM_ST - 1) / PG_MM_ST;
    pl.symGateMask = 1u << 0;
    pl.symCapL = (uint32_t)kn.symCapL.v;
    pl.symRowBits = sym_row_bits(pl.guess);
    pl.symDeliver = kn.symDeliver.v != 0;
    pl.symGridWaves = ((pl.symPasses < pl.symSlots ? pl.symPasses : pl.symSlots) + PG_WG_WAVES - 1) / PG_WG_WAVES * PG_WG_WAVES;
    pl.symZero4 = (nrows + 3) / 4;
    const long long zeroWgs = (pl.symZero4 + 1023) / 1024 < 64 ? (pl.symZero4 + 1023) / 1024 : 64;
    pl.symPlanGrid = (unsigned)(1 + zeroWgs);
    pl.symLimit = kn.symEvictLimit.set ? kn.symEvictLimit.v : nrows / 16;
    const long long mergeWgs = (nrows + 4 * PG_WG_WAVES - 1) / (4 * PG_WG_WAVES);
    long long mergeCap = rowsCap;
    if (kn.symMergeWgs.v >= 1 && kn.symMergeWgs.v < mergeCap) mergeCap = kn.symMergeWgs.v;
    pl.symMergeGrid = (unsigned)(mergeWgs < mergeCap ? mergeWgs : mergeCap);
    if (!pl.probe) pl.mainGateMask = (1u << 0) | (1u << 2);
  }
  pl.evictGateMask = pl.mainGateMask | (pl.sym ? 1u << 3 : 0u);
  pl.split = pl.mainRows < nrows;
  if (pl.split) {
    const long long rem = nrows - pl.mainRows, nb = (rem + pl.rb - 1) / pl.rb;
    const long long simds = (long long)(hw.cus > 0 ? hw.cus : 256) * 4;
    int pieces = (int)(simds / nb);
    pieces = pieces > 16 ? 16 : (pieces < 2 ? 2 : pieces);
    if (kn.mmPieces.v >= 2 && kn.mmPieces.v <= (nb <= 64 ? 16 : 8)) pieces = (int)kn.mmPieces.v;
    pl.nb = nb; pl.pieces = pieces;
    pl.launch.passes = pl.main.passes + nb * pieces;
    pl.launch.tailFrom = pl.launch.passes; pl.launch.tailRows = pl.rb;
    pl.piecesAhead = pl.main.passes + nb * pieces <= simds * occm && kn.mmPiecesAhead.v != 0;
    if (pl.piecesAhead) {
      pl.launch.gridWaves = (pl.launch.passes + PG_WG_WAVES - 1) / PG_WG_WAVES * PG_WG_WAVES;
      pl.launch.grid = (int)(pl.launch.gridWaves / PG_WG_WAVES);
    }
    pl.pieceMergeGrid = (unsigned)((rem + 4 * PG_WG_WAVES - 1) / (4 * PG_WG_WAVES));
  }
  if (pl.alt32) pl.alt = plan_mm(nrows, hw.cus, kn, PG_MM_RB, occ1, true);
  return pl;
}
```

Measured before the change: 41040 billion sequence-pairs/s.

## Fuse sym plan into decide launch, windowed merge pop, prefetch merge piece starts

The symmetric kNN plan kernel now runs as extra workgroups of the probe's decide kernel, which removes one launch. Its prefix scan now uses wave shuffles in place of a shared-memory Hillis-Steele loop. The merge kernel prefetches the next iteration's pieceStart and lowCount values, and its 16-register shift-pop becomes a templated window of width 4 that is refilled only when it empties, which cuts per-round select instructions. A device-side plan API is also added. The risks are extra register pressure and ballot/refill overhead in the merge, plus a coupling between the decide and plan launches.

```diff
diff --git a/include/prograph_hip.h b/include/prograph_hip.h
--- a/include/prograph_hip.h
+++ b/include/prograph_hip.h
@@ -87,6 +87,8 @@
                    void *workspace, void *stream);
 
 int64_t pg_knn_sym_plan(int64_t n, int64_t slots, int piece, int piece_min, int32_t *out, int64_t max_passes);
+int64_t pg_knn_sym_plan_device(int64_t n, int64_t slots, int piece, int piece_min, int32_t *plan_out,
+                               uint32_t *piece_start_out, int64_t max_passes, void *stream);
 
 int pg_knn_hamming_round(const void *row_planes, int64_t row_npad, int64_t row0, int64_t nrows,
                          const void *col_planes, int64_t col_npad, int64_t ncols, int l, int bits,
diff --git a/prograph_amd/_native.py b/prograph_amd/_native.py
--- a/prograph_amd/_native.py
+++ b/prograph_amd/_native.py
@@ -30,7 +30,7 @@
     "pg_version", "pg_last_error", "pg_device_info", "pg_npad", "pg_ngroups", "pg_nchunks", "pg_planes_bytes", "pg_workspace_bytes",
     "pg_pack_planes", "pg_pack_bytes",
     "pg_hamming_dense", "pg_eps_slots", "pg_scan_scratch_bytes", "pg_exclusive_scan",
-    "pg_eps_compact", "pg_eps_fill_rows", "pg_eps_slots_sym", "pg_eps_compact_sym", "pg_knn_hamming", "pg_knn_sym_plan", "pg_knn_hamming_round", "pg_index_flags", "pg_compact_flags",
+    "pg_eps_compact", "pg_eps_fill_rows", "pg_eps_slots_sym", "pg_eps_compact_sym", "pg_knn_hamming", "pg_knn_sym_plan", "pg_knn_sym_plan_device", "pg_knn_hamming_round", "pg_index_flags", "pg_compact_flags",
     "pg_lev_profile", "pg_lev_candidates", "pg_lev_candidates_sym", "pg_lev_knn", "pg_csr_row_stats",
     "pg_levenshtein_dense", "pg_lev_eps_pairs", "pg_lev_eps_count", "pg_lev_eps_fill",
     "pg_lev_long_pack", "pg_levenshtein_long_dense",
@@ -116,6 +116,8 @@
         lib.pg_knn_hamming.argtypes = [_vp, _i64, _i64, _i64, _vp, _i64, _i64, _i32, _i32, _i32, _vp, _vp, _vp, _vp]
         lib.pg_knn_sym_plan.restype = _i64
         lib.pg_knn_sym_plan.argtypes = [_i64, _i64, _i32, _i32, _vp, _i64]
+        lib.pg_knn_sym_plan_device.restype = _i64
+        lib.pg_knn_sym_plan_device.argtypes = [_i64, _i64, _i32, _i32, _vp, _vp, _i64, _vp]
         lib.pg_knn_hamming_round.argtypes = [_vp, _i64, _i64, _i64, _vp, _i64, _i64, _i32, _i32, _i32, _i32, _vp, _vp, _vp,
                                              _vp, _vp, _vp]
         lib.pg_query_workspace_bytes.restype = _i64
diff --git a/prograph_amd/csrc/pg_api.hip b/prograph_amd/csrc/pg_api.hip
--- a/prograph_amd/csrc/pg_api.hip
+++ b/prograph_amd/csrc/pg_api.hip
@@ -58,41 +58,86 @@
 
 }
 
-__global__ __launch_bounds__(1024) void pg_knn_sym_plan_kernel(long long nb, long long nst, long long slots, int piece, int pmin,
-                                                                int4 *plan, u32 *pieceStart, uint4 *zero, long long zero4) {
-  __shared__ u32 sums[1024];
-  const int t = threadIdx.x;
-  if (blockIdx.x > 0) {
-    for (long long i = (long long)(blockIdx.x - 1) * 1024 + t; i < zero4; i += (long long)(gridDim.x - 1) * 1024) zero[i] = make_uint4(0u, 0u, 0u, 0u);
+struct SymPlanArgs {
+  long long nb, nst, slots;
+  int piece, pmin;
+  int4 *plan;
+  u32 *pieceStart;
+  uint4 *zero;
+  long long zero4;
+  unsigned grid;
+};
+static __device__ __forceinline__ void sym_plan_workgroup(unsigned vb, unsigned vgrid, const SymPlanArgs &a) {
+  __shared__ u32 waveTotal[16];
+  const int t = threadIdx.x, lane = t & 63, wv = t >> 6;
+  if (vb > 0) {
+    for (long long i = (long long)(vb - 1) * 1024 + t; i < a.zero4; i += (long long)(vgrid - 1) * 1024) a.zero[i] = make_uint4(0u, 0u, 0u, 0u);
     return;
   }
-  const long long per = (nb + 1023) / 1024, b0 = t * per, b1 = b0 + per < nb ? b0 + per : nb;
-  u32 mine = 0;
-  for (long long b = b0; b < b1; ++b) mine += (u32)sym_block_pieces(b, nst, slots, piece, pmin);
-  sums[t] = mine;
+  const long long nb = a.nb, per = (nb + 1023) / 1024, b0 = t * per, b1 = b0 + per < nb ? b0 + per : nb;
+  const bool few = per <= 4;
+  u32 np4 = 0u, mine = 0;
+  if (few) {
+#pragma unroll 1
+    for (int j = 0; b0 + j < b1; ++j) {
+      const u32 np = (u32)sym_block_pieces(b0 + j, a.nst, a.slots, a.piece, a.pmin);
+      np4 |= np << (8 * j);
+      mine += np;
+    }
+  } else {
+#pragma clang loop vectorize(disable) interleave(disable) unroll(disable)
+    for (long long b = b0; b < b1; ++b) mine += (u32)sym_block_pieces(b, a.nst, a.slots, a.piece, a.pmin);
+  }
+  u32 incl = mine;
+#pragma unroll
+  for (int o = 1; o < 64; o <<= 1) {
+    const u32 x = (u32)__shfl_up((int)incl, o);
+    incl += lane >= o ? x : 0u;
+  }
+  if (lane == 63) waveTotal[wv] = incl;
   __syncthreads();
-  for (int o = 1; o < 1024; o <<= 1) {
-    const u32 x = t >= o ? sums[t - o] : 0u;
-    __syncthreads();
-    sums[t] += x;
-    __syncthreads();
-  }
-  u32 at = sums[t] - mine;
-  for (long long b = b0; b < b1; ++b) {
-    const int np = sym_block_pieces(b, nst, slots, piece, pmin);
-    pieceStart[b] = at;
+  u32 front = 0, total = 0;
+#pragma unroll
+  for (int i = 0; i < 16; ++i) {
+    const u32 x = waveTotal[i];
+    front += i < wv ? x : 0u;
+    total += x;
+  }
+  u32 at = front + incl - mine;
+  auto entries = [&](long long b, int np) {
+    a.pieceStart[b] = at;
+#pragma unroll 1
     for (int q = 0; q < np; ++q, ++at) {
       int f, e;
-      sym_piece_range(b, nst, np, q, &f, &e);
-      plan[at] = make_int4((int)b, f, e, q);
-    }
-  }
-  if (t == 1023) pieceStart[nb] = sums[1023];
-}
+      sym_piece_range(b, a.nst, np, q, &f, &e);
+      a.plan[at] = make_int4((int)b, f, e, q);
+    }
+  };
+  if (few) {
+#pragma unroll 1
+    for (int j = 0; b0 + j < b1; ++j) entries(b0 + j, (int)((np4 >> (8 * j)) & 0xFFu));
+  } else {
+#pragma clang loop vectorize(disable) interleave(disable) unroll(disable)
+    for (long long b = b0; b < b1; ++b) entries(b, sym_block_pieces(b, a.nst, a.slots, a.piece, a.pmin));
+  }
+  if (t == 1023) a.pieceStart[nb] = total;
+}
+__global__ __launch_bounds__(1024) void pg_knn_sym_plan_kernel(SymPlanArgs a) { sym_plan_workgroup(blockIdx.x, gridDim.x, a); }
 extern "C" {
 int64_t pg_knn_sym_plan(int64_t n, int64_t slots, int piece, int piece_min, int32_t *out, int64_t max_passes) {
   if (n <= 0 || slots <= 0) return pg_fail(PG_E_BADARG, "pg_knn_sym_plan: bad argument");
   return sym_plan_host(n, slots, piece, piece_min > 0 ? piece_min : (int)read_knobs().symPieceMin.v, out, max_passes);
+}
+int64_t pg_knn_sym_plan_device(int64_t n, int64_t slots, int piece, int piece_min, int32_t *plan_out, uint32_t *piece_start_out,
+                               int64_t max_passes, void *stream) {
+  if (n <= 0 || n > PG_MAX_N_KNN || slots <= 0 || !plan_out || !piece_start_out) return pg_fail(PG_E_BADARG, "pg_knn_sym_plan_device: bad argument");
+  const int pmin = piece_min > 0 ? piece_min : (int)read_knobs().symPieceMin.v;
+  const int64_t passes = sym_plan_host(n, slots, piece, pmin, nullptr, 0);
+  if (passes > max_passes) return pg_fail(PG_E_BADARG, "pg_knn_sym_plan_device: the plan has more passes than max_passes");
+  SymPlanArgs a = {(n + 63) / 64, (n + PG_MM_ST - 1) / PG_MM_ST, slots, piece, pmin, (int4 *)plan_out, piece_start_out, nullptr, 0, 1u};
+  pg_knn_sym_plan_kernel<<<dim3(1), dim3(1024), 0, (hipStream_t)stream>>>(a);
+  if (int rc = pg_launched("pg_knn_sym_plan_kernel")) return rc;
+  return passes;
 }
 }
 
@@ -381,7 +426,8 @@
 }
 
 __global__ __launch_bounds__(1024) void pg_decide_kernel(const u32 *counts, int nsample, int wavesPerRow, u32 need, long long ncols,
-                                                          int force, u32 *gate, u32 *line, int lineWords) {
+                                                          int force, u32 *gate, u32 *line, int lineWords, SymPlanArgs ride) {
+  if (blockIdx.x > 0) { sym_plan_workgroup(blockIdx.x - 1u, gridDim.x - 1u, ride); return; }
   __shared__ u32 sClustered[16];
   __shared__ unsigned long long sEps[16], sNear[16];
   const int tid = threadIdx.x, s = tid >> 4, sub = tid & 15;
@@ -455,6 +501,7 @@
 
 #define PG_SYM_ROR(x, N) ((u32)__builtin_amdgcn_update_dpp(0, (int)(x), 0x120 + (N), 0xF, 0xF, false))
 #define PG_SYM_CE(a, b) { const u32 x_ = a, y_ = b; a = x_ < y_ ? x_ : y_; b = x_ < y_ ? y_ : x_; }
+template <int W>
 __global__ __launch_bounds__(PG_WG_THREADS) __attribute__((amdgpu_waves_per_eu(7, 8))) void pg_knn_sym_merge_kernel(const u32 *partial, const u32 *pieceStart, const u32 *lowCount,
                                                                          const u32 *lowKeys, u32 capL, int rowBits, long long nrows, int k, int *idx,
                                                                          unsigned char *dist, u32 cap, u32 *evictCount, u32 *evictRows,
@@ -470,14 +517,18 @@
   const bool open = !gate || ((gateMask >> gv) & 1u);
   if (threadIdx.x < 4 * PG_WG_WAVES) binCount[0][threadIdx.x] = 0u;
   int trip = 0;
+  u32 hs0 = 0u, hs1 = 0u, hlogged = 0u;
+  if (open && (long long)blockIdx.x * (4 * PG_WG_WAVES) < nrows) {
+    const long long f0 = (long long)blockIdx.x * (4 * PG_WG_WAVES);
+    hs0 = pieceStart[f0 >> 6]; hs1 = pieceStart[(f0 >> 6) + 1]; hlogged = lowCount[f0];
+  }
   for (long long first = (long long)blockIdx.x * (4 * PG_WG_WAVES); open && first < nrows; first += (long long)gridDim.x * (4 * PG_WG_WAVES), trip ^= 1) {
     const int k1 = k + 1, off = kRec - k1;
-    const long long blk = first >> 6;
     const long long row = first + 4 * wv + g;
     const bool mine = row < nrows;
     const long long rowIn = mine ? row : first;
-    const u32 s0 = pieceStart[blk], s1 = pieceStart[blk + 1];
-    const u32 logged = lowCount[first];
+    const u32 s0 = hs0, s1 = hs1;
+    const u32 logged = (u32)__builtin_amdgcn_readfirstlane((int)hlogged);
     u32 np = s1 - s0;
     np = np > PG_SYM_MAX_PIECES ? PG_SYM_MAX_PIECES : np;
     u32 *own = &keys[wv][g][0];
@@ -506,10 +557,10 @@
     const u32 cnt = mine ? binCount[trip][4 * wv + g] : 0u;
     const int nl = (int)(cnt < capL ? cnt : capL);
     const u32 *low = &bins[4 * wv + g][b];
-    u32 d0, d1, d2, d3, d4, d5, d6, d7, d8, d9, d10, d11, d12, d13, d14, d15;
+    u32 d[16];
 #define PG_SYM_BIN(j, d) d = 16 * j + b < nl ? low[16 * j] : 0xFFFFFFFFu;
-    PG_SYM_BIN(0, d0) PG_SYM_BIN(1, d1) PG_SYM_BIN(2, d2) PG_SYM_BIN(3, d3) PG_SYM_BIN(4, d4) PG_SYM_BIN(5, d5) PG_SYM_BIN(6, d6) PG_SYM_BIN(7, d7)
-    PG_SYM_BIN(8, d8) PG_SYM_BIN(9, d9) PG_SYM_BIN(10, d10) PG_SYM_BIN(11, d11) PG_SYM_BIN(12, d12) PG_SYM_BIN(13, d13) PG_SYM_BIN(14, d14) PG_SYM_BIN(15, d15)
+    PG_SYM_BIN(0, d[0]) PG_SYM_BIN(1, d[1]) PG_SYM_BIN(2, d[2]) PG_SYM_BIN(3, d[3]) PG_SYM_BIN(4, d[4]) PG_SYM_BIN(5, d[5]) PG_SYM_BIN(6, d[6]) PG_SYM_BIN(7, d[7])
+    PG_SYM_BIN(8, d[8]) PG_SYM_BIN(9, d[9]) PG_SYM_BIN(10, d[10]) PG_SYM_BIN(11, d[11]) PG_SYM_BIN(12, d[12]) PG_SYM_BIN(13, d[13]) PG_SYM_BIN(14, d[14]) PG_SYM_BIN(15, d[15])
 #undef PG_SYM_BIN
     __syncthreads();
     {
@@ -517,19 +568,25 @@
       st[0] = r0; st[1] = r1; st[2] = r2; st[3] = r3; st[4] = r4;
     }
     if (__builtin_amdgcn_ballot_w64(nl > 16) != 0) {
-      PG_SYM_CE(d0, d1) PG_SYM_CE(d2, d3) PG_SYM_CE(d4, d5) PG_SYM_CE(d6, d7) PG_SYM_CE(d8, d9) PG_SYM_CE(d10, d11) PG_SYM_CE(d12, d13) PG_SYM_CE(d14, d15)
-      PG_SYM_CE(d0, d2) PG_SYM_CE(d1, d3) PG_SYM_CE(d4, d6) PG_SYM_CE(d5, d7) PG_SYM_CE(d8, d10) PG_SYM_CE(d9, d11) PG_SYM_CE(d12, d14) PG_SYM_CE(d13, d15)
-      PG_SYM_CE(d1, d2) PG_SYM_CE(d5, d6) PG_SYM_CE(d9, d10) PG_SYM_CE(d13, d14) PG_SYM_CE(d0, d4) PG_SYM_CE(d1, d5) PG_SYM_CE(d2, d6) PG_SYM_CE(d3, d7)
-      PG_SYM_CE(d8, d12) PG_SYM_CE(d9, d13) PG_SYM_CE(d10, d14) PG_SYM_CE(d11, d15) PG_SYM_CE(d2, d4) PG_SYM_CE(d3, d5) PG_SYM_CE(d10, d12) PG_SYM_CE(d11, d13)
-      PG_SYM_CE(d1, d2) PG_SYM_CE(d3, d4) PG_SYM_CE(d5, d6) PG_SYM_CE(d9, d10) PG_SYM_CE(d11, d12) PG_SYM_CE(d13, d14) PG_SYM_CE(d0, d8) PG_SYM_CE(d1, d9)
-      PG_SYM_CE(d2, d10) PG_SYM_CE(d3, d11) PG_SYM_CE(d4, d12) PG_SYM_CE(d5, d13) PG_SYM_CE(d6, d14) PG_SYM_CE(d7, d15) PG_SYM_CE(d4, d8) PG_SYM_CE(d5, d9)
-      PG_SYM_CE(d6, d10) PG_SYM_CE(d7, d11) PG_SYM_CE(d2, d4) PG_SYM_CE(d3, d5) PG_SYM_CE(d6, d8) PG_SYM_CE(d7, d9) PG_SYM_CE(d10, d12) PG_SYM_CE(d11, d13)
-      PG_SYM_CE(d1, d2) PG_SYM_CE(d3, d4) PG_SYM_CE(d5, d6) PG_SYM_CE(d7, d8) PG_SYM_CE(d9, d10) PG_SYM_CE(d11, d12) PG_SYM_CE(d13, d14)
-    }
-    int pos = 0;
+      PG_SYM_CE(d[0], d[1]) PG_SYM_CE(d[2], d[3]) PG_SYM_CE(d[4], d[5]) PG_SYM_CE(d[6], d[7]) PG_SYM_CE(d[8], d[9]) PG_SYM_CE(d[10], d[11]) PG_SYM_CE(d[12], d[13]) PG_SYM_CE(d[14], d[15])
+      PG_SYM_CE(d[0], d[2]) PG_SYM_CE(d[1], d[3]) PG_SYM_CE(d[4], d[6]) PG_SYM_CE(d[5], d[7]) PG_SYM_CE(d[8], d[10]) PG_SYM_CE(d[9], d[11]) PG_SYM_CE(d[12], d[14]) PG_SYM_CE(d[13], d[15])
+      PG_SYM_CE(d[1], d[2]) PG_SYM_CE(d[5], d[6]) PG_SYM_CE(d[9], d[10]) PG_SYM_CE(d[13], d[14]) PG_SYM_CE(d[0], d[4]) PG_SYM_CE(d[1], d[5]) PG_SYM_CE(d[2], d[6]) PG_SYM_CE(d[3], d[7])
+      PG_SYM_CE(d[8], d[12]) PG_SYM_CE(d[9], d[13]) PG_SYM_CE(d[10], d[14]) PG_SYM_CE(d[11], d[15]) PG_SYM_CE(d[2], d[4]) PG_SYM_CE(d[3], d[5]) PG_SYM_CE(d[10], d[12]) PG_SYM_CE(d[11], d[13])
+      PG_SYM_CE(d[1], d[2]) PG_SYM_CE(d[3], d[4]) PG_SYM_CE(d[5], d[6]) PG_SYM_CE(d[9], d[10]) PG_SYM_CE(d[11], d[12]) PG_SYM_CE(d[13], d[14]) PG_SYM_CE(d[0], d[8]) PG_SYM_CE(d[1], d[9])
+      PG_SYM_CE(d[2], d[10]) PG_SYM_CE(d[3], d[11]) PG_SYM_CE(d[4], d[12]) PG_SYM_CE(d[5], d[13]) PG_SYM_CE(d[6], d[14]) PG_SYM_CE(d[7], d[15]) PG_SYM_CE(d[4], d[8]) PG_SYM_CE(d[5], d[9])
+      PG_SYM_CE(d[6], d[10]) PG_SYM_CE(d[7], d[11]) PG_SYM_CE(d[2], d[4]) PG_SYM_CE(d[3], d[5]) PG_SYM_CE(d[6], d[8]) PG_SYM_CE(d[7], d[9]) PG_SYM_CE(d[10], d[12]) PG_SYM_CE(d[11], d[13])
+      PG_SYM_CE(d[1], d[2]) PG_SYM_CE(d[3], d[4]) PG_SYM_CE(d[5], d[6]) PG_SYM_CE(d[7], d[8]) PG_SYM_CE(d[9], d[10]) PG_SYM_CE(d[11], d[12]) PG_SYM_CE(d[13], d[14])
+    }
+    {
+      const long long next = first + (long long)gridDim.x * (4 * PG_WG_WAVES);
+      u32 zero = 0u;
+      asm volatile("" : "+v"(zero));
+      if (next < nrows) { hs0 = pieceStart[next >> 6]; hs1 = pieceStart[(next >> 6) + 1]; hlogged = lowCount[next + zero]; }
+    }
+    int pos = 0, used = 0;
     u32 head = has ? own[b * kRec + off] : 0xFFFFFFFFu, res = 0xFFFFFFFFu;
     for (int r = 0; r <= k; ++r) {
-      u32 m = head < d0 ? head : d0, x;
+      u32 m = head < d[0] ? head : d[0], x;
       x = PG_SYM_ROR(m, 8); m = x < m ? x : m;
       x = PG_SYM_ROR(m, 4); m = x < m ? x : m;
       x = PG_SYM_ROR(m, 2); m = x < m ? x : m;
@@ -539,11 +596,8 @@
         ++pos;
         head = pos < k1 ? own[b * kRec + off + pos] : 0xFFFFFFFFu;
       }
-      const bool dwin = any && d0 == m;
-      d0 = dwin ? d1 : d0; d1 = dwin ? d2 : d1; d2 = dwin ? d3 : d2; d3 = dwin ? d4 : d3;
-      d4 = dwin ? d5 : d4; d5 = dwin ? d6 : d5; d6 = dwin ? d7 : d6; d7 = dwin ? d8 : d7;
-      d8 = dwin ? d9 : d8; d9 = dwin ? d10 : d9; d10 = dwin ? d11 : d10; d11 = dwin ? d12 : d11;
-      d12 = dwin ? d13 : d12; d13 = dwin ? d14 : d13; d14 = dwin ? d15 : d14; d15 = dwin ? 0xFFFFFFFFu : d15;
+      sym_window_pop<W>(d, used, any && d[0] == m);
+      if (__builtin_amdgcn_ballot_w64(sym_window_empty<W>(used)) != 0) sym_window_refill<W>(d, used);
       if (b == r - 1) res = m;
       if (b == 0 && mine) {
         if (r > 16) {
@@ -579,7 +633,7 @@
 static const probe_fn kProbe[8] = {pg_launch_probe_g1, pg_launch_probe_g2, pg_launch_probe_g3, pg_launch_probe_g4,
                                    pg_launch_probe_g5, pg_launch_probe_g6, pg_launch_probe_g7, pg_launch_probe_g8};
 static int run_probe(const NsqParams &e, int l, int bits, u32 near, u32 lo, u32 span, u32 need, void *workspace, hipStream_t s,
-                     const PgKnobs &kn, const u32 **gate) {
+                     const PgKnobs &kn, const u32 **gate, const SymPlanArgs *ride = nullptr) {
   if (!workspace) return pg_fail(PG_E_BADARG, "workspace required (pg_workspace_bytes)");
   u32 *gates = (u32 *)((char *)workspace + PG_WS_GATES), *counts = (u32 *)((char *)workspace + PG_WS_COUNTS);
   ProbeParams pp;
@@ -593,8 +647,9 @@
   if (int rc = pg_launched(kProbe[pg_ngroups(l) - 1](bits, pp, s), "pg_probe_kernel")) return rc;
   const int force = (int)kn.gateForce.v;
   static_assert(PG_WS_GATES / 4 <= 1024, "pg_decide_kernel zeroes one word per thread");
-  pg_decide_kernel<<<dim3(1), dim3(1024), 0, s>>>(counts, pp.nsample, pp.wavesPerRow, need, e.ncols, force, gates, (u32 *)workspace,
-                                                  PG_WS_GATES / 4);
+  const SymPlanArgs none = {};
+  pg_decide_kernel<<<dim3(1u + (ride ? ride->grid : 0u)), dim3(1024), 0, s>>>(counts, pp.nsample, pp.wavesPerRow, need, e.ncols, force, gates, (u32 *)workspace,
+                                                                              PG_WS_GATES / 4, ride ? *ride : none);
   if (int rc = pg_launched("pg_decide_kernel")) return rc;
   *gate = gates;
   return 0;
@@ -955,6 +1010,11 @@
   set_rows_plan(&q, &grid, r.pl.valu, r.kn);
   return pg_launched(kNsq[r.ng - 1](PG_MODE_KNN, r.bits, q, grid, r.stream), "pg_nsq_kernel(knn)");
 }
+static SymPlanArgs sym_plan_args(const KnnPlan &pl, void *workspace) {
+  char *base = (char *)workspace + pl.symBase;
+  return SymPlanArgs{pl.symNb, pl.symNst, pl.symSlots, pl.symPiece, pl.symPieceMin, (int4 *)(base + pl.symWs.plan), (u32 *)(base + pl.symWs.pieceStart),
+                     (uint4 *)(base + pl.symWs.lowCount), pl.symZero4, pl.symPlanGrid};
+}
 static int launch_sym(const KnnRun &r) {
   const KnnPlan &pl = r.pl;
   char *base = (char *)r.workspace + pl.symBase;
@@ -974,12 +1034,15 @@
   s.mmGridWaves = pl.symGridWaves;
   s.mmPassCounter = r.p.mmPassCounter + 16;
   u32 *pieceStart = (u32 *)(base + pl.symWs.pieceStart), *gate2 = r.gates() + 2;
-  if (r.kn.debugPlan.set) fprintf(stderr, "[pg plan sym] rows=%lld: %lld passes for %lld slots\n", (long long)r.nrows, pl.symPasses, pl.symSlots);
-  pg_knn_sym_plan_kernel<<<dim3(pl.symPlanGrid), dim3(1024), 0, r.stream>>>(pl.symNb, pl.symNst, pl.symSlots, pl.symPiece, pl.symPieceMin, (int4 *)(base + pl.symWs.plan),
-                                                                            pieceStart, (uint4 *)sa.lowCount, pl.symZero4);
-  if (int rc = pg_launched("pg_knn_sym_plan_kernel")) return rc;
+  if (r.kn.debugPlan.set) fprintf(stderr, "[pg plan sym] rows=%lld: %lld passes for %lld slots, plan %s, merge window %d\n", (long long)r.nrows, pl.symPasses, pl.symSlots,
+                                 pl.symPlanRides ? "rides in the decide launch" : "launched", pl.symMergeWindow);
+  if (!pl.symPlanRides) {
+    pg_knn_sym_plan_kernel<<<dim3(pl.symPlanGrid), dim3(1024), 0, r.stream>>>(sym_plan_args(pl, r.workspace));
+    if (int rc = pg_launched("pg_knn_sym_plan_kernel")) return rc;
+  }
   if (int rc = pg_launched(kMmSym[r.ng - 1](s, (int)(s.mmGridWaves / PG_WG_WAVES), r.stream), "pg_mm_knn_sym_kernel")) return rc;
-  pg_knn_sym_merge_kernel<<<dim3(pl.symMergeGrid), dim3(PG_WG_THREADS), 0, r.stream>>>(
+  auto *merge = pl.symMergeWindow == 1 ? pg_knn_sym_merge_kernel<1> : (pl.symMergeWindow == 2 ? pg_knn_sym_merge_kernel<2> : pg_knn_sym_merge_kernel<4>);
+  merge<<<dim3(pl.symMergeGrid), dim3(PG_WG_THREADS), 0, r.stream>>>(
       sa.partial, pieceStart, sa.lowCount, sa.lowKeys, sa.capL, sa.rowBits, r.nrows, r.k, r.idx, r.dist, r.p.knnGuess, r.p.mmEvict,
       r.p.mmEvictRows, s.gate, s.gateMask, gate2, r.p.mmPassCounter + 17, (u32)(pl.symLimit < 0 ? 0 : pl.symLimit));
   return pg_launched("pg_knn_sym_merge_kernel");
@@ -1042,7 +1105,8 @@
   if (!pl.mm) return launch_valu(r, false);
   if (pl.probe) {
     const u32 *gate = nullptr;
-    if (int rc = run_probe(r.p, l, bits, pl.guess, 1u, 0u, (u32)(first + k), workspace, r.stream, kn, &gate)) return rc;
+    const SymPlanArgs ride = pl.symPlanRides ? sym_plan_args(pl, workspace) : SymPlanArgs{};
+    if (int rc = run_probe(r.p, l, bits, pl.guess, 1u, 0u, (u32)(first + k), workspace, r.stream, kn, &gate, pl.symPlanRides ? &ride : nullptr)) return rc;
     if (int rc = launch_valu(r, true)) return rc;
     r.p.gate = gate;
   }
diff --git a/prograph_amd/csrc/pg_plan.h b/prograph_amd/csrc/pg_plan.h
--- a/prograph_amd/csrc/pg_plan.h
+++ b/prograph_amd/csrc/pg_plan.h
@@ -53,6 +53,25 @@
   const uint32_t rows = n > first ? n - first : 0u;
   return (rows < 16u ? rows : 16u) * capL;
 }
+#define PG_SYM_NONE 0xFFFFFFFFu
+template <int W> PG_HD static inline void sym_window_pop(uint32_t (&d)[16], int &used, bool win) {
+  static_assert(W == 1 || W == 2 || W == 4 || W == 16, "window widths that divide sixteen");
+#ifdef __HIPCC__
+#pragma unroll
+#endif
+  for (int j = 0; j < W - 1; ++j) d[j] = win ? d[j + 1] : d[j];
+  d[W - 1] = win ? PG_SYM_NONE : d[W - 1];
+  used += win ? 1 : 0;
+}
+template <int W> PG_HD static inline bool sym_window_empty(int used) { return W < 16 && used == W; }
+template <int W> PG_HD static inline void sym_window_refill(uint32_t (&d)[16], int &used) {
+  const bool full = sym_window_empty<W>(used);
+#ifdef __HIPCC__
+#pragma unroll
+#endif
+  for (int j = 0; j < 16; ++j) d[j] = full ? (j + W < 16 ? d[j + W < 16 ? j + W : 15] : PG_SYM_NONE) : d[j];
+  used = full ? 0 : used;
+}
 
 #define PG_PROBE_ROWS 64
 #define PG_PROBE_WAVES 128
@@ -68,7 +87,7 @@
 struct PgKnobs {
   PgKnob lbFilter, wavesPerCu, rowsPerWave, debugPlan, engine, engineMinRows, probe, probeS, probeW, gateForce, epsOrdered;
   PgKnob knnGuess, mmShort, mmR, mmSplit, mmEvict, mmPieces, mmPiecesAhead, mmPlan, mmTail, mmPersistent, mmL1, mmL2, mmRun;
-  PgKnob knnSym, symCapL, symPiece, symPieceMin, symOcc, symDeliver, symEvictLimit, symMergeWgs;
+  PgKnob knnSym, symCapL, symPiece, symPieceMin, symOcc, symDeliver, symEvictLimit, symMergeWgs, symMergeWindow;
 };
 enum { PG_ENGINE_AUTO = 0, PG_ENGINE_MFMA = 1, PG_ENGINE_VALU = 2 };
 enum PgKnobRule { PG_KNOB_ANY, PG_KNOB_CLAMP, PG_KNOB_RANGE, PG_KNOB_WIDE, PG_KNOB_NAME };
@@ -113,6 +132,7 @@
     {"PG_KNN_SYM_DELIVER", &PgKnobs::symDeliver, 1, 0, 0, PG_KNOB_ANY, "0: timing experiments, wrong results"},
     {"PG_KNN_SYM_EVICT_LIMIT", &PgKnobs::symEvictLimit, 0, 0, 0, PG_KNOB_WIDE, "evicted rows up to which the sweep's results stand (default: a sixteenth of the rows)"},
     {"PG_KNN_SYM_MERGE_WGS", &PgKnobs::symMergeWgs, 0, 1, PG_KNOB_MAX, PG_KNOB_RANGE, "workgroups of the sweep's merge at most (tests; default and bound: eight a CU)"},
+    {"PG_KNN_SYM_MERGE_WINDOW", &PgKnobs::symMergeWindow, 0, 1, 2, PG_KNOB_RANGE, "delivered keys in the window of the merge's rounds: 1 or 2 (tests: the refill runs often; default: four)"},
 };
 
 static inline PgKnob pg_knob_parse(const PgKnobSpec &s, const char *text) {
@@ -404,6 +424,8 @@
   int symRowBits;
   bool symDeliver;
   unsigned symPlanGrid, symMergeGrid;
+  int symMergeWindow;
+  bool symPlanRides;
   int64_t symBase;
   SymWs symWs;
   bool alt32;
@@ -473,6 +495,8 @@
     long long mergeCap = rowsCap;
     if (kn.symMergeWgs.v >= 1 && kn.symMergeWgs.v < mergeCap) mergeCap = kn.symMergeWgs.v;
     pl.symMergeGrid = (unsigned)(mergeWgs < mergeCap ? mergeWgs : mergeCap);
+    pl.symMergeWindow = kn.symMergeWindow.v >= 1 ? (int)kn.symMergeWindow.v : 4;
+    pl.symPlanRides = pl.probe;
     if (!pl.probe) pl.mainGateMask = (1u << 0) | (1u << 2);
   }
   pl.evictGateMask = pl.mainGateMask | (pl.sym ? 1u << 3 : 0u);
```

New measurement: 41880 billion sequence-pairs/s, median of 6. +2.0%, better.
